# gooofy/zerovox

Hardware: AMD Instinct MI355X
Metric: audio samples/sec + RTF, 128-phoneme zero-shot synth @22.05kHz, 1/2/4/8 GPU (higher is better)
Workload: dtype f16+bf16

## Files before the change

### zerovox_amd/csrc/attention.hip

```cpp
#include "mfma_util.h"
#include "zvx_kernels.h"

#include <type_traits>

namespace zvx {

#ifndef FA_EXP
#define FA_EXP 0
#endif
#ifdef FA_PROFILE
#define FA_STAMP(k) do { const unsigned long long t_ = __builtin_readcyclecounter(); tacc[k] += t_ - tlast; tlast = t_; } while (0)
#else
#define FA_STAMP(k) do {} while (0)
#endif
#define FA_BQ 128
#define FA_BK 64
#define FA_NKB (FA_BK / 32)
#define FA_TAU 8.0f

typedef __attribute__((ext_vector_type(8))) _Float16 fa_f16x8;
template <bool F16>
__device__ __forceinline__ unsigned fa_pack2(float lo, float hi) {
    if (F16) {
        typedef _Float16 h2 __attribute__((ext_vector_type(2)));
// ... 278 lines not shown
        constexpr int C4N = NCOLS / 4, N = NROWS * C4N, IT = (N + 255) / 256;
        AfTile<IT> t;
#pragma unroll
        for (int it = 0; it < IT; it++) {
            const int i = tid + it * 256, r = i / C4N, c4 = i - r * C4N, row = row0 + r;
            t.v[it] = make_float4(0.f, 0.f, 0.f, 0.f);
            if (i < N && row < len) t.v[it] = *(const float4*)(src + (long)row * a.ld + c4 * 4);
        }
        return t;
    };
    auto tile_commit = [&](const auto& t, auto nrows_c, auto ncols_c, float* dst, int pitch) {
        constexpr int NROWS = decltype(nrows_c)::value, NCOLS = decltype(ncols_c)::value;
        constexpr int C4N = NCOLS / 4, N = NROWS * C4N, IT = (N + 255) / 256;
#pragma unroll
        for (int it = 0; it < IT; it++) {
            const int i = tid + it * 256, r = i / C4N, c4 = i - r * C4N;
            if (i < N) *(float4*)(dst + r * pitch + c4 * 4) = t.v[it];
        }
    };
    auto load_tile = [&](const float* src, int row0, auto nrows_c, auto ncols_c, float* dst, int pitch) {
        tile_commit(tile_fetch(src, row0, nrows_c, ncols_c), nrows_c, ncols_c, dst, pitch);
    };
    constexpr std::integral_constant<int, AF_BQ> c_bq{};
    constexpr std::integral_constant<int, AF_BK> c_bk{};
    constexpr std::integral_constant<int, D> c_d{};
    constexpr std::integral_constant<int, C0> c_c0{};
    constexpr std::integral_constant<int, C1> c_c1{};
    load_tile(base + a.q_off, q0, c_bq, c_d, Qs, QP);

    f32x16 o0, o1, o2;
#pragma unroll
    for (int e = 0; e < 16; e++) { o0[e] = 0.f; o1[e] = 0.f; o2[e] = 0.f; }
    float m_run = -INFINITY, l_run = 0.f;
    const int srow = tid >> 3, ssub = tid & 7;
    const float* const qrow = Qs + l32 * QP + 4 * kh;
    const float* const krow = Ks + (wave * 32 + l32) * KP + 4 * kh;
    const float* const prow = Ps + l32 * PP + 4 * kh;

    const int ntiles = (len + AF_BK - 1) / AF_BK;
    for (int kt = 0; kt < ntiles; kt++) {
        const int k0 = kt * AF_BK;
        const bool my_keys = k0 + wave * 32 < len;
        f32x16 s, s2;
#pragma unroll
        for (int e = 0; e < 16; e++) { s[e] = 0.f; s2[e] = 0.f; }
        __syncthreads();
        load_tile(base + a.k_off, k0, c_bk, c_c0, Ks, KP);
        __syncthreads();
        const auto k1 = tile_fetch(base + a.k_off + C0, k0, c_bk, c_c1);
        if (my_keys) {
#pragma unroll
            for (int j = 0; j < C0 / 8; j++) {
                const float4 qa = *(const float4*)(qrow + 8 * j), kb = *(const float4*)(krow + 8 * j);
                s = __builtin_amdgcn_mfma_f32_32x32x2f32(qa.x, kb.x, s, 0, 0, 0);
                s2 = __builtin_amdgcn_mfma_f32_32x32x2f32(qa.y, kb.y, s2, 0, 0, 0);
                s = __builtin_amdgcn_mfma_f32_32x32x2f32(qa.z, kb.z, s, 0, 0, 0);
                s2 = __builtin_amdgcn_mfma_f32_32x32x2f32(qa.w, kb.w, s2, 0, 0, 0);
            }
        }
        __syncthreads();
        tile_commit(k1, c_bk, c_c1, Ks, KP);
        const auto v0 = tile_fetch(base + a.v_off, k0, c_bk, c_c0);
        __syncthreads();
        if (my_keys) {
#pragma unroll
            for (int j = 0; j < C1 / 8; j++) {
                const float4 qa = *(const float4*)(qrow + C0 + 8 * j), kb = *(const float4*)(krow + 8 * j);
                s = __builtin_amdgcn_mfma_f32_32x32x2f32(qa.x, kb.x, s, 0, 0, 0);
                s2 = __builtin_amdgcn_mfma_f32_32x32x2f32(qa.y, kb.y, s2, 0, 0, 0);
                s = __builtin_amdgcn_mfma_f32_32x32x2f32(qa.z, kb.z, s, 0, 0, 0);
                s2 = __builtin_amdgcn_mfma_f32_32x32x2f32(qa.w, kb.w, s2, 0, 0, 0);
            }
            s += s2;
        }
#pragma unroll
        for (int e = 0; e < 16; e++) Ps[(8 * (e >> 2) + 4 * kh + (e & 3)) * PP + wave * 32 + l32] = s[e] * a.scale;
        __syncthreads();
        tile_commit(v0, c_bk, c_c0, Ks, KP);
        const auto v1 = tile_fetch(base + a.v_off + C0, k0, c_bk, c_c1);
        {
            float* const pr = Ps + srow * PP + ssub * 16;
            float v[16];
#pragma unroll
            for (int i = 0; i < 4; i++) { const float4 t = *(const float4*)(pr + 4 * i); v[4 * i] = t.x; v[4 * i + 1] = t.y; v[4 * i + 2] = t.z; v[4 * i + 3] = t.w; }
            const int kbase = k0 + ssub * 16;
            float m = -INFINITY;
#pragma unroll
            for (int i = 0; i < 16; i++) if (kbase + i < len) m = fmaxf(m, v[i]);
            m = fmaxf(m, __shfl_xor(m, 1, 64)); m = fmaxf(m, __shfl_xor(m, 2, 64)); m = fmaxf(m, __shfl_xor(m, 4, 64));
            const float m_new = fmaxf(m_run, m);
            const float alpha = m_run == -INFINITY ? 0.f : expf(m_run - m_new);
            float sum = 0.f;
#pragma unroll
            for (int i = 0; i < 16; i++) { v[i] = kbase + i < len ? expf(v[i] - m_new) : 0.f; sum += v[i]; }
            sum += __shfl_xor(sum, 1, 64); sum += __shfl_xor(sum, 2, 64); sum += __shfl_xor(sum, 4, 64);
            l_run = alpha * l_run + sum; m_run = m_new;
#pragma unroll
            for (int i = 0; i < 4; i++) *(float4*)(pr + 4 * i) = make_float4(v[4 * i], v[4 * i + 1], v[4 * i + 2], v[4 * i + 3]);
            if (ssub == 0) As[srow] = alpha;
        }
        __syncthreads();
        {
            float al[16];
#pragma unroll
            for (int g = 0; g < 4; g++) { const float4 t = *(const float4*)(As + 8 * g + 4 * kh); al[4 * g] = t.x; al[4 * g + 1] = t.y; al[4 * g + 2] = t.z; al[4 * g + 3] = t.w; }
#pragma unroll
            for (int e = 0; e < 16; e++) { o0[e] *= al[e]; o1[e] *= al[e]; o2[e] *= al[e]; }
        }
        auto pv_tile = [&](f32x16 acc, int col) {
            const float* const vc = Ks + col + 4 * kh * KP;
            f32x16 acc2;
#pragma unroll
            for (int e = 0; e < 16; e++) acc2[e] = 0.f;
#pragma unroll
            for (int j = 0; j < AF_BK / 8; j++) {
                const float4 pa = *(const float4*)(prow + 8 * j);
                const float* const vj = vc + 8 * j * KP;
                acc = __builtin_amdgcn_mfma_f32_32x32x2f32(pa.x, vj[0], acc, 0, 0, 0);
                acc2 = __builtin_amdgcn_mfma_f32_32x32x2f32(pa.y, vj[KP], acc2, 0, 0, 0);
                acc = __builtin_amdgcn_mfma_f32_32x32x2f32(pa.z, vj[2 * KP], acc, 0, 0, 0);
                acc2 = __builtin_amdgcn_mfma_f32_32x32x2f32(pa.w, vj[3 * KP], acc2, 0, 0, 0);
            }
            return acc + acc2;
        };
        o0 = pv_tile(o0, wave * 32 + l32);
        __syncthreads();
        tile_commit(v1, c_bk, c_c1, Ks, KP);
        __syncthreads();
        o1 = pv_tile(o1, min(wave * 32 + l32, C1 - 1));
        if (NT1 > 4 && wave == 3) o2 = pv_tile(o2, min(128 + l32, C1 - 1));
    }
    __syncthreads();
    if (ssub == 0) As[srow] = 1.0f / l_run;
    __syncthreads();
    float* const op = a.out + (long)b * a.o_bs + (long)h * D;
    auto store_tile = [&](const f32x16& acc, int col) {
        if (col >= D) return;
#pragma unroll
        for (int e = 0; e < 16; e++) {
            const int r = 8 * (e >> 2) + 4 * kh + (e & 3), q = q0 + r;
            if (q < a.L) {
                const float val = q < len ? acc[e] * As[r] : 0.f;
                op[(long)q * a.ldo + col] = val;
                if (a.planes) {
                    unsigned short hi, lo;
                    if (a.planes_f16) {
                        const _Float16 hh = (_Float16)__builtin_amdgcn_fmed3f(val, -65504.f, 65504.f);
                        hi = __builtin_bit_cast(unsigned short, hh);
                        lo = __builtin_bit_cast(unsigned short, (_Float16)__builtin_amdgcn_fmed3f((val - (float)hh) * 2048.f, -65504.f, 65504.f));
                    } else {
                        hi = __builtin_bit_cast(unsigned short, (__bf16)val);
                        lo = __builtin_bit_cast(unsigned short, (__bf16)(val - __uint_as_float((unsigned)hi << 16)));
                    }
                    unsigned short* const pp = a.planes + ((long)b * a.L + q) * 3 * a.planes_C + h * D + col;
                    pp[0] = hi; pp[a.planes_C] = hi; pp[2 * a.planes_C] = lo;
                }
            }
        }
    };
    store_tile(o0, wave * 32 + l32);
    store_tile(o1, C0 + wave * 32 + l32);
    if (NT1 > 4 && wave == 3) store_tile(o2, C0 + 128 + l32);
}

bool launch_attention_f32(const AttnF32Args& a, hipStream_t stream, bool dry_run) {
    if (a.D != 264 || a.L <= 0 || a.ld % 4 || a.q_off % 4 || a.k_off % 4 || a.v_off % 4) return false;
    if (dry_run) return true;
    if ((size_t)a.qkv & 15) return false;
    constexpr int D = 264, KP = (D - 128) + 4;
    const size_t lds = sizeof(float) * ((size_t)AF_BQ * (D + 4) + (size_t)AF_BK * KP + (size_t)AF_BQ * (AF_BK + 4) + 32);
    auto kfn = attn_f32_kernel<264>;
    if (!lds_opt_in((const void*)kfn)) return false;
    const dim3 grid((a.L + AF_BQ - 1) / AF_BQ, a.nbatch * a.nheads), block(256);
    hipLaunchKernelGGL(kfn, grid, block, lds, stream, a);
    return true;
}

}
```

### zerovox_amd/csrc/gemm.hip

```cpp
#include "mfma_util.h"
#include "zvx_kernels.h"

#include <cstring>
#include <type_traits>

#ifndef ZVX_GEMM_PART
#define ZVX_GEMM_PART 0
#endif
#define ZVX_PART_MAIN (ZVX_GEMM_PART != 2)
#define ZVX_PART_RESFUSE (ZVX_GEMM_PART != 1)
#if ZVX_GEMM_PART == 2
extern thread_local bool zvx_gemm_dry_run;
#else
thread_local hipEvent_t zvx_gemm_ev_start = nullptr, zvx_gemm_ev_stop = nullptr;
thread_local bool zvx_gemm_dry_run = false;
#endif
#define g_dry_run zvx_gemm_dry_run

#define ZVX_LAUNCH(...) do { if (!g_dry_run) ZVX_DISPATCH(__VA_ARGS__); } while (0)

namespace zvx {


#define PITCH 80
// ... 594 lines not shown
    constexpr bool WREG = R == 0;
    constexpr int F = BN / 32, CNT = F >= 4 ? F / 4 : 1, WD = 4, D = WREG ? WD : R - 1, WAITN = WREG ? (WD - 1) * TN : (D - 2) * CNT;
    const int nt32_total = (a.N + 31) >> 5;
    const int nsteps = a.ntaps * 4, gtotal = nkc * nsteps + nkc2 * 4;
    const uint4* wsrc[CNT];
#pragma unroll
    for (int j = 0; j < CNT; j++) {
        const int f = wave * CNT + j, t32 = (n0 >> 5) + f;
        wsrc[j] = (const uint4*)a.Wp + (long)(t32 < nt32_total ? t32 : 0) * gtotal * 64 + lane;
    }
    const int xrow0 = HL + wr * (BM / WM) + (lane & 31);
    const int koff = (lane >> 5) * 16;
    unsigned char* ring = slab + ((SR * SLAB_PITCH + 1023) & ~1023);
    const unsigned lds_base = (unsigned)(size_t)(__attribute__((address_space(3))) unsigned char*)slab;
    const int dvreg = a.dv[lane & (ZVX_MAX_TAPS - 1)];
    const bool loader = wave * CNT < F;
    const unsigned char* wq[TN];
#pragma unroll
    for (int i = 0; i < TN; i++) {
        const int t32 = (n0 >> 5) + wc * TN + i;
        wq[i] = (const unsigned char*)a.Wp + (long)(t32 < nt32_total ? t32 : 0) * gtotal * 1024;
    }
    const bool wave_dead = __builtin_amdgcn_readfirstlane((int)(n0 + wc * TN * 32 >= a.N)) != 0;
    const unsigned lane16 = lane * 16;
    u32x4 wreg[WREG ? WD : 1][TN] = {};
    auto wload = [&](int gs, int slot) {
        const long off = (long)(gs < gtotal ? gs : gtotal - 1) * 1024;
#pragma unroll
        for (int i = 0; i < TN; i++)
            asm volatile("global_load_dwordx4 %0, %1, %2" : "+v"(wreg[WREG ? slot : 0][i]) : "v"(lane16), "s"(wq[i] + off) : "memory");
    };
    auto dma = [&](int gs) {
        if (WREG || !loader) return;
        const int slot = gs & (R - 1);
        const long off = (long)(gs < gtotal ? gs : gtotal - 1) * 64;
#pragma unroll
        for (int j = 0; j < CNT; j++)
            __builtin_amdgcn_global_load_lds((const __attribute__((address_space(1))) void*)(wsrc[j] + off),
                                             (__attribute__((address_space(3))) void*)(ring + (slot * F + wave * CNT + j) * 1024), 16, 0, 0);
    };
    if (WREG) { wload(0, 0); wload(1, 1); wload(2, 2); wload(3, 3); }
    else {
#pragma unroll
        for (int s0 = 0; s0 < D; s0++) dma(s0);
    }

    for (int kc = 0; kc < nkc + nkc2; kc++) {
        const bool src2 = !FULLK && kc >= nkc;
        const unsigned short* const Xs = src2 ? Xp2 : Xp;
        const int ldxs = src2 ? a.ldx2 : a.ldx, Ks = src2 ? a.K2 : a.K, kbase = (src2 ? kc - nkc : kc) * SLAB_KC;
        {
            constexpr int FCH = NIT > 10 ? (NIT + 1) / 2 : NIT;
#pragma unroll
            for (int h0 = 0; h0 < NIT; h0 += FCH) {
                uint4 sv[FCH];
#pragma unroll
                for (int i = 0; i < FCH; i++) {
                    const int it = h0 + i;
                    const int c = tid + it * 256;
                    const int row = c >> 3, q = c & 7;
                    const int g = m0 - HL + row, k = kbase + q * 8;
                    sv[i] = make_uint4(0, 0, 0, 0);
                    if (it < NIT && c < SR * 8 && g >= 0 && g < in_rows && k < Ks && ((rowmask >> it) & 1)) sv[i] = *(const uint4*)(Xs + (long)g * ldxs + k);
                }
                if (kc && h0 == 0) __syncthreads();
#pragma unroll
                for (int i = 0; i < FCH; i++) {
                    const int c = tid + (h0 + i) * 256;
                    if (h0 + i < NIT && c < SR * 8) *(uint4*)(slab + (c >> 3) * SLAB_PITCH + (c & 7) * 16) = sv[i];
                }
            }
        }
        __syncthreads();
        int nk16 = 4;
        if (!FULLK) { nk16 = src2 ? n16_2 - (kc - nkc) * 4 : n16 - kc * 4; if (nk16 > 4) nk16 = 4; if (wave_dead) nk16 = 0; }
        const int ntaps_kc = src2 ? 1 : ntaps;

        uint4 xA[TM], wA[TN], xB[TM], wB[TN];
        const unsigned ring_rd = lds_base + (unsigned)(size_t)(ring - slab) + lane * 16 + wc * TN * 1024;
        const int gs0 = src2 ? nkc * nsteps + (kc - nkc) * 4 : kc * nsteps;
        auto rd = [&](uint4 (&xf)[TM], uint4 (&wf)[TN], int gs, unsigned rowoff, int kk) {
            if (!WREG) {
                const unsigned wa = ring_rd + (gs & ((WREG ? 1 : R) - 1)) * (F * 1024);
#pragma unroll
                for (int i = 0; i < TN; i++)
                    asm volatile("ds_read_b128 %0, %1 offset:%2" : "=v"(wf[i]) : "v"(wa), "n"(i * 1024));
            }
#pragma unroll
            for (int j = 0; j < TM; j++)
                asm volatile("ds_read_b128 %0, %1" : "=v"(xf[j]) : "v"(lds_base + rowoff + j * 32 * SLAB_PITCH + kk * 32));
        };
        auto mma = [&](uint4 (&xf)[TM], uint4 (&wf)[TN]) {
#pragma unroll
            for (int i = 0; i < TN; i++)
#pragma unroll
                for (int j = 0; j < TM; j++)
                    acc[i][j] = F16 ? __builtin_amdgcn_mfma_f32_32x32x16_f16(__builtin_bit_cast(f16x8, wf[i]), __builtin_bit_cast(f16x8, xf[j]), acc[i][j], 0, 0, 0)
                                    : __builtin_amdgcn_mfma_f32_32x32x16_bf16(__builtin_bit_cast(bf16x8, wf[i]),
                                                                       __builtin_bit_cast(bf16x8, xf[j]), acc[i][j], 0, 0, 0);
        };
        auto mma_r = [&](uint4 (&xf)[TM], int slot) {
#pragma unroll
            for (int i = 0; i < TN; i++)
#pragma unroll
                for (int j = 0; j < TM; j++)
                    acc[i][j] = F16 ? __builtin_amdgcn_mfma_f32_32x32x16_f16(__builtin_bit_cast(f16x8, wreg[WREG ? slot : 0][i]), __builtin_bit_cast(f16x8, xf[j]), acc[i][j], 0, 0, 0)
                                    : __builtin_amdgcn_mfma_f32_32x32x16_bf16(__builtin_bit_cast(bf16x8, wreg[WREG ? slot : 0][i]),
                                                                       __builtin_bit_cast(bf16x8, xf[j]), acc[i][j], 0, 0, 0);
        };
        auto rowoff_of = [&](int tap) {
            const int d = src2 ? 0 : __builtin_amdgcn_readlane(dvreg, tap < ntaps ? tap : ntaps - 1);
            return (unsigned)((xrow0 + d) * SLAB_PITCH + koff);
        };
        unsigned rowoff = rowoff_of(0);
        rd(xA, wA, gs0, rowoff, 0);
        for (int tap = 0; tap < ntaps_kc; tap++) {
            const unsigned rowoff_next = rowoff_of(tap + 1);
#pragma unroll
            for (int kk = 0; kk < 4; kk++) {
                const int gs = gs0 + tap * 4 + kk;
                if (WREG) asm volatile("s_waitcnt vmcnt(%0)" :: "n"(WAITN) : "memory");
                else asm volatile("s_waitcnt vmcnt(%0)\n\ts_barrier" :: "n"(WAITN) : "memory");
                dma(gs + D);
                if (kk & 1) rd(xA, wA, gs + 1, kk == 3 ? rowoff_next : rowoff, (kk + 1) & 3);
                else        rd(xB, wB, gs + 1, rowoff, kk + 1);
                asm volatile("s_waitcnt lgkmcnt(%0)" :: "n"(WREG ? TM : TM + TN) : "memory");
                __builtin_amdgcn_sched_barrier(0);
                if (FULLK || kk < nk16) {
                    if (WREG) { if (kk & 1) mma_r(xB, kk); else mma_r(xA, kk); }
                    else { if (kk & 1) mma(xB, wB); else mma(xA, wA); }
                }
                __builtin_amdgcn_sched_barrier(0);
                if (WREG) wload(gs + WD, kk);
            }
            rowoff = rowoff_next;
        }
        asm volatile("s_waitcnt lgkmcnt(0)" ::: "memory");
    }
    if (WREG) {
#pragma unroll
        for (int sl = 0; sl < (WREG ? WD : 1); sl++)
#pragma unroll
            for (int i = 0; i < TN; i++) asm volatile("s_waitcnt vmcnt(0)" : "+v"(wreg[sl][i]) :: "memory");
    } else {
        asm volatile("s_waitcnt vmcnt(0)" ::: "memory");
    }
    __syncthreads();
    if (EPI == ZVX_EPI_FLIP)
        epilogue_direct<TM, TN, !F16>(a, acc, b, m0 + wr * (BM / WM), n0 + wc * (BN / WN), out_len, lane, slab + wave * (32 * (TN * 64 + 16)));
    else if (EPI == ZVX_EPI(0, 0, 1))
        epilogue_direct<TM, TN, F16>(a, acc, b, m0 + wr * (BM / WM), n0 + wc * (BN / WN), out_len, lane, slab + wave * (32 * (TN * 64 + 16)));
    else
        epilogue_rows<TM, TN, 0, EPI, (F16 && EPI >= 0)>(a, acc, b, m0 + wr * (BM / WM), n0 + wc * (BN / WN), out_len, lane, slab + wave * (32 * (TN * 32 * 4 + 16)));
}

template <int C, int NT, int BM, int WM, int WN, int MINW, int MAXH = 64, bool F16 = false>
__global__ __launch_bounds__(256, MINW) void convreg_kernel(const GemmArgs a) {
    constexpr int TM = BM / WM / 32;
    constexpr int KS = C / 16;
    constexpr int PITCH_ = C * 2 + 16;
    constexpr int CPR = C / 8;
    constexpr int NIT = ((BM + MAXH) * CPR + 255) / 256;
    constexpr int FCH = NIT > 12 ? 8 : NIT;
    static_assert(WM * WN == 4 && WN * 32 == C, "wave layout");
    extern __shared__ __attribute__((aligned(16))) unsigned char slab[];

    const int tid = threadIdx.x, lane = tid & 63, wave = tid >> 6;
    const int wr = wave % WM, wc = wave / WM;
    int wg;
    {
        const int nwg = gridDim.x, id = blockIdx.x, q = nwg >> 3, r = nwg & 7, xcd = id & 7;
        wg = (xcd < r ? xcd * (q + 1) : r * (q + 1) + (xcd - r) * q) + (id >> 3);
    }
    const int m0 = wg * BM, b = blockIdx.y;
    const int out_len = a.out_len ? a.out_len[b] : a.M;
    const int in_len = a.in_len ? a.in_len[b] : a.in_len_static;
    if (m0 >= out_len || m0 >= a.M) return;
    const int HL = a.halo_l, SR = BM + a.halo_l + a.halo_r;
    const unsigned short* Xp = (const unsigned short*)a.X + (long)b * a.x_bs;

    uint4 w[NT][KS];
    {
        const uint4* Wq = (const uint4*)a.Wp + ((long)wc * NT * 4) * 64 + lane;
#pragma unroll
        for (int t = 0; t < NT; t++)
#pragma unroll
            for (int kk = 0; kk < KS; kk++) w[t][kk] = Wq[(t * 4 + kk) * 64];
    }
    {
        const bool flat = MAXH > 64 && a.flat_win;
        const int in_rows = flat ? a.flat_rows : in_len;
#pragma unroll
        for (int h0 = 0; h0 < NIT; h0 += FCH) {
            uint4 sv[FCH];
#pragma unroll
            for (int i = 0; i < FCH; i++) {
                const int c = tid + (h0 + i) * 256;
                const int row = c / CPR, q = c % CPR;
                const int g = m0 - HL + row;
                sv[i] = make_uint4(0, 0, 0, 0);
                if (h0 + i < NIT && c < SR * CPR && g >= 0 && g < in_rows && (!flat || (g % a.flat_win) < in_len)) sv[i] = *(const uint4*)(Xp + (long)g * a.ldx + q * 8);
            }
#pragma unroll
            for (int i = 0; i < FCH; i++) {
                const int c = tid + (h0 + i) * 256;
                if (h0 + i < NIT && c < SR * CPR) *(uint4*)(slab + (c / CPR) * PITCH_ + (c % CPR) * 16) = sv[i];
            }
        }
    }
    __syncthreads();

    f32x16 acc[1][TM];
#pragma unroll
    for (int j = 0; j < TM; j++)
#pragma unroll
        for (int e = 0; e < 16; e++) acc[0][j][e] = 0.f;
    const int xrow0 = HL + wr * (BM / WM) + (lane & 31);
    const int koff = (lane >> 5) * 16;
#pragma unroll
    for (int t = 0; t < NT; t++) {
        const unsigned char* rowp = slab + (xrow0 + a.dv[t]) * PITCH_ + koff;
#pragma unroll
        for (int kk = 0; kk < KS; kk++)
#pragma unroll
            for (int j = 0; j < TM; j++) {
                const uint4 xf = *(const uint4*)(rowp + j * 32 * PITCH_ + kk * 32);
                acc[0][j] = mfma16<F16>(w[t][kk], xf, acc[0][j]);
            }
    }
    __syncthreads();
    epilogue_rows<TM, 1>(a, acc, b, m0 + wr * (BM / WM), wc * 32, out_len, lane, slab + wave * (32 * (32 * 4 + 16)));
}

typedef __attribute__((ext_vector_type(2))) unsigned u32x2_t;
__device__ __forceinline__ void store_block_mfma_layout(unsigned short* row_ptr , const uint2 (&pk)[4], int lane, bool ok) {
#pragma unroll
    for (int pr = 0; pr < 2; pr++) {
        const u32x2_t sx = __builtin_amdgcn_permlane32_swap(pk[2 * pr].x, pk[2 * pr + 1].x, false, false);
        const u32x2_t sy = __builtin_amdgcn_permlane32_swap(pk[2 * pr].y, pk[2 * pr + 1].y, false, false);
        if (ok) *(u32x4*)(row_ptr + 8 * (2 * pr + (lane >> 5))) = (u32x4){sx.x, sy.x, sx.y, sy.y};
    }
}

template <int C, int BM, int WM, int WN, int MAXH, int MODE, int WGPC, bool POOL = false>
__global__ __launch_bounds__(WM * WN * 64, WM * WN * WGPC / 4) void conv2d_persist_kernel(const GemmArgs a, const int ntm, const int ntiles) {
    constexpr int NTHR = WM * WN * 64;
    constexpr int NT = 9, TM = BM / WM / 32, KS = C / 16, PITCH_ = C * 2 + 16, CPR = C / 8, RSTEP = NTHR / CPR;
    constexpr int NIT = ((BM + MAXH) * CPR + NTHR - 1) / NTHR;
    constexpr bool EC_LDS = NTHR > 256;
    static_assert(WN * 32 == C && BM % (WM * 32) == 0, "wave layout");
    extern __shared__ __attribute__((aligned(16))) unsigned char slab[];

    const int tid = threadIdx.x, lane = tid & 63, wave = __builtin_amdgcn_readfirstlane(tid >> 6);
    const int wr = wave % WM, wc = wave / WM;
    const int G = gridDim.x, xcd = blockIdx.x & 7, slot = blockIdx.x >> 3;
    auto tile_of = [&](int r) {
        const int base = r * G, n = ntiles - base < G ? ntiles - base : G;
        if (n <= 0) return ntiles;
        const int per = (n + 7) >> 3, t = xcd * per + slot;
        return (slot < per && t < n) ? base + t : ntiles;
    };
    const int HL = a.halo_l, SR = BM + a.halo_l + a.halo_r, win = a.flat_win, in_rows = a.flat_rows;

    uint4 w[NT][KS];
    {
        const uint4* Wq = (const uint4*)a.Wp + ((long)wc * NT * 4) * 64 + lane;
#pragma unroll
        for (int t = 0; t < NT; t++)
#pragma unroll
            for (int kk = 0; kk < KS; kk++) w[t][kk] = Wq[(t * 4 + kk) * 64];
    }
    float* const ecl = (float*)(slab + ((SR * PITCH_ + 15) & ~15));
    float4 ec0[EC_LDS ? 1 : 4], ec1[(MODE == 1 && !EC_LDS) ? 4 : 1];
    if (EC_LDS) {
        if (tid < C) { ecl[tid] = MODE == 0 ? a.bias[tid] : a.post_scale[tid]; if (MODE == 1) ecl[C + tid] = a.post_shift[tid]; }
    } else {
#pragma unroll
        for (int g = 0; g < 4; g++) {
            const int ch = wc * 32 + 8 * g + 4 * (lane >> 5);
            if (MODE == 0) ec0[g] = *(const float4*)(a.bias + ch);
            else { ec0[g] = *(const float4*)(a.post_scale + ch); ec1[g] = *(const float4*)(a.post_shift + ch); }
        }
    }
    u32x4 sv[NIT];
    const int row_t = tid / CPR, q8 = (tid % CPR) * 8;
    auto request = [&](int t) __attribute__((always_inline)) {
        const int b = t / ntm, m0 = (t - b * ntm) * BM;
        const int in_len = a.in_len[b];
        const __amdgpu_buffer_rsrc_t rs = __builtin_amdgcn_make_buffer_rsrc((void*)((const unsigned short*)a.X + (long)b * a.x_bs), 0, in_rows * a.ldx * 2, 0x00020000);
        int g = m0 - HL + row_t;
        int col = (g + 2 * win) % win;
#pragma unroll
        for (int it = 0; it < NIT; it++) {
            const bool ok = tid + it * NTHR < SR * CPR && g >= 0 && g < in_rows && col < in_len;
            sv[it] = __builtin_amdgcn_raw_buffer_load_b128(rs, ok ? (g * a.ldx + q8) * 2 : (int)0x80000000, 0, 0);
            g += RSTEP; col += RSTEP; if (col >= win) col -= win;
        }
    };
    int r = 0, t = tile_of(0);
    if (t < ntiles) request(t);
    const int xrow0 = HL + wr * (BM / WM) + (lane & 31);
    const int koff = (lane >> 5) * 16;
    constexpr bool pool = MODE == 0 && POOL;
    while (t < ntiles) {
        const int b = t / ntm, mt = t - b * ntm, m0 = mt * BM;
        if (r) asm volatile("s_waitcnt lgkmcnt(0)\n\ts_barrier" ::: "memory");
// ... 872 lines not shown
    if (a.flat_win && !a.bflat) {
        if (a.N == a.K && (a.N == 32 || a.N == 64) && !(a.slab_small & 32) && a.dtype == DT_BF16 && a.ntaps == 9 && a.in_len && !a.out_len && hl == a.flat_win + 1 && hr == hl &&
            a.flat_win >= 64 && (long)a.flat_rows * a.ldx * 2 < 0x7fffffffL &&
            a.out && a.out_dtype == DT_BF16 && a.alpha == 1.f && a.out_scale == 1.f && !a.res_mode && !a.accum_mode && !a.out_split3 && a.ldo % 8 == 0 &&
            ((a.post_scale && a.post_shift && a.bias_mode == 0 && a.act == ACT_RELU) || (!a.post_scale && a.bias_mode == 1 && a.bias && a.act == ACT_NONE))) {
            if (a.N == 32 && hl + hr <= 544) { launch_conv2d_persist<32, 384, 4, 1, 544, 2>(a, stream); return 26; }
            if (a.N == 64 && hl + hr <= 288) { launch_conv2d_persist<64, 256, 4, 2, 288, 1>(a, stream); return 27; }
        }
        if (a.N == a.K && a.N == 32 && launch_convreg_c<32, 384, 4, 1, 2>(a, stream)) return 14;
        if (a.N == a.K && a.N == 64 && launch_convreg_c<64, 256, 2, 2, 2>(a, stream)) return 15;
        if (a.N % 128 || a.K % SLAB_KC || hl + hr > 160) return -4;
        const int pad256 = ((a.M + 255) / 256) * 256, pad128 = ((a.M + 127) / 128) * 128;
        if ((long)pad256 * 100 > (long)pad128 * 115) {
            dim3 g128((a.N / 128) * (pad128 / 128), a.nbatch);
            size_t lds128 = ((size_t)(128 + hl + hr) * SLAB_PITCH + 1023) & ~(size_t)1023;
            const size_t stage128 = (size_t)4 * 32 * (2 * 128 + 16);
            if (lds128 < stage128) lds128 = stage128;
            ZVX_LAUNCH((convslab_kernel<128, 128, 2, 2, true, 2, 0, -1, 160>), g128, dim3(256), lds128, stream, a);
            return 22;
        }
        dim3 grid((a.N / 128) * ((a.M + 255) / 256), a.nbatch);
        size_t lds = ((size_t)(256 + hl + hr) * SLAB_PITCH + 1023) & ~(size_t)1023;
        ZVX_LAUNCH((convslab_kernel<256, 128, 2, 2, true, 2, 0, -1, 160>), grid, dim3(256), lds, stream, a);
        return 7;
    }
    if (a.dtype != DT_F32 && a.N == a.K && !a.K2 && (a.ntaps == 3 || a.ntaps == 5 || a.ntaps == 7 || a.ntaps == 11)) {
        if (a.N == 32 && launch_convreg_c<32, 512, 4, 1, 2>(a, stream)) return 14;
        if (a.N == 64 && launch_convreg_c<64, 256, 2, 2, 2>(a, stream)) return 15;
    }
    if (hl + hr > 64) {
        if (hl + hr <= 160 && a.N % 128 == 0 && a.K % SLAB_KC == 0 && !a.K2 && !a.bflat && !a.flat_win && gemm_epi_mode_of(a) == ZVX_EPI(1, 1, 1)) {
            dim3 grid((a.N / 128) * ((a.M + 255) / 256), a.nbatch);
            const size_t lds = ((size_t)(256 + hl + hr) * SLAB_PITCH + 1023) & ~(size_t)1023;
            if (a.dtype == DT_F16) ZVX_LAUNCH((convslab_kernel<256, 128, 2, 2, true, 2, 0, ZVX_EPI(1, 1, 1), 160, true>), grid, dim3(256), lds, stream, a);
            else ZVX_LAUNCH((convslab_kernel<256, 128, 2, 2, true, 2, 0, ZVX_EPI(1, 1, 1), 160>), grid, dim3(256), lds, stream, a);
            return 7;
        }
        return -4;
    }
    static const int bns[4] = {256, 128, 64, 32};
    static const double eff[4] = {0.95, 1.0, 0.7, 0.4};
    int best = 0; double best_cost = -1;
    for (int i = 0; i < 4; i++) {
        const double cost = (double)((a.N + bns[i] - 1) / bns[i]) * bns[i] / eff[i];
        if (best_cost < 0 || cost < best_cost - 1e-9) { best_cost = cost; best = i; }
    }
    static const int bms[4] = {128, 256, 256, 256};
    const int ncu = num_cus();
    if (g_slab_small >= 2 && a.M <= 64 && a.nbatch * ((a.N + 127) / 128) * 4 <= ncu && a.N >= 64 && hl + hr <= 64) {
        a.bflat = 0;
        dim3 g32((a.N + 31) / 32, a.nbatch);
        const size_t lds32 = (((size_t)(256 + hl + hr) * SLAB_PITCH + 1023) & ~(size_t)1023) + (size_t)8 * 1024;
        launch_slab_variant<256, 32, 4, 1, 2, 8>(a, g32, lds32, stream);
        return 9;
    }
    if (g_slab_small && a.M > 128 && a.N >= 128 && hl + hr <= 64) {
        const long wg256 = (long)((a.N + 127) / 128) * ((a.M + 255) / 256) * a.nbatch;
        if (wg256 * 2 <= ncu) {
            a.bflat = 0;
            const bool r64 = wg256 * 4 <= ncu;
            const int bm = r64 ? 64 : 128;
            dim3 gs(((a.N + 127) / 128) * ((a.M + bm - 1) / bm), a.nbatch);
            size_t lds = ((size_t)(bm + hl + hr) * SLAB_PITCH + 1023) & ~(size_t)1023;
            const size_t stage = (size_t)4 * 32 * (2 * 128 + 16);
            if (lds < stage) lds = stage;
            if (r64) launch_slab_variant<64, 128, 2, 2, 2, 0>(a, gs, lds, stream);
            else launch_slab_variant<128, 128, 2, 2, 2, 0>(a, gs, lds, stream);
            return 22;
        }
    }
    if (a.M <= 128 && a.N >= 128) {
        a.bflat = 0;
        const int wide = ((a.N + 255) / 256) * a.nbatch;
        const bool narrow = wide < 2 * ncu;
        const int bn = narrow ? 128 : 256;
        dim3 grid((a.N + bn - 1) / bn, a.nbatch);
        size_t lds = ((size_t)(128 + hl + hr) * SLAB_PITCH + 1023) & ~(size_t)1023;
        const size_t stage = (size_t)4 * 32 * (2 * 128 + 16);
        if (lds < stage) lds = stage;
        if (narrow && a.M > (g_slab_small ? 32 : 64) && ((a.N + 127) / 128) * a.nbatch < 2 * ncu) {
            dim3 g64(((a.N + 127) / 128) * ((a.M + 63) / 64), a.nbatch);
            launch_slab_variant<64, 128, 2, 2, 2, 0>(a, g64, lds, stream);
            return 22;
        }
        if (narrow) { launch_slab_variant<128, 128, 2, 2, 2, 0>(a, grid, lds, stream); return 22; }
        launch_slab_variant<128, 256, 1, 4, 2, 0>(a, grid, lds, stream);
        return 6;
    }
    if (a.ntaps == 1 && a.N >= 512) {
        const long slots = 2L * ncu;
        auto rounds = [&](int bm_, int bn_) {
            const long ntn_ = (a.N + bn_ - 1) / bn_, utt = ntn_ * ((a.M + bm_ - 1) / bm_) * a.nbatch;
            const long flat = a.bflat ? ntn_ * (((long)a.nbatch * a.bflat + bm_ - 1) / bm_) : utt;
            return ((flat < utt ? flat : utt) + slots - 1) / slots;
        };
        best = rounds(256, 128) <= rounds(128, 256) ? 1 : 0;
    }
    const bool wreg = best <= 1;
    const int ring_slots = wreg ? 0 : (best == 0 ? 4 : 8);
    const int bn = bns[best], bm = bms[best];
    const int ntn = (a.N + bn - 1) / bn;
    if (a.bflat) {
        const long slots = 2L * ncu;
        const long wg_utt = (long)ntn * ((a.M + bm - 1) / bm) * a.nbatch, wg_flat = (long)ntn * (((long)a.nbatch * a.bflat + bm - 1) / bm);
        if ((wg_flat + slots - 1) / slots < (wg_utt + slots - 1) / slots) { a.flat_win = a.bflat; a.flat_rows = a.nbatch * a.bflat; a.M = a.flat_rows; a.nbatch = 1; }
        else a.bflat = 0;
    }
    if (best == 1 && bflat_hint && a.M > 256 && hl + hr <= 64) {
        const long slots = 2L * ncu;
        const long t256 = (long)ntn * ((a.M + 255) / 256) * a.nbatch, t128 = (long)ntn * ((a.M + 127) / 128) * a.nbatch;
        const long eff256 = 2 * ((t256 + slots - 1) / slots), eff128 = (t128 + slots - 1) / slots;
        if (eff128 < eff256) {
            dim3 g128(ntn * ((a.M + 127) / 128), a.nbatch);
            size_t lds128 = ((size_t)(128 + hl + hr) * SLAB_PITCH + 1023) & ~(size_t)1023;
            const size_t stage128 = (size_t)4 * 32 * (2 * 128 + 16);
            if (lds128 < stage128) lds128 = stage128;
            switch (gemm_epi_mode_of(a)) {
                case ZVX_EPI(0, 0, 1): launch_slab_variant<128, 128, 2, 2, 2, 0, ZVX_EPI(0, 0, 1)>(a, g128, lds128, stream); break;
                case ZVX_EPI_DEC(0): launch_slab_variant<128, 128, 2, 2, 2, 0, ZVX_EPI_DEC(0)>(a, g128, lds128, stream); break;
                case ZVX_EPI_DEC(1): launch_slab_variant<128, 128, 2, 2, 2, 0, ZVX_EPI_DEC(1)>(a, g128, lds128, stream); break;
                default: launch_slab_variant<128, 128, 2, 2, 2, 0>(a, g128, lds128, stream);
            }
            return 22;
        }
    }
    const int ntm = (a.M + bm - 1) / bm;
    dim3 grid(ntn * ntm, a.nbatch);
    const int tn = (bn >= 128) ? 2 : 1;
    if (a.accum_mode && a.accum && a.accum_dtype == DT_F16 && tn == 2 && !(best == 1 && gemm_epi_mode_of(a) >= 0)) return -6;
    size_t lds = (((size_t)(bm + hl + hr) * SLAB_PITCH + 1023) & ~(size_t)1023) + (size_t)ring_slots * (bn / 32) * 1024;
    const size_t stage = (size_t)4 * 32 * (tn * 128 + 16);
    if (lds < stage) lds = stage;
    switch (best) {
        case 0: launch_slab_variant<128, 256, 1, 4, 2, 0>(a, grid, lds, stream); break;
        case 1: switch (gemm_epi_mode_of(a)) {
                    case ZVX_EPI(0, 0, 1): launch_slab_variant<256, 128, 2, 2, 2, 0, ZVX_EPI(0, 0, 1)>(a, grid, lds, stream); break;
                    case ZVX_EPI_FLIP: launch_slab_variant<256, 128, 2, 2, 2, 0, ZVX_EPI_FLIP>(a, grid, lds, stream); break;
                    case ZVX_EPI(1, 0, 1): launch_slab_variant<256, 128, 2, 2, 2, 0, ZVX_EPI(1, 0, 1)>(a, grid, lds, stream); break;
                    case ZVX_EPI(1, 2, 0): launch_slab_variant<256, 128, 2, 2, 2, 0, ZVX_EPI(1, 2, 0)>(a, grid, lds, stream); break;
                    case ZVX_EPI(1, 3, 0): launch_slab_variant<256, 128, 2, 2, 2, 0, ZVX_EPI(1, 3, 0)>(a, grid, lds, stream); break;
                    case ZVX_EPI(1, 1, 1): launch_slab_variant<256, 128, 2, 2, 2, 0, ZVX_EPI(1, 1, 1)>(a, grid, lds, stream); break;
                    case ZVX_EPI_DEC(0): launch_slab_variant<256, 128, 2, 2, 2, 0, ZVX_EPI_DEC(0)>(a, grid, lds, stream); break;
                    case ZVX_EPI_DEC(1): launch_slab_variant<256, 128, 2, 2, 2, 0, ZVX_EPI_DEC(1)>(a, grid, lds, stream); break;
                    default: launch_slab_variant<256, 128, 2, 2, 2, 0>(a, grid, lds, stream);
                }
                break;
        case 2: launch_slab_variant<256, 64, 2, 2, 2, 8>(a, grid, lds, stream); break;
        case 3: launch_slab_variant<256, 32, 4, 1, 2, 8>(a, grid, lds, stream); break;
    }
    return 6 + best;
}


int launch_gemm(const GemmArgs& a, hipStream_t stream) {
    if (a.N <= 0 || a.M <= 0 || a.nbatch <= 0) return -1;
    if (a.ds_out) return launch_conv2d_s2(a, stream) ? 28 : -7;
    if (a.stride == 2 && a.wout > 0 && a.ntaps == 9 && a.K == 64 && a.Wp && launch_conv2d_s2(a, stream)) return 29;
    if (a.ntaps < 1 || a.ntaps > ZVX_MAX_TAPS) return -2;
    if (a.out_split3 && (a.out_dtype != DT_F32 || a.N % 8 || a.flat_win || a.wout > 0)) return -2;
    if (a.N % 4 && (a.bias_mode == 1 || a.res_mode || a.accum_mode || a.post_scale || a.ldo < ((a.N + 3) & ~3))) return -2;
    if (a.Wp && a.dtype == DT_BF16 && a.wout > 0 && a.stride == 1 && a.ntaps == 9 && a.wout == a.win && a.M == a.hin * a.win && a.nheads == 1 && a.w_bs == 0 &&
        !a.k_len && a.K % 16 == 0 && a.N % 32 == 0 && a.ldo % 8 == 0 && a.ldx == a.K && !a.res_mode && !a.accum_mode && a.bias_mode != 2 && a.win <= 271) {
        bool ok9 = true;
        for (int t = 0; t < 9; t++) ok9 = ok9 && a.du[t] == t / 3 - 1 && a.dv[t] == t % 3 - 1;
        if (ok9 && (a.N == a.K ? (a.N == 32 || a.N == 64 || (a.N % 128 == 0 && 2 * (a.win + 1) <= 160)) : false)) {
            GemmArgs f = a;
            f.flat_win = a.win; f.flat_rows = a.hin * a.win;
            for (int t = 0; t < 9; t++) { f.dv[t] = a.du[t] * a.win + a.dv[t]; f.du[t] = 0; }
            f.wout = 0; f.out_len = nullptr;
            const int id = launch_convslab(f, stream);
            if (id >= 0) return id;
        }
    }
    if (a.Wp && a.dtype != DT_F32 && a.wout <= 0 && a.nheads == 1 && a.w_bs == 0 && !a.k_len && a.K % 16 == 0 && a.N % 8 == 0 && a.ldo % 8 == 0) {
        int lo = 0, hi = 0;
        for (int i = 0; i < a.ntaps; i++) { if (a.dv[i] < lo) lo = a.dv[i]; if (a.dv[i] > hi) hi = a.dv[i]; }
        if (hi - lo <= 64 && hi >= 0 && lo <= 0) return launch_convslab(a, stream);
        if (hi - lo <= 96 && hi >= 0 && lo <= 0 && a.ntaps == 7 && a.N == a.K && (a.N == 32 || a.N == 64 || a.N == 128) && !a.K2 && !a.out_split3 && !a.bflat) {
            const int id = launch_convslab(a, stream);
            if (id >= 0) return id;
        }
    }
    if (a.out_split3 || a.K2) return -2;
    static const int bns[3] = {128, 64, 32};
    static const double eff[3] = {1.0, 0.75, 0.45};
    int best = 0; double best_cost = -1;
    for (int i = 0; i < 3; i++) {
        const double cost = (double)((a.N + bns[i] - 1) / bns[i]) * bns[i] / eff[i];
        if (best_cost < 0 || cost < best_cost - 1e-9) { best_cost = cost; best = i; }
    }
    int bn = bns[best], bm = (bn == 128) ? 128 : 256;
    int ntn = (a.N + bn - 1) / bn, ntm = (a.M + bm - 1) / bm;
    if ((long)ntn * ntm * a.nbatch * a.nheads < 512 && a.N >= 64) {
        bm = bn = 64; ntn = (a.N + 63) / 64; ntm = (a.M + 63) / 64;
        dim3 grid(ntn * ntm, a.nbatch * a.nheads), block(256);
        if (a.dtype == DT_BF16) { ZVX_LAUNCH((gemm_kernel<DT_BF16, 64, 64, 2, 2>), grid, block, 0, stream, a); return 18; }
        if (a.dtype == DT_F16) { ZVX_LAUNCH((gemm_kernel<DT_F16, 64, 64, 2, 2>), grid, block, 0, stream, a); return 18; }
        ZVX_LAUNCH((gemm_kernel<DT_F32, 64, 64, 2, 2>), grid, block, 0, stream, a);
        return 19;
    }
    dim3 grid(ntn * ntm, a.nbatch * a.nheads), block(256);
    const int base = (a.dtype != DT_F32) ? 0 : 3;
    const int id = base + best;
    if (a.dtype == DT_F16) {
        switch (id) {
            case 0: ZVX_LAUNCH((gemm_kernel<DT_F16, 128, 128, 2, 2>), grid, block, 0, stream, a); break;
            case 1: ZVX_LAUNCH((gemm_kernel<DT_F16, 256, 64, 4, 1>), grid, block, 0, stream, a); break;
            case 2: ZVX_LAUNCH((gemm_kernel<DT_F16, 256, 32, 4, 1>), grid, block, 0, stream, a); break;
        }
        return id;
    }
    switch (id) {
        case 0: ZVX_LAUNCH((gemm_kernel<DT_BF16, 128, 128, 2, 2>), grid, block, 0, stream, a); break;
        case 1: ZVX_LAUNCH((gemm_kernel<DT_BF16, 256, 64, 4, 1>), grid, block, 0, stream, a); break;
        case 2: ZVX_LAUNCH((gemm_kernel<DT_BF16, 256, 32, 4, 1>), grid, block, 0, stream, a); break;
        case 3: ZVX_LAUNCH((gemm_kernel<DT_F32, 128, 128, 2, 2>), grid, block, 0, stream, a); break;
        case 4: ZVX_LAUNCH((gemm_kernel<DT_F32, 256, 64, 4, 1>), grid, block, 0, stream, a); break;
        case 5: ZVX_LAUNCH((gemm_kernel<DT_F32, 256, 32, 4, 1>), grid, block, 0, stream, a); break;
    }
    return id;
}

int gemm_variant_of(const GemmArgs& a) {
    g_dry_run = true;
    const int id = a.fused == 2 ? launch_rb2fuse(a, nullptr) : (a.fused ? launch_resfuse(a, nullptr) : launch_gemm(a, nullptr));
    g_dry_run = false;
    return id;
}

#endif
}
```

### zerovox_amd/csrc/ops.hip

```cpp
#include "zvx_kernels.h"

#include <algorithm>

namespace zvx {

__device__ __forceinline__ float ld(const void* p, int dt, long i) {
    if (dt == DT_F16) return (float)((const _Float16*)p)[i];
    return dt == DT_F32 ? ((const float*)p)[i] : __uint_as_float(((unsigned)((const unsigned short*)p)[i]) << 16);
}
__device__ __forceinline__ unsigned short tobf(float f) {
    unsigned u = __float_as_uint(f);
    u += 0x7fffu + ((u >> 16) & 1u);
    return (unsigned short)(u >> 16);
}
__device__ __forceinline__ void unpack8(const uint4 t, int dt, float v[8]) {
    if (dt == DT_F16) {
        typedef _Float16 h2 __attribute__((ext_vector_type(2)));
        const h2 a = __builtin_bit_cast(h2, t.x), b = __builtin_bit_cast(h2, t.y), c = __builtin_bit_cast(h2, t.z), d = __builtin_bit_cast(h2, t.w);
        v[0] = (float)a.x; v[1] = (float)a.y; v[2] = (float)b.x; v[3] = (float)b.y; v[4] = (float)c.x; v[5] = (float)c.y; v[6] = (float)d.x; v[7] = (float)d.y;
    } else {
        v[0] = __uint_as_float(t.x << 16); v[1] = __uint_as_float(t.x & 0xffff0000u);
        v[2] = __uint_as_float(t.y << 16); v[3] = __uint_as_float(t.y & 0xffff0000u);
        v[4] = __uint_as_float(t.z << 16); v[5] = __uint_as_float(t.z & 0xffff0000u);
        v[6] = __uint_as_float(t.w << 16); v[7] = __uint_as_float(t.w & 0xffff0000u);
    }
}
__device__ __forceinline__ float clamp_h(float v) { return __builtin_amdgcn_fmed3f(v, -65504.f, 65504.f); }
__device__ __forceinline__ uint4 pack8(const float v[8], int dt) {
    uint4 o;
    if (dt == DT_F16) {
        typedef _Float16 h2 __attribute__((ext_vector_type(2)));
        o.x = __builtin_bit_cast(unsigned, (h2){(_Float16)clamp_h(v[0]), (_Float16)clamp_h(v[1])}); o.y = __builtin_bit_cast(unsigned, (h2){(_Float16)clamp_h(v[2]), (_Float16)clamp_h(v[3])});
        o.z = __builtin_bit_cast(unsigned, (h2){(_Float16)clamp_h(v[4]), (_Float16)clamp_h(v[5])}); o.w = __builtin_bit_cast(unsigned, (h2){(_Float16)clamp_h(v[6]), (_Float16)clamp_h(v[7])});
    } else {
        o.x = (unsigned)tobf(v[0]) | ((unsigned)tobf(v[1]) << 16); o.y = (unsigned)tobf(v[2]) | ((unsigned)tobf(v[3]) << 16);
        o.z = (unsigned)tobf(v[4]) | ((unsigned)tobf(v[5]) << 16); o.w = (unsigned)tobf(v[6]) | ((unsigned)tobf(v[7]) << 16);
    }
    return o;
}
__device__ __forceinline__ void st(void* p, int dt, long i, float v) {
    if (dt == DT_F16) { ((_Float16*)p)[i] = (_Float16)clamp_h(v); return; }
    if (dt == DT_F32) ((float*)p)[i] = v; else ((unsigned short*)p)[i] = tobf(v);
}
__device__ __forceinline__ float wave_sum(float v) {
#pragma unroll
    for (int o = 32; o > 0; o >>= 1) v += __shfl_xor(v, o, 64);
    return v;
}
__device__ __forceinline__ float wave_max(float v) {
#pragma unroll
    for (int o = 32; o > 0; o >>= 1) v = fmaxf(v, __shfl_xor(v, o, 64));
    return v;
}
__device__ __forceinline__ float act_apply(float v, int act, float slope) {
    if (act == ACT_RELU) return fmaxf(v, 0.f);
    if (act == ACT_LRELU) return v >= 0.f ? v : v * slope;
    if (act == ACT_TANH) return tanhf(v);
    return v;
}

__global__ void k_cast(const void* in, int idt, void* out, int odt, size_t n) {
    size_t i = (size_t)blockIdx.x * blockDim.x + threadIdx.x;
    const size_t stride = (size_t)gridDim.x * blockDim.x;
    for (; i < n; i += stride) st(out, odt, i, ld(in, idt, i));
}
void launch_cast(const void* in, int in_dt, void* out, int out_dt, size_t n, hipStream_t s) {
    if (!n) return;
    int blocks = (int)((n + 255) / 256); if (blocks > 4096) blocks = 4096;
    hipLaunchKernelGGL(k_cast, dim3(blocks), dim3(256), 0, s, in, in_dt, out, out_dt, n);
}
__global__ __launch_bounds__(256) void k_transpose16(const unsigned short* in, int ld_in, unsigned short* out, int ld_out, int rows_max, int C, const int* len) {
    __shared__ unsigned short tile[64][66];
    const int b = blockIdx.z, r0 = blockIdx.y * 64, c0 = blockIdx.x * 64;
    const int rows = len ? min(len[b], rows_max) : rows_max;
    const unsigned short* ip = in + (long)b * rows_max * ld_in;
    unsigned short* op = out + (long)b * C * ld_out;
    for (int i = threadIdx.x; i < 64 * 64; i += 256) {
        const int r = i >> 6, c = i & 63;
        tile[r][c] = (r0 + r < rows && c0 + c < C) ? ip[(long)(r0 + r) * ld_in + c0 + c] : (unsigned short)0;
    }
    __syncthreads();
    for (int i = threadIdx.x; i < 64 * 64; i += 256) {
        const int c = i >> 6, r = i & 63;
        if (c0 + c < C && r0 + r < ld_out) op[(long)(c0 + c) * ld_out + r0 + r] = (r0 + r < rows) ? tile[r][c] : (unsigned short)0;
    }
}
void launch_transpose16(const void* in, int ld_in, void* out, int ld_out, int B, int rows, int C, hipStream_t s, const int* len) {
    if (rows <= 0) return;
    hipLaunchKernelGGL(k_transpose16, dim3((C + 63) / 64, (ld_out + 63) / 64, B), dim3(256), 0, s, (const unsigned short*)in, ld_in, (unsigned short*)out, ld_out, rows, C, len);
}

void launch_f32_to_bf16(const float* in, bf16_t* out, size_t n, hipStream_t s) { launch_cast(in, DT_F32, out, DT_BF16, n, s); }

__device__ __forceinline__ void split2(float v, unsigned short& hi, unsigned short& lo) {
    hi = tobf(v);
    lo = tobf(v - __uint_as_float(((unsigned)hi) << 16));
}
__device__ __forceinline__ void split2h(float v, unsigned short& hi, unsigned short& lo) {
    const _Float16 h = (_Float16)clamp_h(v);
    hi = __builtin_bit_cast(unsigned short, h);
    lo = __builtin_bit_cast(unsigned short, (_Float16)clamp_h((v - (float)h) * 2048.f));
}
__device__ __forceinline__ void split2x(float v, int f16, unsigned short& hi, unsigned short& lo) { if (f16) split2h(v, hi, lo); else split2(v, hi, lo); }
__global__ __launch_bounds__(256) void k_split3(const float* x, int ldx, unsigned short* out, int rows_max, const int* rows, int C, int f16) {
    const int b = blockIdx.y, r = blockIdx.x;
    const bool live = r < (rows ? rows[b] : rows_max);
    const float* xr = x + ((long)b * rows_max + r) * ldx;
    unsigned short* o = out + ((long)b * rows_max + r) * 3 * C;
    for (int c = threadIdx.x * 4; c < C; c += blockDim.x * 4) {
        unsigned short h[4], l[4];
        if (live) { const float4 v = *(const float4*)(xr + c); split2x(v.x, f16, h[0], l[0]); split2x(v.y, f16, h[1], l[1]); split2x(v.z, f16, h[2], l[2]); split2x(v.w, f16, h[3], l[3]); }
        else { for (int e = 0; e < 4; e++) h[e] = l[e] = 0; }
        const uint2 hv = make_uint2(h[0] | ((unsigned)h[1] << 16), h[2] | ((unsigned)h[3] << 16));
        const uint2 lv = make_uint2(l[0] | ((unsigned)l[1] << 16), l[2] | ((unsigned)l[3] << 16));
        *(uint2*)(o + c) = hv; *(uint2*)(o + C + c) = hv; *(uint2*)(o + 2 * C + c) = lv;
    }
}
void launch_split3(const float* x, int ldx, void* out, int B, int rows_max, const int* rows, int C, hipStream_t s, int f16) {
    if (rows_max <= 0) return;
    hipLaunchKernelGGL(k_split3, dim3(rows_max, B), dim3(C >= 1024 ? 256 : 128), 0, s, x, ldx, (unsigned short*)out, rows_max, rows, C, f16);
}
__global__ void k_split3_w(const float* w, unsigned short* out, long nrows, int K, int f16, float scale) {
    const long r = blockIdx.x;
    if (r >= nrows) return;
    for (int k = threadIdx.x; k < K; k += blockDim.x) {
        unsigned short h, l, h3;
        if (f16) {
            const float v = w[r * K + k] * scale;
            const _Float16 wh = (_Float16)clamp_h(v);
            h = __builtin_bit_cast(unsigned short, wh);
            l = __builtin_bit_cast(unsigned short, (_Float16)(v - (float)wh));
            h3 = __builtin_bit_cast(unsigned short, (_Float16)clamp_h(v * (1.0f / 2048.f)));
        } else { split2(w[r * K + k], h, l); h3 = h; }
        out[r * 3 * K + k] = h; out[r * 3 * K + K + k] = l; out[r * 3 * K + 2 * K + k] = h3;
    }
}
void launch_split3_weights(const float* w, void* out, long nrows, int K, hipStream_t s, int f16, float scale) {
    hipLaunchKernelGGL(k_split3_w, dim3((unsigned)nrows), dim3(256), 0, s, w, (unsigned short*)out, nrows, K, f16, scale);
}
__global__ void k_absmax(const float* x, size_t n, unsigned* out) {
    float m = 0.f;
    for (size_t i = (size_t)blockIdx.x * blockDim.x + threadIdx.x; i < n; i += (size_t)gridDim.x * blockDim.x) m = fmaxf(m, fabsf(x[i]));
    m = wave_max(m);
    if ((threadIdx.x & 63) == 0) atomicMax(out, __float_as_uint(m));
}
void launch_absmax(const float* x, size_t n, float* out, hipStream_t s) {
    (void)hipMemsetAsync(out, 0, 4, s);
    if (!n) return;
    int blocks = (int)((n + 255) / 256); if (blocks > 1024) blocks = 1024;
    hipLaunchKernelGGL(k_absmax, dim3(blocks), dim3(256), 0, s, x, n, (unsigned*)out);
}

__global__ void k_embed(const int* ph, const int* pu, const float* emb, int ed, const float* pemb, int pd,
                        const float* pe, float* out, int Tmax, const int* T) {
    const int b = blockIdx.y, t = blockIdx.x;
    if (t >= T[b]) return;
    const int H = ed + pd;
    const int p = ph[b * Tmax + t], q = pu[b * Tmax + t];
    float* o = out + ((long)b * Tmax + t) * H;
    for (int c = threadIdx.x; c < H; c += blockDim.x) {
        float v = c < ed ? emb[(long)p * ed + c] : pemb[(long)q * pd + (c - ed)];
        o[c] = v + pe[(long)t * H + c];
    }
}
void launch_embed(const int* phoneme, const int* puncts, const float* emb, int emb_dim, const float* pemb,
                  int pemb_dim, const float* pe, float* out, int B, int Tmax, const int* T, hipStream_t s) {
    hipLaunchKernelGGL(k_embed, dim3(Tmax, B), dim3(128), 0, s, phoneme, puncts, emb, emb_dim, pemb, pemb_dim, pe, out, Tmax, T);
}

__global__ void k_layernorm(const void* x, int xdt, int ldx, void* y, int ydt, int ldy, int rows_max, const int* rows,
                            int C, int mode, float eps, const float* gamma, const float* beta, const float* bg,
                            long bg_bs, const float* post_add, unsigned short* planes, int planes_f16) {
    const int b = blockIdx.y;
    const int r = blockIdx.x * 4 + (threadIdx.x >> 6);
    const int lane = threadIdx.x & 63;
    const int nr = rows ? rows[b] : rows_max;
    if (r >= nr) {
        if (planes && r < rows_max) { unsigned short* o = planes + ((long)b * rows_max + r) * 3 * C; for (int c = lane; c < 3 * C; c += 64) o[c] = 0; }
        return;
    }
    const long xo = ((long)b * rows_max + r) * ldx, yo = ((long)b * rows_max + r) * ldy;
    if ((C & 7) == 0 && C <= 1024 && (ldx & 7) == 0 && (ldy & 7) == 0) {
        float v[2][8];
        bool has[2];
        float s = 0.f;
#pragma unroll
        for (int i = 0; i < 2; i++) {
            const int c = (lane + 64 * i) * 8;
            has[i] = c < C;
            if (has[i] && xdt == DT_F32) {
                const float4 t0 = *(const float4*)((const float*)x + xo + c), t1 = *(const float4*)((const float*)x + xo + c + 4);
                v[i][0] = t0.x; v[i][1] = t0.y; v[i][2] = t0.z; v[i][3] = t0.w; v[i][4] = t1.x; v[i][5] = t1.y; v[i][6] = t1.z; v[i][7] = t1.w;
            } else if (has[i]) unpack8(*(const uint4*)((const unsigned short*)x + xo + c), xdt, v[i]);
            else { for (int e = 0; e < 8; e++) v[i][e] = 0.f; }
#pragma unroll
            for (int e = 0; e < 8; e++) s += v[i][e];
        }
        const float mu = wave_sum(s) / C;
        float q = 0.f;
#pragma unroll
        for (int i = 0; i < 2; i++)
#pragma unroll
            for (int e = 0; e < 8; e++) { const float d = has[i] ? v[i][e] - mu : 0.f; q += d * d; }
        q = wave_sum(q);
        const float inv = mode == 0 ? 1.0f / sqrtf(q / C + eps) : 1.0f / (sqrtf(q / (C - 1)) + eps);
#pragma unroll
        for (int i = 0; i < 2; i++) {
            if (!has[i]) continue;
            const int c = (lane + 64 * i) * 8;
            const float* gp = mode == 0 ? gamma + c : bg + (long)b * bg_bs + C + c;
            const float* bp = mode == 0 ? beta + c : bg + (long)b * bg_bs + c;
            const float4 g0 = *(const float4*)gp, g1 = *(const float4*)(gp + 4), b0 = *(const float4*)bp, b1 = *(const float4*)(bp + 4);
            const float g[8] = {g0.x, g0.y, g0.z, g0.w, g1.x, g1.y, g1.z, g1.w}, be[8] = {b0.x, b0.y, b0.z, b0.w, b1.x, b1.y, b1.z, b1.w};
            float o[8];
#pragma unroll
            for (int e = 0; e < 8; e++) o[e] = (v[i][e] - mu) * inv * g[e] + be[e];
            if (post_add) {
                const float4 p0 = *(const float4*)(post_add + (long)b * C + c), p1 = *(const float4*)(post_add + (long)b * C + c + 4);
                o[0] += p0.x; o[1] += p0.y; o[2] += p0.z; o[3] += p0.w; o[4] += p1.x; o[5] += p1.y; o[6] += p1.z; o[7] += p1.w;
            }
            if (ydt != DT_F32) *(uint4*)((unsigned short*)y + yo + c) = pack8(o, ydt);
            else {
                *(float4*)((float*)y + yo + c) = make_float4(o[0], o[1], o[2], o[3]);
                *(float4*)((float*)y + yo + c + 4) = make_float4(o[4], o[5], o[6], o[7]);
            }
            if (planes) {
                unsigned short hh[8], ll[8];
#pragma unroll
                for (int e = 0; e < 8; e++) split2x(o[e], planes_f16, hh[e], ll[e]);
                const uint4 hv = make_uint4(hh[0] | ((unsigned)hh[1] << 16), hh[2] | ((unsigned)hh[3] << 16), hh[4] | ((unsigned)hh[5] << 16), hh[6] | ((unsigned)hh[7] << 16));
                const uint4 lv = make_uint4(ll[0] | ((unsigned)ll[1] << 16), ll[2] | ((unsigned)ll[3] << 16), ll[4] | ((unsigned)ll[5] << 16), ll[6] | ((unsigned)ll[7] << 16));
                unsigned short* po = planes + ((long)b * rows_max + r) * 3 * C + c;
                *(uint4*)po = hv; *(uint4*)(po + C) = hv; *(uint4*)(po + 2 * C) = lv;
            }
        }
        return;
    }
    float s = 0.f;
    for (int c = lane; c < C; c += 64) s += ld(x, xdt, xo + c);
    const float mu = wave_sum(s) / C;
    float q = 0.f;
    for (int c = lane; c < C; c += 64) { float d = ld(x, xdt, xo + c) - mu; q += d * d; }
    q = wave_sum(q);
    float inv;
    if (mode == 0) inv = 1.0f / sqrtf(q / C + eps);
    else inv = 1.0f / (sqrtf(q / (C - 1)) + eps);
    for (int c = lane; c < C; c += 64) {
        float g, be;
        if (mode == 0) { g = gamma[c]; be = beta[c]; }
        else { be = bg[(long)b * bg_bs + c]; g = bg[(long)b * bg_bs + C + c]; }
        float v = (ld(x, xdt, xo + c) - mu) * inv * g + be;
        if (post_add) v += post_add[(long)b * C + c];
        st(y, ydt, yo + c, v);
        if (planes) {
            unsigned short hi, lo;
            split2x(v, planes_f16, hi, lo);
            unsigned short* o = planes + ((long)b * rows_max + r) * 3 * C;
            o[c] = hi; o[C + c] = hi; o[2 * C + c] = lo;
        }
    }
}
void launch_layernorm(const void* x, int x_dt, int ldx, void* y, int y_dt, int ldy, int B, int rows_max,
                      const int* rows, int C, int mode, float eps, const float* gamma, const float* beta,
                      const float* bg, long bg_bs, const float* post_add, hipStream_t s, void* split_planes, int planes_f16) {
    hipLaunchKernelGGL(k_layernorm, dim3((rows_max + 3) / 4, B), dim3(256), 0, s, x, x_dt, ldx, y, y_dt, ldy, rows_max,
                       rows, C, mode, eps, gamma, beta, bg, bg_bs, post_add, (unsigned short*)split_planes, planes_f16);
}

__global__ void k_softmax_rows(const float* sc, int lds, void* P, int pdt, int ldp, int nheads, int Lmax, const int* len) {
    const int z = blockIdx.y, b = z / nheads;
    const int r = blockIdx.x * 4 + (threadIdx.x >> 6), lane = threadIdx.x & 63;
    const int L = len[b];
    if (r >= L) return;
    const float* row = sc + ((long)z * Lmax + r) * lds;
    const long po = ((long)z * Lmax + r) * ldp;
    float m = -INFINITY;
    for (int c = lane; c < L; c += 64) m = fmaxf(m, row[c]);
    m = wave_max(m);
    float s = 0.f;
    for (int c = lane; c < L; c += 64) s += expf(row[c] - m);
    s = wave_sum(s);
    const float inv = 1.0f / s;
    const int Lp = (L + 7) & ~7;
    for (int c = lane; c < Lp; c += 64) st(P, pdt, po + c, c < L ? expf(row[c] - m) * inv : 0.f);
}
void launch_softmax_rows(const float* scores, int lds, void* P, int p_dt, int ldp, int nbatch, int nheads,
                         int Lmax, const int* len, hipStream_t s) {
    hipLaunchKernelGGL(k_softmax_rows, dim3((Lmax + 3) / 4, nbatch * nheads), dim3(256), 0, s, scores, lds, P, p_dt, ldp, nheads, Lmax, len);
}

__global__ void k_rowdot(const float* x, int ldx, const float* w, float bias, float* out, int Tmax, const int* T, int C) {
    const int b = blockIdx.y, t = blockIdx.x * 4 + (threadIdx.x >> 6), lane = threadIdx.x & 63;
    if (t >= T[b]) return;
    const float* row = x + ((long)b * Tmax + t) * ldx;
    float s = 0.f;
    for (int c = lane; c < C; c += 64) s += row[c] * w[c];
    s = wave_sum(s);
    if (lane == 0) out[b * Tmax + t] = s + bias;
}
void launch_rowdot(const float* x, int ldx, const float* w, float bias, float* out, int B, int Tmax,
                   const int* T, int C, hipStream_t s) {
    hipLaunchKernelGGL(k_rowdot, dim3((Tmax + 3) / 4, B), dim3(256), 0, s, x, ldx, w, bias, out, Tmax, T, C);
}

__global__ void k_bucket_embed_add(const float* pred, const float* table, int nb, float* x, int ldx, int C, int* idx_out,
                                   int Tmax, const int* T) {
    const int b = blockIdx.y, t = blockIdx.x * 4 + (threadIdx.x >> 6), lane = threadIdx.x & 63;
    if (t >= T[b]) return;
    float p = rintf(pred[b * Tmax + t] * (float)(nb - 1));
    p = fminf(fmaxf(p, 0.f), (float)(nb - 1));
    const int idx = (int)p;
    if (lane == 0 && idx_out) idx_out[b * Tmax + t] = idx;
    float* row = x + ((long)b * Tmax + t) * ldx;
    for (int c = lane; c < C; c += 64) row[c] += table[(long)idx * C + c];
}
void launch_bucket_embed_add(const float* pred, const float* table, int nbins, float* x, int ldx, int C,
                             int* idx_out, int B, int Tmax, const int* T, hipStream_t s) {
    hipLaunchKernelGGL(k_bucket_embed_add, dim3((Tmax + 3) / 4, B), dim3(256), 0, s, pred, table, nbins, x, ldx, C, idx_out, Tmax, T);
}

__global__ void k_bucket_embed_add_ctl(const float* pred, const float* shift, const float* range, const float* target,
                                       const float* table, int nb, float* x, int ldx, int C, int* idx_out, int Tmax, const int* T) {
#pragma clang fp contract(off)
    const int b = blockIdx.y, t = blockIdx.x * 4 + (threadIdx.x >> 6), lane = threadIdx.x & 63;
    const int n = T[b];
    const float* pb = pred + (long)b * Tmax;
    if (blockIdx.x * 4 >= n) return;
    __shared__ float mean_s;
    if (range) {
        if (threadIdx.x < 64) {
            double s = 0.0;
            for (int u = lane; u < n; u += 64) s += (double)pb[u];
#pragma unroll
            for (int o = 32; o > 0; o >>= 1) s += __shfl_xor(s, o, 64);
            if (lane == 0) mean_s = (float)(s / (double)n);
        }
        __syncthreads();
    }
    if (t >= n) return;
    const float r1 = range ? range[b] - 1.0f : 0.f, sh = shift ? shift[b] : 0.f;
    float v = pb[t];
    if (range) v = v + r1 * (v - mean_s);
    if (shift) v = v + sh;
    if (target) { const float g = target[(long)b * Tmax + t]; if (g == g) v = g; }
    float p = rintf(v * (float)(nb - 1));
    p = fminf(fmaxf(p, 0.f), (float)(nb - 1));
    const int idx = (int)p;
    if (lane == 0 && idx_out) idx_out[b * Tmax + t] = idx;
    float* row = x + ((long)b * Tmax + t) * ldx;
    for (int c = lane; c < C; c += 64) row[c] += table[(long)idx * C + c];
}
void launch_bucket_embed_add_ctl(const float* pred, const float* shift, const float* range, const float* target, const float* table,
                                 int nbins, float* x, int ldx, int C, int* idx_out, int B, int Tmax, const int* T, hipStream_t s) {
    hipLaunchKernelGGL(k_bucket_embed_add_ctl, dim3((Tmax + 3) / 4, B), dim3(256), 0, s, pred, shift, range, target, table, nbins, x, ldx, C, idx_out, Tmax, T);
}

__global__ void k_durations(const int* forced, const float* logd, int* dur, int* cum, int* mel_len, int Tmax, const int* T) {
    const int b = blockIdx.x, lane = threadIdx.x;
    const int n = T[b];
    long long carry = 0;
    for (int t0 = 0; t0 < n; t0 += 64) {
        const int t = t0 + lane;
        int d = 0;
        if (t < n) {
            if (forced) d = min(max(forced[b * Tmax + t], 0), 65536);
            else d = (int)fminf(fmaxf(rintf(expf(logd[b * Tmax + t]) - 1.0f), 0.f), 65536.f);
            dur[b * Tmax + t] = d;
        }
        int v = d;
#pragma unroll
        for (int o = 1; o < 64; o <<= 1) { int u = __shfl_up(v, o, 64); if (lane >= o) v += u; }
        if (t < n) cum[b * Tmax + t] = (int)min(carry + v, 0x7fffffffLL);
        carry += __shfl(v, 63, 64);
    }
    if (lane == 0) mel_len[b] = (int)min(carry, 0x7fffffffLL);
}
void launch_durations(const int* forced, const float* logd, int* dur, int* cum, int* mel_len, int B, int Tmax,
                      const int* T, hipStream_t s) {
    hipLaunchKernelGGL(k_durations, dim3(B), dim3(64), 0, s, forced, logd, dur, cum, mel_len, Tmax, T);
}

__global__ void k_durations_q16(const int* forced, const float* logd, const int* q, int* dur, int* cum, int* mel_len, int Tmax, const int* T) {
    const int b = blockIdx.x, lane = threadIdx.x;
    const int n = T[b];
    long long carry = 0;
    for (int t0 = 0; t0 < n; t0 += 64) {
        const int t = t0 + lane;
        long long wgt = 0;
        if (t < n) {
            int d;
            if (forced) d = min(max(forced[b * Tmax + t], 0), 65536);
            else d = (int)fminf(fmaxf(rintf(expf(logd[b * Tmax + t]) - 1.0f), 0.f), 65536.f);
            wgt = (long long)d * q[b * Tmax + t];
        }
        long long v = wgt;
#pragma unroll
        for (int o = 1; o < 64; o <<= 1) { long long u = __shfl_up(v, o, 64); if (lane >= o) v += u; }
        if (t < n) {
            const long long P = carry + v;
            const long long Cn = (P + 32768) >> 16, Cp = (P - wgt + 32768) >> 16;
            dur[b * Tmax + t] = (int)(Cn - Cp);
            cum[b * Tmax + t] = (int)min(Cn, 0x7fffffffLL);
        }
        carry += __shfl(v, 63, 64);
    }
    if (lane == 0) mel_len[b] = (int)min((carry + 32768) >> 16, 0x7fffffffLL);
}
void launch_durations_q16(const int* forced, const float* logd, const int* q, int* dur, int* cum, int* mel_len, int B, int Tmax,
                          const int* T, hipStream_t s) {
    hipLaunchKernelGGL(k_durations_q16, dim3(B), dim3(64), 0, s, forced, logd, q, dur, cum, mel_len, Tmax, T);
}
// ... 1260 lines not shown
```

### zerovox_amd/csrc/zvx.hip

```cpp
#include "../../include/zvx.h"
#include "zvx_kernels.h"

#include <dlfcn.h>
#include <math.h>
#include <cmath>
#include <rccl/rccl.h>
#include <stdarg.h>
#include <stdio.h>
#include <string.h>

#include <algorithm>
#include <map>
#include <sstream>
#include <stdexcept>
#include <string>
#include <vector>

using namespace zvx;

namespace {

struct ZvxError : std::runtime_error {
    int code;
    ZvxError(int c, const std::string& m) : std::runtime_error(m), code(c) {}
// ... 89 lines not shown
    int slab_small = 2, slab_flat = 1;
    int poison_pads = 0;
    int sat_check = 0;
    unsigned long long* sat_count_dev() { return (unsigned long long*)buf("sat.count", 64); }
    void sat_scan(const void* x, int dt, long bs, int ld, int B, int rows_max, const int* rows, int C) {
        if (sat_check && x && dt == DT_F16) launch_count_sat16(x, bs, ld, B, rows_max, rows, C, sat_count_dev(), stream);
    }
    int use_rb2fuse = 1;
    int use_stagefuse = 1;
    struct NsWeights { void* W = nullptr; float* bias = nullptr; int woff[18] = {0}; };
    std::map<std::string, NsWeights> ns_weights;
    int use_pairstream = 1;
    int shape_log = 0;
    int max_frames = 1 << 18;
    int out_rate = 0;
    struct RsBank { int L = 0, M = 0, half = 0, T = 0, pitch = 0; const float* dev = nullptr; };
    std::map<std::pair<int, int>, RsBank> rs_banks;
    std::map<int, LoudCoef> loud_coefs;
    void* join_host = nullptr;
    size_t join_host_cap = 0;
    void* join_pinned(size_t bytes) {
        if (bytes > join_host_cap) {
            if (join_host) { HIPCHK(hipStreamSynchronize(stream)); HIPCHK(hipHostFree(join_host)); join_host = nullptr; join_host_cap = 0; }
            const size_t cap = bytes + bytes / 8 + 256;
            HIPCHK(hipHostMalloc(&join_host, cap, hipHostMallocDefault));
            join_host_cap = cap;
        }
        return join_host;
    }
    hipEvent_t stage_ev[ZVX_T_COUNT][2];
    bool stage_used[ZVX_T_COUNT];
    float stage_ms[ZVX_T_COUNT];
    std::vector<GemmEvent> pending;
    std::vector<zvx_kernel_stat> stats;
    std::string tag = "other";
    std::map<std::string, zvx_kernel_stat> tagstats;
    std::map<std::string, zvx_kernel_stat> namedstats;
    std::vector<hipEvent_t> event_pool;

    int cfg_int(const char* k) const {
        auto it = cfg.find(k);
        if (it == cfg.end()) fail(ZVX_E_MANIFEST, "manifest: missing cfg '%s'", k);
        return atoi(it->second.c_str());
    }
    std::vector<int> cfg_list(const char* k) const {
        auto it = cfg.find(k);
        if (it == cfg.end()) fail(ZVX_E_MANIFEST, "manifest: missing cfg '%s'", k);
        std::vector<int> v; std::stringstream ss(it->second); std::string tok;
        while (std::getline(ss, tok, ',')) if (!tok.empty()) v.push_back(atoi(tok.c_str()));
        return v;
    }
    const Tensor& t(const std::string& name) const {
        auto it = tensors.find(name);
        if (it == tensors.end()) fail(ZVX_E_MANIFEST, "weights: tensor '%s' missing", name.c_str());
        return it->second;
    }
    bool has(const std::string& name) const { return tensors.count(name) != 0; }
    const float* pf(const std::string& name) const { return (const float*)t(name).dev; }

    void drain_for_free() {
        HIPCHK(hipStreamSynchronize(stream));
        for (hipStream_t s2 : {main0, front_stream, aux_stream, voc_aux[0], voc_aux[1], comm_stream, copy_stream})
            if (s2 && s2 != stream) HIPCHK(hipStreamSynchronize(s2));
    }
    void* buf(const std::string& name, size_t bytes) {
        DevBuf& d = bufs[name];
        if (bytes > d.cap) {
            if (d.base) { drain_for_free(); HIPCHK(hipFree(d.base)); d.base = nullptr; d.p = nullptr; }
            size_t cap = bytes + bytes / 8 + 256;
            HIPCHK(hipMalloc(&d.base, cap));
            HIPCHK(hipMemsetAsync(d.base, 0, cap, stream));
            d.p = d.base;
            d.cap = cap;
        }
        return d.p;
    }
    char* carve(const std::string& pool, const std::vector<std::string>& names, size_t bytes_each, size_t* stride_out) {
        const size_t stride = (bytes_each + 255) & ~(size_t)255;
        char* base = (char*)buf(pool, stride * names.size());
        for (size_t i = 0; i < names.size(); i++) {
            DevBuf& d = bufs[names[i]];
            if (d.base) { drain_for_free(); HIPCHK(hipFree(d.base)); d.base = nullptr; }
            d.p = base + i * stride; d.cap = stride;
        }
        *stride_out = stride;
        return base;
    }
    int* ibuf(const std::string& name, size_t n) { return (int*)buf(name, n * sizeof(int)); }
    float* fbuf(const std::string& name, size_t n) { return (float*)buf(name, n * sizeof(float)); }
    struct Arena { char* p = nullptr; size_t cap = 0, cur = 0; hipEvent_t ev = nullptr; bool pending = false; };
    Arena arena[2];
    int arena_i = 0;
    int api_depth = 0;
    static constexpr size_t ARENA_BYTES = 2u << 20;
    void arena_begin() {
        Arena& a = arena[arena_i];
        if (a.pending) { HIPCHK(hipEventSynchronize(a.ev)); a.pending = false; }
        a.cur = 0;
    }
    void arena_end() {
        Arena& a = arena[arena_i];
        if (!a.cur || !stream) return;
        if (!a.ev) HIPCHK(hipEventCreateWithFlags(&a.ev, hipEventDisableTiming));
        HIPCHK(hipEventRecord(a.ev, stream));
        a.pending = true;
        arena_i ^= 1;
    }
    void upload(void* dst, const void* src, size_t bytes) {
        Arena& a = arena[arena_i];
        const size_t need = (bytes + 63) & ~(size_t)63;
        if (!a.p) { HIPCHK(hipHostMalloc((void**)&a.p, ARENA_BYTES, hipHostMallocDefault)); a.cap = ARENA_BYTES; }
        if (a.cur + need > a.cap) {
            HIPCHK(hipMemcpyAsync(dst, src, bytes, hipMemcpyHostToDevice, stream));
            HIPCHK(hipStreamSynchronize(stream));
            return;
        }
        memcpy(a.p + a.cur, src, bytes);
        HIPCHK(hipMemcpyAsync(dst, a.p + a.cur, bytes, hipMemcpyHostToDevice, stream));
        a.cur += need;
    }
    int* upload_ints(const std::string& name, const int* v, size_t n) {
        int* d = ibuf(name, n);
        upload(d, v, n * sizeof(int));
        return d;
    }
    size_t es() const { return dtype_size(dt); }

    hipEvent_t new_event() {
        hipEvent_t e;
        if (!event_pool.empty()) { e = event_pool.back(); event_pool.pop_back(); return e; }
        HIPCHK(hipEventCreate(&e));
        return e;
    }
    void stage_begin(int s) { if (profile) { HIPCHK(hipEventRecord(stage_ev[s][0], stream)); } }
    void stage_end(int s) { if (profile) { HIPCHK(hipEventRecord(stage_ev[s][1], stream)); stage_used[s] = true; } }

    template <typename V, typename L, typename D>
    void profiled(V&& vid, L&& launch, D&& describe) {
        const bool prof = profile >= 2 && (profile_only < 0 || vid() == profile_only);
        if (!prof) { launch(); return; }
        GemmEvent ev{};
        ev.a = new_event(); ev.b = new_event();
        struct Armed { Armed(hipEvent_t a, hipEvent_t b) { profile_events(a, b); } ~Armed() { profile_events(nullptr, nullptr); } };
        ev.variant = [&] { Armed armed(ev.a, ev.b); return launch(); }();
        describe(ev);
        ev.tag = tag;
        pending.push_back(ev);
    }
    void gemm(GemmArgs& a) {
        if (a.flops <= 0) a.flops = 2.0 * (double)a.M * a.nbatch * a.nheads * (double)a.N * ((double)a.K * a.ntaps + (double)a.K2);
        if (!a.Wp && a.dtype != DT_F32) { auto it = packed.find(a.W); if (it != packed.end()) a.Wp = it->second; }
        a.slab_small = slab_small | (spk_s2_fuse ? 0 : 32); a.xcd_flat = slab_flat;
        profiled([&] { return gemm_variant_of(a); }, [&] {
            const int id = a.fused == 2 ? launch_rb2fuse(a, stream) : (a.fused ? launch_resfuse(a, stream) : launch_gemm(a, stream));
            if (id < 0) fail(ZVX_E_INVALID, "launch_gemm rejected shape M=%d N=%d K=%d taps=%d", a.M, a.N, a.K, a.ntaps);
            return id;
        }, [&](GemmEvent& ev) {
            ev.flops = a.flops; ev.rows = (long)a.M * a.nbatch * a.nheads; ev.N = a.N; ev.K = a.K; ev.taps = a.ntaps; ev.res = a.res_mode; ev.fused = a.fused;
            const double esz = dtype_size(a.dtype);
            const double cells = (double)a.M * a.nbatch * a.nheads * a.N;
            ev.bytes = ((double)a.M * a.nbatch * a.nheads) * (double)(a.K + a.K2) * esz + (double)a.N * ((double)a.K * a.ntaps + a.K2) * esz * (a.fused ? 2 : 1) +
                       (a.out ? cells * dtype_size(a.out_dtype) : 0.0) + ((a.res_mode && !a.fused) ? cells * dtype_size(a.res_dtype) : 0.0) +
                       ((a.accum && (a.accum_mode & 1)) ? cells * dtype_size(a.accum_dtype) : 0.0) + ((a.accum && (a.accum_mode & 2)) ? cells * dtype_size(a.accum_dtype) : 0.0);
        });
        if (sat_check && a.nheads == 1) {
            sat_scan(a.out, a.out_dtype, a.o_bs, a.ldo, a.nbatch, a.M, a.out_len, a.N);
            if (a.accum && (a.accum_mode & 2)) sat_scan(a.accum, a.accum_dtype, a.a_bs, a.lda, a.nbatch, a.M, a.out_len, a.N);
        }
    }
    bool run_stream(StreamArgs& a) {
        const int id = launch_resstream(a, this->stream, true);
        if (id < 0) return false;
        profiled([&] { return id; }, [&] {
            const int id2 = launch_resstream(a, this->stream, false);
            if (id2 < 0) fail(ZVX_E_INVALID, "launch_resstream rejected a shape its dry run accepted (C=%d k=%d pairs=%d)", a.C, a.ntaps, a.npair);
            return id2;
        }, [&](GemmEvent& ev) {
            const double rows = (double)a.M * a.nbatch;
            ev.flops = 2.0 * 2.0 * a.npair * rows * a.C * a.C * a.ntaps; ev.rows = (long)rows; ev.N = a.C; ev.K = a.C; ev.taps = a.ntaps;
            ev.res = a.accum_mode; ev.fused = 10 + a.npair;
            ev.bytes = rows * a.C * 2.0 * (1 + (a.out ? 1 : 0) + ((a.accum && (a.accum_mode & 1)) ? 1 : 0) + ((a.accum && (a.accum_mode & 2)) ? 1 : 0));
        });
        return true;
    }
    template <typename F>
    void timed(double flops, double bytes, F&& f, const char* kname = nullptr) {
        const bool prof = profile >= 2 && profile_only < 0;
        GemmEvent ev{};
        if (prof) { ev.a = new_event(); ev.b = new_event(); HIPCHK(hipEventRecord(ev.a, stream)); }
        f();
        if (prof) { HIPCHK(hipEventRecord(ev.b, stream)); ev.variant = -1; ev.flops = flops; ev.bytes = bytes; ev.tag = tag; if (kname) ev.kname = kname; pending.push_back(ev); }
    }
    void resolve_events() {
        if (stats.empty()) {
            stats.resize(gemm_num_variants());
            for (int i = 0; i < gemm_num_variants(); i++) { memset(&stats[i], 0, sizeof stats[i]); snprintf(stats[i].name, 64, "%s", gemm_variant_name(i)); }
        }
        for (auto& e : pending) {
            float ms = 0.f;
            HIPCHK(hipEventElapsedTime(&ms, e.a, e.b));
            if (shape_log && e.variant >= 0) fprintf(stderr, "launch %-24s rows=%-8ld N=%-4d K=%-4d taps=%-2d res=%d fused=%d  %8.3f ms %8.1f TF/s %8.1f GB/s(alg)\n",
                                   gemm_variant_name(e.variant), e.rows, e.N, e.K, e.taps, e.res, e.fused, ms, e.flops / ms / 1e9, e.bytes / ms / 1e6);
            else if (shape_log) fprintf(stderr, "launch %-24s [%s]  %8.3f ms %8.1f GB/s(alg)\n", "(helper)", e.tag.c_str(), ms, e.bytes / ms / 1e6);
            if (e.variant >= 0) { auto& s = stats[e.variant]; s.launches++; s.ms += ms; s.flops += e.flops; s.bytes += e.bytes; }
            auto& ts = tagstats[e.tag];
            if (!ts.name[0]) snprintf(ts.name, 64, "%s", e.tag.c_str());
            ts.launches++; ts.ms += ms; ts.flops += e.flops; ts.bytes += e.bytes;
            if (!e.kname.empty()) {
                auto& ks = namedstats[e.kname];
                if (!ks.name[0]) snprintf(ks.name, 64, "%s", e.kname.c_str());
                ks.launches++; ks.ms += ms; ks.flops += e.flops; ks.bytes += e.bytes;
            }
            event_pool.push_back(e.a); event_pool.push_back(e.b);
        }
        pending.clear();
        for (int s = 0; s < ZVX_T_COUNT; s++)
            if (stage_used[s]) { float ms = 0.f; HIPCHK(hipEventElapsedTime(&ms, stage_ev[s][0], stage_ev[s][1])); stage_ms[s] = ms; stage_used[s] = false; }
    }
    void sync() {
        if (front_stream) HIPCHK(hipStreamSynchronize(front_stream));
        HIPCHK(hipStreamSynchronize(stream));
        if (comm_stream) HIPCHK(hipStreamSynchronize(comm_stream));
        if (copy_stream && !copy_is_comm) HIPCHK(hipStreamSynchronize(copy_stream));
        if (profile) resolve_events();
    }
    void quiesce_side_streams() noexcept {
        if (front_stream) (void)hipStreamSynchronize(front_stream);
        if (aux_stream) (void)hipStreamSynchronize(aux_stream);
        for (int i = 0; i < 2; i++) if (voc_aux[i]) (void)hipStreamSynchronize(voc_aux[i]);
        front_dirty_main = true; mel_free_pending = false;
    }
    void front_setup() {
        if (front_stream) return;
        int least = 0, greatest = 0;
        HIPCHK(hipDeviceGetStreamPriorityRange(&least, &greatest));
        HIPCHK(hipStreamCreateWithPriority(&front_stream, hipStreamNonBlocking, greatest));
        HIPCHK(hipEventCreateWithFlags(&ev_front_done, hipEventDisableTiming));
        HIPCHK(hipEventCreateWithFlags(&ev_mel_free, hipEventDisableTiming));
        HIPCHK(hipEventCreateWithFlags(&ev_main_join, hipEventDisableTiming));
    }
};

namespace {

GemmArgs gemm_base(int dtype) {
    GemmArgs a;
    memset(&a, 0, sizeof a);
    a.dtype = dtype; a.nbatch = 1; a.nheads = 1; a.ntaps = 1; a.stride = 1; a.wout = 0; a.hin = 1; a.win = 0;
    a.alpha = 1.f; a.out_scale = 1.f; a.out_dtype = dtype; a.res_dtype = dtype;
    return a;
}
void set_taps_1d(GemmArgs& a, int k, int dilation) {
    a.ntaps = k;
    for (int i = 0; i < k; i++) { a.du[i] = 0; a.dv[i] = (int)((i - (k - 1) / 2) * dilation); }
}

void parse_manifest(zvx_ctx* c, const char* manifest, const void* weights, size_t nbytes) {
    if (!manifest || !weights) fail(ZVX_E_MANIFEST, "manifest/weights pointer is NULL");
    const size_t nfloats = nbytes / 4;
    c->host_blob.assign((const float*)weights, (const float*)weights + nfloats);
    std::stringstream ss(manifest);
    std::string line;
    bool first = true;
    while (std::getline(ss, line)) {
        if (line.empty()) continue;
        std::stringstream ls(line);
        std::string kw; ls >> kw;
        if (first) { if (kw != "zvx_manifest") fail(ZVX_E_MANIFEST, "manifest: bad magic '%s'", kw.c_str()); first = false; continue; }
        if (kw == "cfg") {
            std::string k, v; ls >> k; std::getline(ls, v);
            size_t p = v.find_first_not_of(' ');
            c->cfg[k] = p == std::string::npos ? "" : v.substr(p);
        } else if (kw == "tensor") {
            std::string name, kind; int nd = 0; ls >> name >> kind >> nd;
            Tensor t; t.kind = kind.empty() ? 'p' : kind[0]; t.numel = 1;
            for (int i = 0; i < nd; i++) { int d; ls >> d; t.dims.push_back(d); t.numel *= (size_t)d; }
            ls >> t.off;
            if (ls.fail() || t.off + t.numel > nfloats) fail(ZVX_E_MANIFEST, "manifest: tensor '%s' out of blob bounds", name.c_str());
            c->tensors[name] = t;
        } else {
            fail(ZVX_E_MANIFEST, "manifest: unknown line '%s'", line.c_str());
        }
    }
    if (first) fail(ZVX_E_MANIFEST, "manifest: empty");
}

void build_split_weights(zvx_ctx* c, bool f16) {
    const char* sfx = f16 ? ".s3h" : ".s3";
    if (c->has(std::string("enc.0.wqk") + sfx)) return;
    std::vector<std::pair<std::string, Tensor>> add;
    size_t stotal = 0;
    for (auto& kv : c->tensors) {
        const Tensor& t = kv.second;
        const bool mine = kv.first.rfind("enc.", 0) == 0;
        if (!mine || t.kind != 'f' || t.dtype != DT_F32 || t.dims.size() != 3 || (3 * t.dim(2)) % 16 || t.dim(1) % 8) continue;
        Tensor s3 = t;
        s3.kind = 's'; s3.dtype = f16 ? DT_F16 : DT_BF16; s3.dims = {t.dim(0), t.dim(1), 3 * t.dim(2)}; s3.numel = t.numel * 3; s3.host = nullptr;
        stotal += ((s3.numel * 2 + 255) & ~(size_t)255) + ((packed_weight_elems(s3.dim(0), s3.dim(1), s3.dim(2)) * 2 + 255) & ~(size_t)255);
        add.emplace_back(kv.first + sfx, s3);
    }
    char* sarena = stotal ? (char*)c->buf(f16 ? "weights_split_h" : "weights_split", stotal) : nullptr;
    float* mx_d = f16 ? c->fbuf("weights_split_absmax", 64) : nullptr;
    size_t soff = 0;
    for (auto& kv : add) {
        Tensor& s3 = kv.second;
        const Tensor& src = c->tensors[kv.first.substr(0, kv.first.size() - strlen(sfx))];
        float scale = 1.f;
        if (f16) {
            float mx = 0.f;
            launch_absmax((const float*)src.dev, src.numel, mx_d, c->stream);
            HIPCHK(hipMemcpyAsync(&mx, mx_d, 4, hipMemcpyDeviceToHost, c->stream));
            HIPCHK(hipStreamSynchronize(c->stream));
            if (!(mx > 0.f) || !std::isfinite(mx)) mx = 1.f;
            int e = 0; (void)frexpf(mx, &e);
            int sh = 15 - e; sh = std::max(-24, std::min(sh, 40));
            scale = ldexpf(1.f, sh);
            s3.alpha = ldexpf(1.f, -sh);
        }
        s3.dev = sarena + soff; soff += (s3.numel * 2 + 255) & ~(size_t)255;
        launch_split3_weights((const float*)src.dev, s3.dev, (long)src.dim(0) * src.dim(1), src.dim(2), c->stream, f16 ? 1 : 0, scale);
        void* pk = sarena + soff; soff += (packed_weight_elems(s3.dim(0), s3.dim(1), s3.dim(2)) * 2 + 255) & ~(size_t)255;
        launch_pack_weights(s3.dev, s3.dim(0), s3.dim(1), s3.dim(2), pk, c->stream);
        c->packed[s3.dev] = pk;
        c->tensors[kv.first] = s3;
    }
    HIPCHK(hipStreamSynchronize(c->stream));
}

void upload_weights(zvx_ctx* c) {
    size_t total = 0;
    for (auto& kv : c->tensors) {
        Tensor& t = kv.second;
        t.dtype = (t.kind == 'w') ? c->dt : DT_F32;
        total += (t.numel * dtype_size(t.dtype) + 255) & ~(size_t)255;
    }
    char* arena = (char*)c->buf("weights", total);
    float* staging = c->fbuf("weights_staging", c->host_blob.size());
    HIPCHK(hipMemcpyAsync(staging, c->host_blob.data(), c->host_blob.size() * 4, hipMemcpyHostToDevice, c->stream));
    size_t off = 0;
    for (auto& kv : c->tensors) {
        Tensor& t = kv.second;
        t.dev = arena + off;
        t.host = c->host_blob.data() + t.off;
        launch_cast(staging + t.off, DT_F32, t.dev, t.dtype, t.numel, c->stream);
        off += (t.numel * dtype_size(t.dtype) + 255) & ~(size_t)255;
    }
    size_t ptotal = 0;
    for (auto& kv : c->tensors) {
        Tensor& t = kv.second;
        if (t.kind == 'w' && t.dtype == DT_BF16 && t.dims.size() == 3 && t.dim(2) % 8 == 0)
            ptotal += (packed_weight_elems(t.dim(0), t.dim(1), t.dim(2)) * 2 + 255) & ~(size_t)255;
    }
    if (ptotal) {
        char* parena = (char*)c->buf("weights_packed", ptotal);
        size_t poff = 0;
        for (auto& kv : c->tensors) {
            Tensor& t = kv.second;
            if (t.kind == 'w' && t.dtype == DT_BF16 && t.dims.size() == 3 && t.dim(2) % 8 == 0) {
                launch_pack_weights(t.dev, t.dim(0), t.dim(1), t.dim(2), parena + poff, c->stream);
                c->packed[t.dev] = parena + poff;
                poff += (packed_weight_elems(t.dim(0), t.dim(1), t.dim(2)) * 2 + 255) & ~(size_t)255;
            }
        }
    }
    if (c->dt == DT_BF16) {
        std::vector<std::pair<std::string, Tensor>> add16;
        size_t htotal = 0;
        for (auto& kv : c->tensors) {
            const Tensor& t = kv.second;
            if ((kv.first.rfind("sty.", 0) != 0 && kv.first.rfind("dec.", 0) != 0 && kv.first.rfind("voc.", 0) != 0) || t.kind != 'w' || t.dtype != DT_BF16 || t.dims.size() != 3 || t.dim(2) % 8) continue;
            Tensor hcopy = t; hcopy.dtype = DT_F16; hcopy.kind = 'h';
            htotal += ((t.numel * 2 + 255) & ~(size_t)255) + ((packed_weight_elems(t.dim(0), t.dim(1), t.dim(2)) * 2 + 255) & ~(size_t)255);
            add16.emplace_back(kv.first + ".h16", hcopy);
        }
        char* harena = htotal ? (char*)c->buf("weights_f16", htotal) : nullptr;
        size_t hoff = 0;
        for (auto& kv : add16) {
            Tensor& t = kv.second;
            t.dev = harena + hoff; hoff += (t.numel * 2 + 255) & ~(size_t)255;
            launch_cast(staging + t.off, DT_F32, t.dev, DT_F16, t.numel, c->stream);
            void* pk = harena + hoff; hoff += (packed_weight_elems(t.dim(0), t.dim(1), t.dim(2)) * 2 + 255) & ~(size_t)255;
            launch_pack_weights(t.dev, t.dim(0), t.dim(1), t.dim(2), pk, c->stream);
            c->packed[t.dev] = pk;
            c->tensors[kv.first] = t;
        }
    }
    for (const char* blk : {"sty.enc0", "sty.dec0", "sty.dec1", "sty.dec2"})
        for (const char* sfx : {"", ".h16"}) {
            const std::string n2 = std::string(blk) + ".c2" + sfx, ns = std::string(blk) + ".sc" + sfx;
            if (!c->has(n2) || !c->has(ns) || c->has(std::string(blk) + ".sc_b")) continue;
            const Tensor& t2 = c->t(n2); const Tensor& ts = c->t(ns);
            if (t2.dims.size() != 3 || ts.dims.size() != 3 || ts.dim(0) != 1 || ts.dim(1) != t2.dim(1) || !c->packed.count(t2.dev) || !c->packed.count(ts.dev)) continue;
            const size_t bytes = (packed_weight_elems(t2.dim(0), t2.dim(1), t2.dim(2)) + packed_weight_elems(1, ts.dim(1), ts.dim(2))) * 2;
            void* comb = c->buf("weights_pair." + n2, bytes);
            launch_pack_pair(c->packed[t2.dev], t2.dim(0), t2.dim(2), c->packed[ts.dev], 1, ts.dim(2), t2.dim(1), comb, c->stream);
            c->pair_packed[t2.dev] = comb;
        }
    {
        std::vector<std::pair<std::string, Tensor>> add;
        for (auto& kv : c->tensors) {
            const std::string& nm = kv.first;
            if (nm.size() < 5 || nm.compare(nm.size() - 4, 4, ".wqk") != 0) continue;
            const std::string pre = nm.substr(0, nm.size() - 4);
            const Tensor& wqk = kv.second;
            if (!c->has(pre + ".wv") || !c->has(pre + ".bqk") || !c->has(pre + ".bv") || wqk.dtype != DT_F32 || wqk.dims.size() != 3) continue;
            const Tensor& wv = c->t(pre + ".wv");
            if (wv.dtype != DT_F32 || wv.dims.size() != 3 || wv.dim(2) != wqk.dim(2)) continue;
            Tensor w = wqk; w.dims = {1, wqk.dim(1) + wv.dim(1), wqk.dim(2)}; w.numel = wqk.numel + wv.numel; w.host = nullptr;
            w.dev = c->buf(pre + ".wqkv", w.numel * 4);
            HIPCHK(hipMemcpyAsync(w.dev, wqk.dev, wqk.numel * 4, hipMemcpyDeviceToDevice, c->stream));
            HIPCHK(hipMemcpyAsync((float*)w.dev + wqk.numel, wv.dev, wv.numel * 4, hipMemcpyDeviceToDevice, c->stream));
            const Tensor& bqk = c->t(pre + ".bqk"); const Tensor& bv = c->t(pre + ".bv");
            Tensor bb = bqk; bb.dims = {(int)(bqk.numel + bv.numel)}; bb.numel = bqk.numel + bv.numel; bb.host = nullptr;
            bb.dev = c->buf(pre + ".bqkv", bb.numel * 4);
            HIPCHK(hipMemcpyAsync(bb.dev, bqk.dev, bqk.numel * 4, hipMemcpyDeviceToDevice, c->stream));
            HIPCHK(hipMemcpyAsync((float*)bb.dev + bqk.numel, bv.dev, bv.numel * 4, hipMemcpyDeviceToDevice, c->stream));
            add.emplace_back(pre + ".wqkv", w); add.emplace_back(pre + ".bqkv", bb);
        }
        for (auto& kv : add) c->tensors[kv.first] = kv.second;
    }
    {
        std::vector<std::pair<std::string, Tensor>> add;
        for (auto& kv : c->tensors) {
            const std::string& nm = kv.first;
            const std::string sfx = ".wqk.h16";
            if (nm.size() <= sfx.size() || nm.compare(nm.size() - sfx.size(), sfx.size(), sfx) != 0) continue;
            const std::string pre = nm.substr(0, nm.size() - sfx.size());
            if (!c->has(pre + ".wv.h16") || !c->has(pre + ".bqk") || !c->has(pre + ".bv")) continue;
            const Tensor& wqk = kv.second; const Tensor& wv = c->t(pre + ".wv.h16");
            if (wqk.dims.size() != 3 || wv.dims.size() != 3 || wqk.dim(0) != 1 || wv.dim(0) != 1 || wv.dim(2) != wqk.dim(2) || wqk.dim(2) % 8) continue;
            Tensor w = wqk; w.dims = {1, wqk.dim(1) + wv.dim(1), wqk.dim(2)}; w.numel = wqk.numel + wv.numel; w.host = nullptr;
            w.dev = c->buf(pre + ".wqkv.h16", w.numel * 2);
            HIPCHK(hipMemcpyAsync(w.dev, wqk.dev, wqk.numel * 2, hipMemcpyDeviceToDevice, c->stream));
            HIPCHK(hipMemcpyAsync((char*)w.dev + wqk.numel * 2, wv.dev, wv.numel * 2, hipMemcpyDeviceToDevice, c->stream));
            void* pk = c->buf(pre + ".wqkv.h16.packed", packed_weight_elems(1, w.dim(1), w.dim(2)) * 2);
            launch_pack_weights(w.dev, 1, w.dim(1), w.dim(2), pk, c->stream);
            c->packed[w.dev] = pk;
            add.emplace_back(pre + ".wqkv.h16", w);
            if (!c->has(pre + ".bqkv")) {
                const Tensor& bqk = c->t(pre + ".bqk"); const Tensor& bv = c->t(pre + ".bv");
                Tensor bb = bqk; bb.dims = {(int)(bqk.numel + bv.numel)}; bb.numel = bqk.numel + bv.numel; bb.host = nullptr;
                bb.dev = c->buf(pre + ".bqkv", bb.numel * 4);
                HIPCHK(hipMemcpyAsync(bb.dev, bqk.dev, bqk.numel * 4, hipMemcpyDeviceToDevice, c->stream));
                HIPCHK(hipMemcpyAsync((float*)bb.dev + bqk.numel, bv.dev, bv.numel * 4, hipMemcpyDeviceToDevice, c->stream));
                add.emplace_back(pre + ".bqkv", bb);
            }
        }
        for (auto& kv : add) c->tensors[kv.first] = kv.second;
    }
    if (c->enc_split) build_split_weights(c, c->enc_split == 2);
    HIPCHK(hipStreamSynchronize(c->stream));
    DevBuf& st = c->bufs["weights_staging"];
    HIPCHK(hipFree(st.base)); st.base = nullptr; st.p = nullptr; st.cap = 0;
}

void read_config(zvx_ctx* c) {
    auto it = c->cfg.find("precision");
    if (it == c->cfg.end()) fail(ZVX_E_MANIFEST, "manifest: missing cfg 'precision'");
    if (it->second == "bf16") c->dt = DT_BF16; else if (it->second == "f32") c->dt = DT_F32;
    else fail(ZVX_E_MANIFEST, "manifest: unknown precision '%s'", it->second.c_str());
    c->enc_split = c->dt == DT_BF16 ? (c->cfg.count("enc_split") ? std::max(0, std::min(2, c->cfg_int("enc_split"))) : 2) : 0;
    c->H = c->cfg_int("hidden"); c->emb_dim = c->cfg_int("emb_dim"); c->punct_dim = c->cfg_int("punct_dim");
    c->n_phone_rows = c->cfg_int("n_phone_rows"); c->n_punct_rows = c->cfg_int("n_punct_rows");
    c->max_txt_len = c->cfg_int("max_txt_len"); c->max_mel_len = c->cfg_int("max_mel_len");
    c->enc_layers = c->cfg_int("enc_layers"); c->enc_heads = c->cfg_int("enc_heads"); c->ffn_dim = c->cfg_int("ffn_dim");
    auto fk = c->cfg_list("ffn_k"); if (fk.size() != 2) fail(ZVX_E_MANIFEST, "manifest: ffn_k needs 2 entries");
    c->ffn_k0 = fk[0]; c->ffn_k1 = fk[1];
    c->vp_dim = c->cfg_int("vp_dim"); c->vp_k = c->cfg_int("vp_k"); c->n_bins = c->cfg_int("n_bins");
    c->dec_layers = c->cfg_int("dec_layers"); c->dec_heads = c->cfg_int("dec_heads"); c->dec_scln = c->cfg_int("dec_scln");
    c->n_mels = c->cfg_int("n_mels"); c->hop = c->cfg_int("hop"); c->res_dim = c->cfg_int("res_dim");
    c->rn_layers = c->cfg_list("rn_layers"); c->rn_filters = c->cfg_list("rn_filters"); c->rn_asp = c->cfg_int("rn_asp");
    const std::string dk = c->cfg["dec_kind"];
    if (dk == "fastspeech2") c->dec_kind = 0; else if (dk == "styletts") c->dec_kind = 1;
    else fail(ZVX_E_MANIFEST, "unknown decoder kind: '%s'", dk.c_str());
    c->voc_resblock = c->cfg_int("voc_resblock"); c->voc_c0 = c->cfg_int("voc_c0");
    c->voc_rates = c->cfg_list("voc_rates"); c->voc_ksizes = c->cfg_list("voc_ksizes"); c->voc_rb_k = c->cfg_list("voc_rb_k");
    {
        std::stringstream ss(c->cfg["voc_rb_d"]); std::string grp;
        while (std::getline(ss, grp, ';')) {
            std::vector<int> v; std::stringstream gs(grp); std::string tok;
            while (std::getline(gs, tok, ',')) if (!tok.empty()) v.push_back(atoi(tok.c_str()));
            c->voc_rb_d.push_back(v);
        }
    }
    int prod = 1; for (int r : c->voc_rates) prod *= r;
    if (prod != c->hop) fail(ZVX_E_MANIFEST, "prod(voc_rates)=%d != hop=%d", prod, c->hop);
    if (c->voc_rb_d.size() != c->voc_rb_k.size()) fail(ZVX_E_MANIFEST, "voc_rb_d / voc_rb_k size mismatch");
    if (c->H % 8 || (c->H / c->enc_heads) % 8 || (c->H / c->dec_heads) % 8) fail(ZVX_E_UNSUPPORTED, "hidden/head dims must be multiples of 8");
}

struct FftWeights { std::string p; bool scln; const float* bg; long bg_bs; const float* post_add; };

void fft_block(zvx_ctx* c, void* x, int dt, int B, int Lmax, const int* len_dev, int nheads, const FftWeights& w, int Ls = 0, bool flat = false) {
    if (Ls <= 0) Ls = Lmax;
    const int H = c->H, d = H / nheads, Lp = (Lmax + 7) & ~7, F = c->ffn_dim;
    const size_t es = dtype_size(dt);
    const bool h16 = dt == DT_F16;
    auto wdev = [&](const char* n) { return c->t(w.p + n + (h16 ? ".h16" : "")).dev; };
    void* qk = c->buf("fft.qk", (size_t)B * Ls * 2 * H * es);
    void* vt = c->buf("fft.vt", (size_t)B * H * Lp * es);
    float* sc = c->fbuf("fft.scores", (size_t)B * nheads * Lmax * Lp);
    void* P = c->buf("fft.P", (size_t)B * nheads * Lmax * Lp * es);
    void* o = c->buf("fft.o", (size_t)B * Ls * H * es);
    float* y = c->fbuf("fft.y", (size_t)B * Ls * H);
    void* const yv = h16 ? c->buf("fft.y16", (size_t)B * Ls * H * 2) : (void*)y;
    const int ydt = h16 ? (int)DT_F16 : (int)DT_F32;
    void* hbuf = c->buf("fft.h", (size_t)B * Ls * F * es);

    const bool sp16 = c->enc_split == 2;
    const char* const s3 = sp16 ? ".s3h" : ".s3";
    const bool split = dt == DT_F32 && c->enc_split && c->has(w.p + ".wqk" + s3);
    void* xs = split ? c->buf("fft.xs", (size_t)B * Ls * 3 * H * 2) : nullptr;
    auto split_of = [&](const float* src, int C, void* dst) { launch_split3(src, C, dst, B, Ls, len_dev, C, c->stream, sp16); };
    auto as_split = [&](GemmArgs& a, const void* planes, int C, const std::string& wname) {
        const Tensor& ws = c->t(wname + s3);
        a.dtype = sp16 ? DT_F16 : DT_BF16; a.X = planes; a.x_bs = (long)Ls * 3 * C; a.ldx = 3 * C; a.K = 3 * C;
        a.alpha = ws.alpha;
        a.W = ws.dev; a.ldw = 3 * C; a.w_ts = (long)ws.dim(1) * 3 * C;
        a.flops = 2.0 * (double)a.M * a.nbatch * a.N * C * a.ntaps;
    };
    AttnF32Args af;
    memset(&af, 0, sizeof af);
    af.ld = 3 * H; af.bs = (long)Ls * 3 * H; af.q_off = 0; af.k_off = H; af.v_off = 2 * H;
    af.out = (float*)o; af.o_bs = (long)Ls * H; af.ldo = H; af.len = len_dev; af.L = Lmax; af.D = d; af.nheads = nheads; af.nbatch = B;
    af.scale = (float)(1.0 / pow((double)d, 0.5));
    const bool fused_f32 = dt == DT_F32 && c->use_attn_f32 && c->has(w.p + ".wqkv") && launch_attention_f32(af, c->stream, true);
    const bool xs_from_producer = split && c->fft_xs_ready == x;
    if (split && !xs_from_producer) split_of((const float*)x, H, xs);
    c->fft_xs_ready = nullptr;
    if (fused_f32) {
        float* qkv = c->fbuf("fft.qkv", (size_t)B * Ls * 3 * H);
        GemmArgs a = gemm_base(dt);
        a.X = x; a.x_bs = (long)Ls * H; a.ldx = H; a.W = c->t(w.p + ".wqkv").dev; a.ldw = H;
        a.M = Lmax; a.N = 3 * H; a.K = H; a.nbatch = B; a.in_len = len_dev; a.out_len = len_dev; if (flat) a.bflat = Ls;
        if (split) { as_split(a, xs, H, w.p + ".wqkv"); a.out_dtype = DT_F32; }
        a.bias = c->pf(w.p + ".bqkv"); a.bias_mode = 1;
        a.out = qkv; a.o_bs = (long)Ls * 3 * H; a.ldo = 3 * H;
        c->gemm(a);
        af.qkv = qkv;
        if (split) { af.planes = (unsigned short*)xs; af.planes_C = H; af.planes_f16 = sp16; }
        c->timed(4.0 * B * nheads * (double)Lmax * Lmax * d, (double)B * Lmax * 4.0 * H * 4, [&] { launch_attention_f32(af, c->stream, false); });
    } else {
    if (split) split_of((const float*)x, H, xs);
    void* qkvbuf = h16 ? c->buf("fft.qkv16", (size_t)B * Ls * 3 * H * es) : nullptr;
    if (h16) {
        GemmArgs a = gemm_base(dt);
        a.X = x; a.x_bs = (long)Ls * H; a.ldx = H; a.W = c->t(w.p + ".wqkv.h16").dev; a.ldw = H;
        a.M = Lmax; a.N = 3 * H; a.K = H; a.nbatch = B; a.in_len = len_dev; a.out_len = len_dev; if (flat) a.bflat = Ls;
        a.bias = c->pf(w.p + ".bqkv"); a.bias_mode = 1;
        a.out = qkvbuf; a.o_bs = (long)Ls * 3 * H; a.ldo = 3 * H;
        c->gemm(a);
        c->timed(0, (double)B * Lmax * H * 4.0, [&] { launch_transpose16((const char*)qkvbuf + (size_t)2 * H * es, 3 * H, vt, Lp, B, Ls, H, c->stream, len_dev); });
    } else {
    {
        GemmArgs a = gemm_base(dt);
        a.X = x; a.x_bs = (long)Ls * H; a.ldx = H; a.W = wdev(".wqk"); a.ldw = H;
        a.M = Lmax; a.N = 2 * H; a.K = H; a.nbatch = B; a.in_len = len_dev; a.out_len = len_dev; if (flat) a.bflat = Ls;
        if (split) { as_split(a, xs, H, w.p + ".wqk"); a.out_dtype = DT_F32; }
        a.bias = c->pf(w.p + ".bqk"); a.bias_mode = 1;
        a.out = qk; a.o_bs = (long)Ls * 2 * H; a.ldo = 2 * H;
        c->gemm(a);
    }
    {
        GemmArgs a = gemm_base(dt);
        a.X = c->t(w.p + ".wv").dev; a.x_bs = 0; a.ldx = H; a.W = x; a.w_bs = (long)Ls * H; a.ldw = H;
        a.M = H; a.N = Lmax; a.K = H; a.nbatch = B; a.in_len_static = H;
        a.bias = c->pf(w.p + ".bv"); a.bias_mode = 2;
        a.out = vt; a.o_bs = (long)H * Lp; a.ldo = Lp;
        if (Lp > Lmax) HIPCHK(hipMemset2DAsync((char*)vt + (size_t)Lmax * es, (size_t)Lp * es, 0, (size_t)(Lp - Lmax) * es, (size_t)B * H, c->stream));
        c->gemm(a);
        launch_zero_tail_cols(vt, (int)es, Lp, (long)H * Lp, B, H, Lmax, len_dev, c->stream);
    }
    }
    FlashArgs fa;
    memset(&fa, 0, sizeof fa);
    fa.qk = qk; fa.qk_bs = (long)Ls * 2 * H; fa.ldq = 2 * H; fa.k_off = H; fa.vt = vt;
    if (h16) { fa.qk = qkvbuf; fa.qk_bs = (long)Ls * 3 * H; fa.ldq = 3 * H; } fa.vt_bs = (long)H * Lp; fa.ldv = Lp;
    fa.out = o; fa.o_bs = (long)Ls * H; fa.ldo = H; fa.len = len_dev; fa.L = Lmax; fa.D = d; fa.nheads = nheads; fa.nbatch = B;
    fa.scale = (float)(1.0 / pow((double)d, 0.5));
    fa.f16 = h16;
    const bool flash = (dt == DT_BF16 || h16) && c->use_flash && launch_flash_attention(fa, c->stream, true);
    if (h16 && !flash) fail(ZVX_E_UNSUPPORTED, "half-precision FFT block without the fused attention (head depth %d)", d);
    if (flash) {
        c->timed(4.0 * B * nheads * (double)Lmax * Lmax * d, (double)B * Lmax * (3.0 * H + H) * es, [&] { launch_flash_attention(fa, c->stream, false); });
        c->sat_scan(o, dt, (long)Ls * H, H, B, Lmax, len_dev, H);
    } else {
    {
        GemmArgs a = gemm_base(dt);
        a.X = qk; a.x_bs = (long)Ls * 2 * H; a.x_hs = d; a.ldx = 2 * H;
        a.W = (const char*)qk + (size_t)H * es; a.w_bs = (long)Ls * 2 * H; a.w_hs = d; a.ldw = 2 * H;
        a.M = Lmax; a.N = Lmax; a.K = d; a.nbatch = B; a.nheads = nheads; a.in_len = len_dev; a.out_len = len_dev;
        a.alpha = (float)(1.0 / pow((double)d, 0.5));
        a.out = sc; a.out_dtype = DT_F32; a.o_bs = (long)nheads * Lmax * Lp; a.o_hs = (long)Lmax * Lp; a.ldo = Lp;
        a.flops = 2.0 * B * nheads * (double)Lmax * Lmax * d;
        c->gemm(a);
    }
    c->timed(0, (double)B * nheads * Lmax * Lp * (4.0 + es), [&] { launch_softmax_rows(sc, Lp, P, dt, Lp, B, nheads, Lmax, len_dev, c->stream); });
    {
        GemmArgs a = gemm_base(dt);
        a.X = P; a.x_bs = (long)nheads * Lmax * Lp; a.x_hs = (long)Lmax * Lp; a.ldx = Lp;
        a.W = vt; a.w_bs = (long)H * Lp; a.w_hs = (long)d * Lp; a.ldw = Lp;
        a.M = Lmax; a.N = d; a.K = Lp; a.k_len = len_dev; a.nbatch = B; a.nheads = nheads; a.in_len = len_dev; a.out_len = len_dev;
        a.out = o; a.o_bs = (long)Ls * H; a.o_hs = d; a.ldo = H;
        a.flops = 2.0 * B * nheads * (double)Lmax * Lmax * d;
        c->gemm(a);
    }
    }
    }
    {
        GemmArgs a = gemm_base(dt);
        a.X = o; a.x_bs = (long)Ls * H; a.ldx = H; a.W = wdev(".wo"); a.ldw = H;
        a.M = Lmax; a.N = H; a.K = H; a.nbatch = B; a.in_len = len_dev; a.out_len = len_dev; if (flat) a.bflat = Ls;
        a.bias = c->pf(w.p + ".bo"); a.bias_mode = 1;
        a.res = x; a.r_bs = (long)Ls * H; a.ldr = H; a.res_mode = 1; a.res_dtype = dt;
        a.out = yv; a.out_dtype = ydt; a.o_bs = (long)Ls * H; a.ldo = H;
        if (split) { if (!fused_f32) split_of((const float*)o, H, xs); as_split(a, xs, H, w.p + ".wo"); }
        c->gemm(a);
    }
    const double ln_bytes = (double)B * Lmax * H * ((h16 ? 2.0 : 4.0) + es);
    c->timed(0, ln_bytes, [&] {
        if (w.scln) launch_layernorm(yv, ydt, H, x, dt, H, B, Ls, len_dev, H, 1, 1e-8f, nullptr, nullptr, w.bg, w.bg_bs, nullptr, c->stream);
        else launch_layernorm(yv, ydt, H, x, dt, H, B, Ls, len_dev, H, 0, 1e-5f, c->pf(w.p + ".ln1_g"), c->pf(w.p + ".ln1_b"), nullptr, 0, nullptr, c->stream, split ? xs : nullptr, sp16);
    });
    c->sat_scan(x, dt, (long)Ls * H, H, B, Lmax, len_dev, H);
    {
        GemmArgs a = gemm_base(dt);
        a.X = x; a.x_bs = (long)Ls * H; a.ldx = H; a.W = wdev(".w1"); a.ldw = H; a.w_ts = (long)F * H;
        a.M = Lmax; a.N = F; a.K = H; a.nbatch = B; a.in_len = len_dev; a.out_len = len_dev; if (flat) a.bflat = Ls;
        set_taps_1d(a, c->ffn_k0, 1);
        a.bias = c->pf(w.p + ".b1"); a.bias_mode = 1; a.act = ACT_RELU;
        a.out = hbuf; a.o_bs = (long)Ls * F; a.ldo = F;
        void* hs = split ? c->buf("fft.hs", (size_t)B * Ls * 3 * F * 2) : nullptr;
        if (split) {
            if (w.scln) split_of((const float*)x, H, xs);
            as_split(a, xs, H, w.p + ".w1");
            a.out_dtype = DT_F32; a.out_split3 = sp16 ? 2 : 1; a.out = hs; a.o_bs = (long)Ls * 3 * F; a.ldo = 3 * F;
        }
        c->gemm(a);
    }
    {
        GemmArgs a = gemm_base(dt);
        a.X = hbuf; a.x_bs = (long)Ls * F; a.ldx = F; a.W = wdev(".w2"); a.ldw = F; a.w_ts = (long)H * F;
        a.M = Lmax; a.N = H; a.K = F; a.nbatch = B; a.in_len = len_dev; a.out_len = len_dev; if (flat) a.bflat = Ls;
        set_taps_1d(a, c->ffn_k1, 1);
        a.bias = c->pf(w.p + ".b2"); a.bias_mode = 1;
        a.res = x; a.r_bs = (long)Ls * H; a.ldr = H; a.res_mode = 1; a.res_dtype = dt;
        a.out = yv; a.out_dtype = ydt; a.o_bs = (long)Ls * H; a.ldo = H;
        if (split) as_split(a, c->buf("fft.hs", (size_t)B * Ls * 3 * F * 2), F, w.p + ".w2");
        c->gemm(a);
    }
    c->timed(0, ln_bytes, [&] {
        if (w.scln) launch_layernorm(yv, ydt, H, x, dt, H, B, Ls, len_dev, H, 1, 1e-8f, nullptr, nullptr, w.bg + 2 * H, w.bg_bs, w.post_add, c->stream);
        else launch_layernorm(yv, ydt, H, x, dt, H, B, Ls, len_dev, H, 0, 1e-5f, c->pf(w.p + ".ln2_g"), c->pf(w.p + ".ln2_b"), nullptr, 0, w.post_add, c->stream, split ? xs : nullptr, sp16);
    });
    c->sat_scan(x, dt, (long)Ls * H, H, B, Lmax, len_dev, H);
    if (split && !w.scln) c->fft_xs_ready = x;
}

void variance_predictor(zvx_ctx* c, const char* nm, const float* x, int B, int Tmax, const int* T_dev, float* pred, const char* bufsfx = "") {
    const int H = c->H, Fv = c->vp_dim;
    const std::string p = std::string("va.") + nm;
    float* h1 = c->fbuf(std::string("va.h1") + bufsfx, (size_t)B * Tmax * Fv);
    float* h2 = c->fbuf(std::string("va.h2") + bufsfx, (size_t)B * Tmax * Fv);
    {
        GemmArgs a = gemm_base(DT_F32);
        a.X = x; a.x_bs = (long)Tmax * H; a.ldx = H; a.W = c->t(p + ".c1").dev; a.ldw = H; a.w_ts = (long)Fv * H;
        a.M = Tmax; a.N = Fv; a.K = H; a.nbatch = B; a.in_len = T_dev; a.out_len = T_dev;
        set_taps_1d(a, c->vp_k, 1);
        a.bias = c->pf(p + ".b1"); a.bias_mode = 1; a.act = ACT_RELU;
        a.out = h1; a.o_bs = (long)Tmax * Fv; a.ldo = Fv;
        c->gemm(a);
    }
    launch_layernorm(h1, DT_F32, Fv, h1, DT_F32, Fv, B, Tmax, T_dev, Fv, 0, 1e-5f, c->pf(p + ".ln1_g"), c->pf(p + ".ln1_b"), nullptr, 0, nullptr, c->stream);
    {
        GemmArgs a = gemm_base(DT_F32);
        a.X = h1; a.x_bs = (long)Tmax * Fv; a.ldx = Fv; a.W = c->t(p + ".c2").dev; a.ldw = Fv; a.w_ts = (long)Fv * Fv;
        a.M = Tmax; a.N = Fv; a.K = Fv; a.nbatch = B; a.in_len = T_dev; a.out_len = T_dev;
        a.ntaps = c->vp_k;
        for (int k = 0; k < c->vp_k; k++) { a.du[k] = 0; a.dv[k] = (int)(k - 1); }
        a.bias = c->pf(p + ".b2"); a.bias_mode = 1; a.act = ACT_RELU;
        a.out = h2; a.o_bs = (long)Tmax * Fv; a.ldo = Fv;
        c->gemm(a);
    }
    launch_layernorm(h2, DT_F32, Fv, h2, DT_F32, Fv, B, Tmax, T_dev, Fv, 0, 1e-5f, c->pf(p + ".ln2_g"), c->pf(p + ".ln2_b"), nullptr, 0, nullptr, c->stream);
    launch_rowdot(h2, Fv, c->pf(p + ".lw"), c->t(p + ".lb").host[0], pred, B, Tmax, T_dev, Fv, c->stream);
}

void check_prosody(const zvx_prosody* p, const int32_t* T, int B, int Tmax) {
    const float* per_utt[4] = {p->pitch_shift, p->pitch_range, p->energy_shift, p->energy_range};
    const char* nm[4] = {"pitch_shift", "pitch_range", "energy_shift", "energy_range"};
    for (int i = 0; i < 4; i++)
        if (per_utt[i])
            for (int b = 0; b < B; b++) {
                const float v = per_utt[i][b];
                if (!std::isfinite(v)) fail(ZVX_E_INVALID, "prosody %s[%d] is not finite", nm[i], b);
                if ((i & 1) && (v < 0.f || v > 4.f)) fail(ZVX_E_INVALID, "prosody %s[%d]=%g outside [0, 4]", nm[i], b, v);
            }
    const float* tg[2] = {p->pitch_target, p->energy_target};
    for (int i = 0; i < 2; i++)
        if (tg[i])
            for (int b = 0; b < B; b++)
                for (int t = 0; t < T[b]; t++) {
                    const float v = tg[i][(size_t)b * Tmax + t];
                    if (v == v && !(v >= 0.f && v <= 1.f)) fail(ZVX_E_INVALID, "prosody %s_target[%d][%d]=%g is neither NaN nor in [0, 1]", i ? "energy" : "pitch", b, t, v);
                }
    if (p->dur_scale_q16)
        for (int b = 0; b < B; b++)
            for (int t = 0; t < T[b]; t++) {
                const int q = p->dur_scale_q16[(size_t)b * Tmax + t];
                if (q < 4096 || q > 1048576) fail(ZVX_E_INVALID, "prosody dur_scale_q16[%d][%d]=%d outside [4096, 1048576]", b, t, q);
            }
}

void run_encode(zvx_ctx* c, const int32_t* phoneme, const int32_t* puncts, const int32_t* duration, const int32_t* T,
                int B, int Tmax, const float* spk, int32_t* mel_len_out, int Lmax_cap, const zvx_prosody* pros = nullptr) {
    const int H = c->H;
    c->have_features = false; c->have_mel = false;
    if (c->stream != c->front_stream) c->front_dirty_main = true;
    if (B <= 0 || Tmax <= 0) fail(ZVX_E_INVALID, "B and Tmax must be positive");
    if (c->vp_k != 3) fail(ZVX_E_UNSUPPORTED, "vp_kernel_size != 3 changes the sequence length (fs2.py:543 padding=1)");
    c->T_host.assign(T, T + B);
    for (int b = 0; b < B; b++) {
        if (T[b] <= 0 || T[b] > Tmax) fail(ZVX_E_INVALID, "T[%d]=%d out of range (1..%d)", b, T[b], Tmax);
        for (int t = 0; t < T[b]; t++) {
            const int ph = phoneme[b * Tmax + t], pu = puncts[b * Tmax + t];
            if (ph < 0 || ph >= c->n_phone_rows) fail(ZVX_E_INVALID, "phoneme id %d out of range at [%d][%d]", ph, b, t);
            if (pu < 0 || pu >= c->n_punct_rows) fail(ZVX_E_INVALID, "punct id %d out of range at [%d][%d]", pu, b, t);
        }
    }
    if (pros) check_prosody(pros, T, B, Tmax);
    c->B = B; c->Tmax = Tmax; c->have_features = false; c->have_mel = false;
    const size_t nid = (size_t)B * Tmax;
    std::vector<std::string> planes = {"in.phoneme", "in.puncts", "in.duration", "in.T", "in.spk"};
    const void* pros_src[3] = {pros ? pros->pitch_target : nullptr, pros ? pros->energy_target : nullptr, pros ? pros->dur_scale_q16 : nullptr};
    int pros_plane[3] = {-1, -1, -1};
    if (pros) {
        planes.push_back("in.pros_utt");
        const char* nm[3] = {"in.pitch_target", "in.energy_target", "in.dur_scale"};
        for (int i = 0; i < 3; i++) if (pros_src[i]) { pros_plane[i] = (int)planes.size(); planes.push_back(nm[i]); }
    }
    const size_t np = planes.size();
    size_t in_stride = 0;
    char* in_base = c->carve("in.all", planes, std::max(std::max(nid, (size_t)B * 4), (size_t)B * H) * 4, &in_stride);
    c->in_stage.resize(in_stride * np / sizeof(int));
    {
        int* hs = c->in_stage.data();
        const size_t st = in_stride / sizeof(int);
        memcpy(hs, phoneme, nid * 4); memcpy(hs + st, puncts, nid * 4);
        if (duration) memcpy(hs + 2 * st, duration, nid * 4);
        memcpy(hs + 3 * st, T, (size_t)B * 4);
        memcpy(hs + 4 * st, spk, (size_t)B * H * 4);
        if (pros) {
            const float* per_utt[4] = {pros->pitch_shift, pros->pitch_range, pros->energy_shift, pros->energy_range};
            for (int i = 0; i < 4; i++) if (per_utt[i]) memcpy(hs + 5 * st + (size_t)i * B, per_utt[i], (size_t)B * 4);
            for (int i = 0; i < 3; i++) if (pros_src[i]) memcpy(hs + pros_plane[i] * st, pros_src[i], nid * 4);
        }
        c->upload(in_base, hs, in_stride * np);
    }
    int* ph_d = (int*)in_base; int* pu_d = (int*)(in_base + in_stride);
    int* dur_in = duration ? (int*)(in_base + 2 * in_stride) : nullptr;
    int* T_d = (int*)(in_base + 3 * in_stride);
    float* spk_d = (float*)(in_base + 4 * in_stride);
    const float* pros_utt = pros ? (const float*)(in_base + 5 * in_stride) : nullptr;
    const float* p_shift = (pros && pros->pitch_shift) ? pros_utt : nullptr;
    const float* p_range = (pros && pros->pitch_range) ? pros_utt + B : nullptr;
    const float* e_shift = (pros && pros->energy_shift) ? pros_utt + 2 * B : nullptr;
    const float* e_range = (pros && pros->energy_range) ? pros_utt + 3 * B : nullptr;
    const float* p_tgt = pros_src[0] ? (const float*)(in_base + pros_plane[0] * in_stride) : nullptr;
    const float* e_tgt = pros_src[1] ? (const float*)(in_base + pros_plane[1] * in_stride) : nullptr;
    const int* dq = pros_src[2] ? (const int*)(in_base + pros_plane[2] * in_stride) : nullptr;
    const bool pitch_ctl = p_shift || p_range || p_tgt, energy_ctl = e_shift || e_range || e_tgt;

    c->stage_begin(ZVX_T_ENCODER);
    c->tag = "encoder";
    const float* pe = c->pf("enc.pe");
    if (Tmax > c->t("enc.pe").dim(0)) {
        std::vector<float> tab((size_t)Tmax * H);
        for (int pos = 0; pos < Tmax; pos++)
            for (int j = 0; j < H; j++) {
                const double ang = pos / pow(10000.0, 2.0 * (j / 2) / H);
                tab[(size_t)pos * H + j] = (float)((j & 1) ? cos(ang) : sin(ang));
            }
        float* d = c->fbuf("enc.pe_ext", tab.size());
        HIPCHK(hipMemcpyAsync(d, tab.data(), tab.size() * 4, hipMemcpyHostToDevice, c->stream));
        HIPCHK(hipStreamSynchronize(c->stream));
        pe = d;
    }
    float* x = c->fbuf("enc.x", nid * H);
    launch_embed(ph_d, pu_d, c->pf("enc.emb"), c->emb_dim, c->pf("enc.pemb"), c->punct_dim, pe, x, B, Tmax, T_d, c->stream);
    c->fft_xs_ready = nullptr;
    for (int i = 0; i < c->enc_layers; i++) {
        FftWeights w{"enc." + std::to_string(i), false, nullptr, 0, (i == c->enc_layers - 1) ? spk_d : nullptr};
        fft_block(c, x, DT_F32, B, Tmax, T_d, c->enc_heads, w);
    }
    c->fft_xs_ready = nullptr;
    c->stage_end(ZVX_T_ENCODER);

    c->stage_begin(ZVX_T_VARIANCE);
    c->tag = "variance";
    HIPCHK(hipMemcpyAsync(c->fbuf("enc.out", nid * H), x, nid * H * 4, hipMemcpyDeviceToDevice, c->stream));
    size_t va_stride = 0;
// ... 1165 lines not shown
    need = rs ? (int)rs_out_len(need_native, rs_L, rs_M) : need_native;
    const bool host_async = flags & ZVX_HOST_ASYNC;
    if (!host_async && wav_stride < need) fail(ZVX_E_BUFFER, "wav_stride %lld < %d samples", (long long)wav_stride, need);
    const zvx_ctx::RsBank* bank = rs ? &rs_bank(c, rs_L, rs_M) : nullptr;
    c->stage_begin(ZVX_T_VOCODER);
    void* wdev; long wstride;
    const bool dev_out = (flags & ZVX_DEVICE_OUT) && !host_async;
    const int pcm16 = (flags & ZVX_PCM16) ? 1 : 0;
    const size_t ss = pcm16 ? 2 : 4;
    zvx_ctx::HostSlot* hs = nullptr;
    if (host_async) {
        const int slot = c->host_next; c->host_next ^= 1; c->host_last = slot;
        hs = &c->host_slot[slot];
        if (!c->copy_stream) { if (c->comm_stream) { c->copy_stream = c->comm_stream; c->copy_is_comm = true; } else HIPCHK(hipStreamCreateWithFlags(&c->copy_stream, hipStreamNonBlocking)); }
        if (!hs->ready) { HIPCHK(hipEventCreateWithFlags(&hs->ready, hipEventDisableTiming)); HIPCHK(hipEventCreateWithFlags(&hs->done, hipEventDisableTiming)); }
        if (hs->pending) { HIPCHK(hipEventSynchronize(hs->done)); hs->pending = false; }
        wstride = (std::max(need, 1) + 7) & ~7;
        const size_t bytes = (size_t)B * wstride * ss;
        if (bytes > hs->cap) {
            if (hs->p) { HIPCHK(hipHostFree(hs->p)); hs->p = nullptr; hs->cap = 0; }
            const size_t cap = bytes + bytes / 8 + 256;
            HIPCHK(hipHostMalloc(&hs->p, cap, hipHostMallocDefault));
            hs->cap = cap;
        }
        wdev = c->buf(slot ? "wav.async1" : "wav.async0", bytes);
        hs->B = B; hs->pcm16 = pcm16; hs->stride = wstride; hs->need = need;
    } else if (dev_out) {
        wdev = wav; wstride = wav_stride;
        auto f = c->gather_fence.find(wav);
        if (f != c->gather_fence.end()) HIPCHK(hipStreamWaitEvent(c->stream, f->second, 0));
    }
    else { wstride = (std::max(need, 1) + 7) & ~7; wdev = c->buf("wav", (size_t)B * wstride * ss); }
    if (rs) {
        const long nstride = (std::max(need_native, 1) + 7) & ~7;
        float* native = c->fbuf("wav.native", (size_t)B * nstride);
        run_vocoder(c, c->fbuf("mel", 0), c->n_mels, c->Lmax, c->mel_len_host.data(), P.data(), B, native, nstride, 0);
        c->stage_end(ZVX_T_VOCODER);
        double nin = 0, nout = 0;
        for (int b = 0; b < B; b++) { nin += (double)c->mel_len_host[b] * c->hop; nout += (double)rs_out_len((long)c->mel_len_host[b] * c->hop, rs_L, rs_M); }
        if (need > 0) run_resample(c, *bank, native, nstride, c->ibuf("voc.lens", 0), c->hop, B, wdev, wstride, pcm16, 0, 0, -1, need, nin, nout);
    } else {
        run_vocoder(c, c->fbuf("mel", 0), c->n_mels, c->Lmax, c->mel_len_host.data(), P.data(), B, wdev, wstride, pcm16);
        c->stage_end(ZVX_T_VOCODER);
    }
    if (host_async) {
        HIPCHK(hipEventRecord(hs->ready, c->stream));
        HIPCHK(hipStreamWaitEvent(c->copy_stream, hs->ready, 0));
        if (need > 0) HIPCHK(hipMemcpyAsync(hs->p, wdev, (size_t)B * wstride * ss, hipMemcpyDeviceToHost, c->copy_stream));
        HIPCHK(hipEventRecord(hs->done, c->copy_stream));
        hs->pending = true;
        return;
    }
    if (!dev_out && need > 0)
        HIPCHK(hipMemcpy2DAsync(wav, (size_t)wav_stride * ss, wdev, (size_t)wstride * ss, (size_t)need * ss, B, hipMemcpyDeviceToHost, c->stream));
    if (!(dev_out && (flags & ZVX_NO_SYNC))) c->sync();
}

template <typename F>
zvx_status guarded(zvx_ctx* ctx, F&& f) {
    if (!ctx) return ZVX_E_INVALID;
    try {
        HIPCHK(hipSetDevice(ctx->device));
        const bool outer = ctx->api_depth++ == 0;
        struct End { zvx_ctx* c; ~End() { try { if (--c->api_depth == 0) c->arena_end(); } catch (...) {} } } end{ctx};
        if (outer) ctx->arena_begin();
        f();
        return ZVX_OK;
    } catch (const ZvxError& e) {
        ctx->err = e.what();
        ctx->quiesce_side_streams();
        return e.code;
    } catch (const std::exception& e) {
        ctx->err = e.what();
        ctx->quiesce_side_streams();
        return ZVX_E_INVALID;
    }
}

}

extern "C" {

zvx_status zvx_create(const char* manifest, const void* weights, size_t nbytes, int device, zvx_ctx** out) {
    if (!out) return ZVX_E_INVALID;
    *out = nullptr;
    zvx_ctx* c = new zvx_ctx();
    try {
        int ndev = 0;
        hipError_t e = hipGetDeviceCount(&ndev);
        if (e != hipSuccess || ndev <= 0) fail(ZVX_E_HIP, "no HIP device available (%s)", hipGetErrorString(e));
        if (device < 0 || device >= ndev) fail(ZVX_E_INVALID, "device %d out of range (%d visible)", device, ndev);
        c->device = device;
        HIPCHK(hipSetDevice(device));
        HIPCHK(hipStreamCreate(&c->stream));
        c->main0 = c->stream;
        for (int s = 0; s < ZVX_T_COUNT; s++) { HIPCHK(hipEventCreate(&c->stage_ev[s][0])); HIPCHK(hipEventCreate(&c->stage_ev[s][1])); c->stage_used[s] = false; c->stage_ms[s] = 0.f; }
        parse_manifest(c, manifest, weights, nbytes);
        read_config(c);
        upload_weights(c);
        *out = c;
        return ZVX_OK;
    } catch (const ZvxError& e) {
        g_create_error = e.what();
        delete c;
        return e.code;
    } catch (const std::exception& e) {
        g_create_error = e.what();
        delete c;
        return ZVX_E_INVALID;
    }
}

void zvx_destroy(zvx_ctx* c) {
    if (!c) return;
    (void)hipSetDevice(c->device);
    if (c->front_stream) (void)hipStreamSynchronize(c->front_stream);
    if (c->stream) (void)hipStreamSynchronize(c->stream);
    zvx_comm_destroy(c);
    for (int i = 0; i < 2; i++) { if (c->arena[i].p) (void)hipHostFree(c->arena[i].p); if (c->arena[i].ev) (void)hipEventDestroy(c->arena[i].ev); }
    if (c->copy_stream && !c->copy_is_comm) { (void)hipStreamSynchronize(c->copy_stream); (void)hipStreamDestroy(c->copy_stream); }
    for (auto& hs : c->host_slot) { if (hs.p) (void)hipHostFree(hs.p); if (hs.ready) (void)hipEventDestroy(hs.ready); if (hs.done) (void)hipEventDestroy(hs.done); }
    if (c->join_host) (void)hipHostFree(c->join_host);
    for (int i = 0; i < 2; i++) if (c->voc_aux[i]) { (void)hipStreamSynchronize(c->voc_aux[i]); (void)hipStreamDestroy(c->voc_aux[i]); }
    for (int i = 0; i < 3; i++) if (c->voc_ev[i]) (void)hipEventDestroy(c->voc_ev[i]);
    if (c->aux_stream) { (void)hipStreamSynchronize(c->aux_stream); (void)hipStreamDestroy(c->aux_stream); (void)hipEventDestroy(c->ev_aux[0]); (void)hipEventDestroy(c->ev_aux[1]); }
    if (c->front_stream) {
        (void)hipStreamSynchronize(c->front_stream); (void)hipStreamDestroy(c->front_stream);
        (void)hipEventDestroy(c->ev_front_done); (void)hipEventDestroy(c->ev_mel_free); (void)hipEventDestroy(c->ev_main_join);
    }
    for (auto& kv : c->bufs) if (kv.second.base) (void)hipFree(kv.second.base);
    for (auto e : c->event_pool) (void)hipEventDestroy(e);
    if (c->stream) {
        for (int s = 0; s < ZVX_T_COUNT; s++) { (void)hipEventDestroy(c->stage_ev[s][0]); (void)hipEventDestroy(c->stage_ev[s][1]); }
        (void)hipStreamDestroy(c->stream);
    }
    delete c;
}

const char* zvx_last_error(const zvx_ctx* c) { return c ? c->err.c_str() : g_create_error.c_str(); }

namespace {

struct Switch { const char* key; int zvx_ctx::*v; bool (*ok)(int64_t); };
bool flag(int64_t v) { return v == 0 || v == 1; }
bool count(int64_t v) { return v >= 0 && v <= INT32_MAX; }
const Switch kSwitches[] = {
    {"profile", &zvx_ctx::profile, [](int64_t v) { return v >= 0 && v <= 2; }},
    {"profile_only", &zvx_ctx::profile_only, [](int64_t v) { return v >= -1 && v < gemm_num_variants(); }},
    {"shape_log", &zvx_ctx::shape_log, flag},
    {"rs_prof", &zvx_ctx::rs_prof, flag},
    {"f16_sat_check", &zvx_ctx::sat_check, flag},
    {"poison_pads", &zvx_ctx::poison_pads, flag},
    {"max_frames", &zvx_ctx::max_frames, [](int64_t v) { return v >= 1 && v <= (1 << 24); }},
    {"enc_split", &zvx_ctx::enc_split, [](int64_t v) { return v >= 0 && v <= 2; }},
    {"attn_f32", &zvx_ctx::use_attn_f32, flag},
    {"flash", &zvx_ctx::use_flash, flag},
    {"front_overlap", &zvx_ctx::front_overlap, [](int64_t v) { return v >= 0 && v <= 2; }},
    {"va_overlap_maxb", &zvx_ctx::va_overlap_maxb, count},
    {"dec_f16", &zvx_ctx::dec_f16, flag},
    {"dec_flat", &zvx_ctx::dec_flat, flag},
    {"dec_sc_fuse", &zvx_ctx::dec_sc_fuse, flag},
    {"norm_fuse_maxb", &zvx_ctx::norm_fuse_maxb, count},
    {"voc_f16", &zvx_ctx::voc_f16, flag},
    {"voc_f16_stages", &zvx_ctx::voc_f16_stages, [](int64_t v) { return v >= -1 && v <= INT32_MAX; }},
    {"voc_overlap_maxb", &zvx_ctx::voc_overlap_maxb, count},
    {"voc_overlap_frames", &zvx_ctx::voc_overlap_frames, count},
    {"stagefuse", &zvx_ctx::use_stagefuse, flag},
    {"rb2fuse", &zvx_ctx::use_rb2fuse, flag},
    {"resstream", &zvx_ctx::use_resstream, flag},
    {"rs_seg_min", &zvx_ctx::rs_seg_min, [](int64_t v) { return v >= -1 && v <= INT32_MAX; }},
    {"pairstream", &zvx_ctx::use_pairstream, [](int64_t v) { return v == -1 || v == 0 || v == 1 || v == 3; }},
    {"slab_small", &zvx_ctx::slab_small, [](int64_t v) { return (v & ~32) >= 0 && (v & ~32) <= 2; }},
    {"slab_flat", &zvx_ctx::slab_flat, flag},
    {"spk_pool_fuse", &zvx_ctx::spk_pool_fuse, flag},
    {"spk_s2_fuse", &zvx_ctx::spk_s2_fuse, flag},
    {"out_rate", &zvx_ctx::out_rate, count},
};
const Switch* find_switch(const char* key) {
    for (const Switch& s : kSwitches) if (!strcmp(s.key, key)) return &s;
    return nullptr;
}

}

int64_t zvx_get_int(const zvx_ctx* c, const char* key) {
    if (!c || !key) return -1;
    if (const Switch* s = find_switch(key)) return c->*s->v;
    const std::string k(key);
    if (k == "precision") return c->dt == DT_F32 ? 1 : 0;
    if (k == "hidden") return c->H;
    if (k == "n_mels") return c->n_mels;
    if (k == "hop") return c->hop;
    if (k == "device") return c->device;
    if (k == "dec_kind") return c->dec_kind;
    if (k == "Lmax") return c->Lmax;
    if (k == "f16_sat_events") {
        zvx_ctx* m = const_cast<zvx_ctx*>(c);
        unsigned long long n = 0;
        if (hipSetDevice(m->device) != hipSuccess) return -1;
        try { unsigned long long* d = m->sat_count_dev(); m->sync(); if (hipMemcpy(&n, d, sizeof n, hipMemcpyDeviceToHost) != hipSuccess) return -1; } catch (...) { return -1; }
        return (int64_t)n;
    }
    if (k == "host_slot") return c->host_last;
    if (k.rfind("variant_id:", 0) == 0) { for (int i = 0; i < gemm_num_variants(); i++) if (k.substr(11) == gemm_variant_name(i)) return i; return -1; }
    auto it = c->cfg.find(k);
    if (it != c->cfg.end()) return atoll(it->second.c_str());
    return -1;
}

zvx_status zvx_set_int(zvx_ctx* c, const char* key, int64_t value) {
    return guarded(c, [&] {
        if (!key) fail(ZVX_E_INVALID, "key is NULL");
        const Switch* s = find_switch(key);
        if (!s) fail(ZVX_E_INVALID, "unknown option '%s'", key);
        if (!s->ok(value)) fail(ZVX_E_INVALID, "option '%s' does not take the value %lld", key, (long long)value);
        const std::string k(key);
        if (k == "out_rate" && value) {
            int L = 1, M = 1;
            rs_pair(model_rate(c), (int)value, &L, &M);
            if ((int)value != model_rate(c)) rs_bank(c, L, M);
        }
        if (k == "profile" || k == "profile_only" || k == "f16_sat_check" || k == "front_overlap") c->sync();
        c->*s->v = (int)value;
        if (k == "f16_sat_check") HIPCHK(hipMemsetAsync(c->sat_count_dev(), 0, 64, c->stream));
        if (k == "front_overlap") c->front_dirty_main = true;
        if (k == "enc_split") {
            if (c->dt != DT_BF16) c->enc_split = 0;
            if (c->enc_split) { c->sync(); build_split_weights(c, c->enc_split == 2); }
        }
    });
}

zvx_status zvx_spkemb(zvx_ctx* c, const float* ref_mels, const int32_t* lens, int B, int Tmax, float* out) {
    return guarded(c, [&] {
        if (!ref_mels || !lens || !out || B <= 0 || Tmax <= 0) fail(ZVX_E_INVALID, "zvx_spkemb: bad arguments");
        run_spkemb(c, ref_mels, lens, B, Tmax, out, 0);
    });
}

zvx_status zvx_spkemb_ex(zvx_ctx* c, const float* ref_mels, const int32_t* lens, int B, int Tmax, float* out, int flags) {
    return guarded(c, [&] {
        if (!ref_mels || !lens || !out || B <= 0 || Tmax <= 0) fail(ZVX_E_INVALID, "zvx_spkemb_ex: bad arguments");
        run_spkemb(c, ref_mels, lens, B, Tmax, out, flags);
    });
}

zvx_status zvx_melspec(zvx_ctx* c, const float* wav, const int32_t* nsamples, int B, int Nmax, float* mel, int Tmax, int32_t* frames) {
    return guarded(c, [&] {
        if (!wav || !nsamples || B <= 0 || Nmax <= 0 || Tmax <= 0) fail(ZVX_E_INVALID, "zvx_melspec: bad arguments");
        run_melspec(c, wav, nsamples, B, Nmax, mel, Tmax, frames);
    });
}

zvx_status zvx_encode(zvx_ctx* c, const int32_t* phoneme, const int32_t* puncts, const int32_t* duration, const int32_t* T,
                      int B, int Tmax, const float* spk, int32_t* mel_len, float* log_duration, float* pitch, float* energy) {
    return zvx_encode_ex(c, phoneme, puncts, duration, T, B, Tmax, spk, mel_len, log_duration, pitch, energy, nullptr);
}

zvx_status zvx_encode_ex(zvx_ctx* c, const int32_t* phoneme, const int32_t* puncts, const int32_t* duration, const int32_t* T,
                         int B, int Tmax, const float* spk, int32_t* mel_len, float* log_duration, float* pitch, float* energy,
                         const zvx_prosody* prosody) {
    return guarded(c, [&] {
        if (!phoneme || !puncts || !T || !spk) fail(ZVX_E_INVALID, "zvx_encode: NULL input");
        run_encode(c, phoneme, puncts, duration, T, B, Tmax, spk, mel_len, 0, prosody);
        const size_t nid = (size_t)B * Tmax;
        if (log_duration) HIPCHK(hipMemcpyAsync(log_duration, c->fbuf("va.logd", nid), nid * 4, hipMemcpyDeviceToHost, c->stream));
        if (pitch) HIPCHK(hipMemcpyAsync(pitch, c->fbuf("va.pitch", nid), nid * 4, hipMemcpyDeviceToHost, c->stream));
        if (energy) HIPCHK(hipMemcpyAsync(energy, c->fbuf("va.energy", nid), nid * 4, hipMemcpyDeviceToHost, c->stream));
        c->sync();
    });
}

zvx_status zvx_decode(zvx_ctx* c, float* mel_out, int Lstride, int flags) {
    return guarded(c, [&] {
        if (!c->have_features) fail(ZVX_E_STATE, "zvx_decode: no features in the context (call zvx_encode first)");
        const int B = c->B;
        int* L_d = c->upload_ints("dec.L", c->mel_len_host.data(), B);
        run_decode(c, c->fbuf("features", 0), c->fbuf("in.spk", 0), L_d, B, c->Lmax);
        if (mel_out && c->Lmax > 0) copy_out_rows(c, c->fbuf("mel", 0), c->Lmax, c->n_mels, mel_out, Lstride, B, flags & ZVX_DEVICE_OUT);
        c->sync();
    });
}

zvx_status zvx_decode_features(zvx_ctx* c, const float* features, const int32_t* L, int B, int Lmax, const float* spk,
                               float* mel_out, int Lstride) {
    return guarded(c, [&] {
        if (!features || !L || !spk || B <= 0 || Lmax <= 0) fail(ZVX_E_INVALID, "zvx_decode_features: bad arguments");
        for (int b = 0; b < B; b++) if (L[b] < 2 || L[b] > Lmax) fail(ZVX_E_INVALID, "L[%d]=%d out of range (2..%d)", b, L[b], Lmax);
        c->B = B; c->Lmax = Lmax; c->mel_len_host.assign(L, L + B); c->Tmax = 0;
        c->have_features = false; c->have_mel = false;
        float* f = c->fbuf("features", (size_t)B * Lmax * c->H);
        HIPCHK(hipMemcpyAsync(f, features, (size_t)B * Lmax * c->H * 4, hipMemcpyHostToDevice, c->stream));
        float* spk_d = c->fbuf("in.spk", (size_t)B * c->H);
        HIPCHK(hipMemcpyAsync(spk_d, spk, (size_t)B * c->H * 4, hipMemcpyHostToDevice, c->stream));
        int* L_d = c->upload_ints("dec.L", L, B);
        c->have_features = true;
        run_decode(c, f, spk_d, L_d, B, Lmax);
        if (mel_out) copy_out_rows(c, c->fbuf("mel", 0), Lmax, c->n_mels, mel_out, Lstride, B, false);
        c->sync();
    });
}

zvx_status zvx_vocode(zvx_ctx* c, const int32_t* pad_to, void* wav, int64_t wav_stride, int flags) {
    return guarded(c, [&] {
        if (!wav && !(flags & ZVX_HOST_ASYNC)) fail(ZVX_E_INVALID, "zvx_vocode: wav is NULL");
        do_vocode(c, pad_to, wav, wav_stride, flags);
    });
}

zvx_status zvx_vocode_mel(zvx_ctx* c, const float* mel, const int32_t* P, int B, int Pmax, void* wav, int64_t wav_stride, int flags) {
    return guarded(c, [&] {
        if (!mel || !P || (!wav && !(flags & ZVX_HOST_ASYNC)) || B <= 0 || Pmax <= 0) fail(ZVX_E_INVALID, "zvx_vocode_mel: bad arguments");
        for (int b = 0; b < B; b++) if (P[b] < 1 || P[b] > Pmax) fail(ZVX_E_INVALID, "P[%d]=%d out of range (1..%d)", b, P[b], Pmax);
        c->B = B; c->Lmax = Pmax; c->Tmax = 0; c->mel_len_host.assign(P, P + B);
        c->have_features = false; c->have_mel = false;
        float* m = c->fbuf("mel", (size_t)B * Pmax * c->n_mels);
        HIPCHK(hipMemcpyAsync(m, mel, (size_t)B * Pmax * c->n_mels * 4, (flags & ZVX_DEVICE_IN) ? hipMemcpyDeviceToDevice : hipMemcpyHostToDevice, c->stream));
        c->have_mel = true;
        do_vocode(c, nullptr, wav, wav_stride, flags);
    });
}

zvx_status zvx_resample(zvx_ctx* c, const float* in, const int32_t* nsamples, int B, int Nmax, int rate_in, int rate_out, void* out,
                        int64_t out_stride, int32_t* out_len, int flags) {
    return guarded(c, [&] { do_resample(c, in, nsamples, B, Nmax, rate_in, rate_out, out, out_stride, out_len, flags, 0, 0, -1); });
}

zvx_status zvx_resample_ex(zvx_ctx* c, const float* in, const int32_t* nsamples, int B, int Nmax, int rate_in, int rate_out, void* out,
                           int64_t out_stride, int32_t* out_len, int flags, int64_t in_origin, int64_t out_begin, int64_t out_count) {
    return guarded(c, [&] { do_resample(c, in, nsamples, B, Nmax, rate_in, rate_out, out, out_stride, out_len, flags, in_origin, out_begin, out_count); });
}

zvx_status zvx_trim_bounds(zvx_ctx* c, const float* in, const int32_t* nsamples, int B, int Nmax, const zvx_join_params* params, int32_t* begin,
                           int32_t* end, int flags) {
    return guarded(c, [&] { do_trim_bounds(c, in, nsamples, B, Nmax, params, begin, end, flags); });
}

zvx_status zvx_join(zvx_ctx* c, const float* in, const int32_t* nsamples, int B, int Nmax, const int32_t* gap, const zvx_join_params* params,
                    void* out, int64_t out_capacity, int64_t* out_len, int64_t* seg_pos, int32_t* seg_begin, int32_t* seg_len, int flags) {
    return guarded(c, [&] { do_join(c, in, nsamples, B, Nmax, gap, params, out, out_capacity, out_len, seg_pos, seg_begin, seg_len, flags); });
}

zvx_status zvx_loudness(zvx_ctx* c, const float* in, const int32_t* nsamples, int B, int Nmax, int rate, double* lufs, float* peak, int flags) {
    return guarded(c, [&] { do_loudness(c, "zvx_loudness", in, nsamples, B, Nmax, rate, nullptr, nullptr, 0, lufs, peak, nullptr, flags); });
}

zvx_status zvx_normalize(zvx_ctx* c, const float* in, const int32_t* nsamples, int B, int Nmax, int rate, const zvx_loudness_params* params,
                         void* out, int64_t out_stride, double* lufs, float* peak, float* gain, int flags) {
    return guarded(c, [&] {
        if (!params) fail(ZVX_E_INVALID, "zvx_normalize: params is NULL");
        do_loudness(c, "zvx_normalize", in, nsamples, B, Nmax, rate, params, out, out_stride, lufs, peak, gain, flags);
    });
}

zvx_status zvx_synthesize(zvx_ctx* c, const int32_t* phoneme, const int32_t* puncts, const int32_t* duration, const int32_t* T,
                          int B, int Tmax, const float* spk, const int32_t* pad_to, int Lmax_cap, void* wav, int64_t wav_stride,
                          int32_t* mel_len, float* mel_out, int Lstride, float* log_duration, int flags) {
    return zvx_synthesize_ex(c, phoneme, puncts, duration, T, B, Tmax, spk, pad_to, Lmax_cap, wav, wav_stride, mel_len, mel_out, Lstride,
                             log_duration, flags, nullptr);
}

zvx_status zvx_synthesize_ex(zvx_ctx* c, const int32_t* phoneme, const int32_t* puncts, const int32_t* duration, const int32_t* T,
                             int B, int Tmax, const float* spk, const int32_t* pad_to, int Lmax_cap, void* wav, int64_t wav_stride,
                             int32_t* mel_len, float* mel_out, int Lstride, float* log_duration, int flags, const zvx_prosody* prosody) {
    return guarded(c, [&] {
        const bool host_async = flags & ZVX_HOST_ASYNC;
        if (!phoneme || !puncts || !T || !spk || (!wav && !host_async)) fail(ZVX_E_INVALID, "zvx_synthesize: NULL input");
        if (host_async && ((mel_out && !(flags & ZVX_DEVICE_OUT)) || log_duration)) fail(ZVX_E_INVALID, "zvx_synthesize: ZVX_HOST_ASYNC takes no host mel / log_duration output (they would make the call wait)");
        auto front_end = [&] {
            run_encode(c, phoneme, puncts, duration, T, B, Tmax, spk, mel_len, Lmax_cap, prosody);
            if (log_duration) HIPCHK(hipMemcpyAsync(log_duration, c->fbuf("va.logd", 0), (size_t)B * Tmax * 4, hipMemcpyDeviceToHost, c->stream));
            int* L_d = c->upload_ints("dec.L", c->mel_len_host.data(), B);
            run_decode(c, c->fbuf("features", 0), c->fbuf("in.spk", 0), L_d, B, c->Lmax);
            if (mel_out && c->Lmax > 0) copy_out_rows(c, c->fbuf("mel", 0), c->Lmax, c->n_mels, mel_out, Lstride, B, flags & ZVX_DEVICE_OUT);
        };
        if (c->front_overlap == 2 || (c->front_overlap == 1 && (host_async || ((flags & ZVX_NO_SYNC) && (flags & ZVX_DEVICE_OUT))))) {
            c->front_setup();
            hipStream_t const main_stream = c->stream;
            if (c->front_dirty_main) {
                HIPCHK(hipEventRecord(c->ev_main_join, main_stream));
                HIPCHK(hipStreamWaitEvent(c->front_stream, c->ev_main_join, 0));
// ... 291 lines not shown
```

### zerovox_amd/csrc/zvx_kernels.h

```cpp
#pragma once
#include <hip/hip_runtime.h>
#include <hip/hip_ext.h>
#include <stdint.h>
#include <atomic>
#include <mutex>
#include <set>
#include <utility>

extern thread_local hipEvent_t zvx_gemm_ev_start, zvx_gemm_ev_stop;
#define ZVX_DISPATCH(kernel, grid, block, lds, stream, ...) \
    do { if (zvx_gemm_ev_start) hipExtLaunchKernelGGL(kernel, grid, block, lds, stream, zvx_gemm_ev_start, zvx_gemm_ev_stop, 0, __VA_ARGS__); \
         else hipLaunchKernelGGL(kernel, grid, block, lds, stream, __VA_ARGS__); } while (0)

namespace zvx {

inline void profile_events(hipEvent_t start, hipEvent_t stop) { zvx_gemm_ev_start = start; zvx_gemm_ev_stop = stop; }

typedef unsigned short bf16_t;

enum DType { DT_F32 = 0, DT_BF16 = 1, DT_F16 = 2 };
static inline size_t dtype_size(int dt) { return dt == DT_F32 ? 4 : 2; }
inline int num_cus() {
    static const int n = [] { int dev = 0, v = 0; if (hipGetDevice(&dev) != hipSuccess || hipDeviceGetAttribute(&v, hipDeviceAttributeMultiprocessorCount, dev) != hipSuccess || v <= 0) v = 256; return v; }();
    return n;
}
inline int persistent_cus() { return num_cus(); }

inline bool lds_opt_in(const void* kfn) {
    static std::mutex mu;
    static std::set<std::pair<const void*, int>> done;
    int dev = 0;
    if (hipGetDevice(&dev) != hipSuccess) return false;
    std::lock_guard<std::mutex> lk(mu);
    if (done.count({kfn, dev})) return true;
    if (hipFuncSetAttribute(kfn, hipFuncAttributeMaxDynamicSharedMemorySize, 160 * 1024) != hipSuccess) return false;
    done.insert({kfn, dev});
    return true;
}

enum Act { ACT_NONE = 0, ACT_RELU = 1, ACT_LRELU = 2, ACT_TANH = 3 };

#define ZVX_MAX_TAPS 16

struct GemmArgs {
    const void* X; long x_bs, x_hs; int ldx;
    const void* W; long w_bs, w_hs, w_ts; int ldw;
    const void* Wp;
    int halo_l, halo_r;
    const void* Wp2; const float* bias1; int dv1[ZVX_MAX_TAPS]; int fused; float slope1;
    int no_pairstream;
    int dtype;
    int M, N, K;
    int nbatch, nheads;
    const int* in_len;
    const int* out_len;
    const int* k_len;
    int in_len_static;
    int ntaps; int du[ZVX_MAX_TAPS], dv[ZVX_MAX_TAPS];
    int stride, wout, hin, win;
    int flat_win, flat_rows;
    int bflat;
    const void* X2; long x2_bs; int ldx2, K2;
    int xcd_flat;
    int slab_small;
    int out_split3;
    float alpha;
    const float* bias; int bias_mode;
    const void* res; long r_bs, r_hs; int ldr; int res_dtype; int res_mode;
    float res_inv_slope;
    void* accum; long a_bs; int lda; int accum_mode;
    int accum_dtype;
    float out_scale;
    int act; float slope;
    const float* post_scale; const float* post_shift;
    void* out; long o_bs, o_hs; int ldo; int out_dtype;
    float* se_part; int* se_part_S;
    void* ds_out; const void* ds_Wp; const float* ds_bias;
    double flops;
};

int launch_gemm(const GemmArgs& a, hipStream_t stream);
int gemm_variant_of(const GemmArgs& a);
int gemm_epi_mode_of(const GemmArgs& a);
int launch_resfuse(GemmArgs a, hipStream_t stream);
int launch_rb2fuse(GemmArgs a, hipStream_t stream);
size_t packed_weight_elems(int ntaps, int N, int K);
void launch_pack_pair(const void* packedA, int ntapsA, int KA, const void* packedB, int ntapsB, int KB, int N, void* out, hipStream_t s);
void launch_pack_weights(const void* w_bf16, int ntaps, int N, int K, void* out, hipStream_t s);
const char* gemm_variant_name(int id);
int gemm_num_variants();

struct StreamArgs {
    const void* X; long x_bs; int ldx;
    const void* W1[3]; const void* W2[3];
    const float* b1[3]; const float* b2[3];
    int dil[3];
    int C, ntaps, npair;
    void* out; long o_bs; int ldo;
    void* accum; long a_bs; int lda; int accum_mode;
    float slope1, res_inv_slope, out_scale, slope;
    const int* len; int M, nbatch;
    int S, nseg;
    int dX0, dT, dX[3];
    double flops;
    long long* prof;
    int seg_min;
    int f16;
};
int launch_resstream(StreamArgs a, hipStream_t stream, bool dry_run);

struct PairArgs {
    const void* X; long x_bs; int ldx;
    const void* W1; const void* W2;
    const float* b1; const float* b2;
    int C, ntaps, dil;
    void* out; long o_bs; int ldo;
    void* accum; long a_bs; int lda; int accum_mode;
    float slope1, res_inv_slope, out_scale, slope;
    const int* len; int M, nbatch;
    int force;
    int f16;
    int S, nseg, DX, DT, G0;
    long long* prof;
};
bool launch_pairstream(PairArgs a, hipStream_t stream, bool dry_run);

struct StageArgs {
    const void* X; long x_bs; int ldx;
    const void* W;
    int woff[18];
    const float* bias;
    int C, nk, ks[3], dil[3][3];
    void* out; long o_bs; int ldo;
    float slope1, res_inv_slope, slope;
    const int* len; int M, nbatch;
    int f16;
};
bool launch_narrowstage(const StageArgs& a, hipStream_t stream, bool dry_run);
int narrowstage_steps(int C, int k);
void launch_pack_narrow(const void* w16 , int k, int C, void* out, hipStream_t s);

struct FlashArgs {
    const void* qk; long qk_bs; int ldq; int k_off;
    const void* vt; long vt_bs; int ldv;
    void* out; long o_bs; int ldo;
    const int* len; int L, D, nheads, nbatch;
    float scale;
    int f16;
    long long* prof;
};
bool launch_flash_attention(const FlashArgs& a, hipStream_t stream, bool dry_run);
struct AttnF32Args {
    const float* qkv; long bs; int ld; int q_off, k_off, v_off;
    float* out; long o_bs; int ldo;
    unsigned short* planes; int planes_C;
    int planes_f16;
    const int* len; int L, D, nheads, nbatch;
    float scale;
};
bool launch_attention_f32(const AttnF32Args& a, hipStream_t stream, bool dry_run);

void launch_instnorm_fused(const void* x, int x_dt, int ldx, void* y, int y_dt, int ldy, int B, int Lmax, const int* L, int C, float eps,
                           float* mean, float* rstd, const float* gamma, const float* beta, long g_bs, int one_plus, int act, float slope, hipStream_t s);
void launch_transpose16(const void* in, int ld_in, void* out, int ld_out, int B, int rows, int C, hipStream_t s, const int* len = nullptr);
void launch_f32_to_bf16(const float* in, bf16_t* out, size_t n, hipStream_t s);
void launch_zero_tail_cols(void* x, int es, long ld, long bs, int B, int rows, int cols, const int* len, hipStream_t s);
void launch_cast(const void* in, int in_dt, void* out, int out_dt, size_t n, hipStream_t s);

void launch_split3(const float* x, int ldx, void* out, int B, int rows_max, const int* rows, int C, hipStream_t s, int f16 = 0);
void launch_split3_weights(const float* w, void* out, long nrows, int K, hipStream_t s, int f16 = 0, float scale = 1.f);
void launch_absmax(const float* x, size_t n, float* out , hipStream_t s);

void launch_embed(const int* phoneme, const int* puncts, const float* emb, int emb_dim, const float* pemb,
                  int pemb_dim, const float* pe, float* out, int B, int Tmax, const int* T, hipStream_t s);

void launch_layernorm(const void* x, int x_dt, int ldx, void* y, int y_dt, int ldy, int B, int rows_max,
                      const int* rows, int C, int mode, float eps, const float* gamma, const float* beta,
                      const float* bg, long bg_bs, const float* post_add, hipStream_t s, void* split_planes = nullptr, int planes_f16 = 0);

void launch_softmax_rows(const float* scores, int lds, void* P, int p_dt, int ldp, int nbatch, int nheads,
                         int Lmax, const int* len, hipStream_t s);

void launch_rowdot(const float* x, int ldx, const float* w, float bias, float* out, int B, int Tmax,
                   const int* T, int C, hipStream_t s);

void launch_bucket_embed_add(const float* pred, const float* table, int nbins, float* x, int ldx, int C,
                             int* idx_out, int B, int Tmax, const int* T, hipStream_t s);

void launch_durations(const int* forced, const float* logd, int* dur, int* cum, int* mel_len, int B, int Tmax,
                      const int* T, hipStream_t s);

void launch_bucket_embed_add_ctl(const float* pred, const float* shift, const float* range, const float* target, const float* table,
                                 int nbins, float* x, int ldx, int C, int* idx_out, int B, int Tmax, const int* T, hipStream_t s);
void launch_durations_q16(const int* forced, const float* logd, const int* q, int* dur, int* cum, int* mel_len, int B, int Tmax,
                          const int* T, hipStream_t s);

void launch_length_regulate(const float* x, int ldx, const int* cum, const int* T, const int* mel_len,
                            float* feats, int B, int Tmax, int Lmax, int C, hipStream_t s);
void launch_add_pe_cast(const float* x, const float* pe, void* y, int y_dt, int ldy, int B, int Lmax,
                        const int* L, int C, hipStream_t s, int out_rows_max = 0);

void launch_instnorm_stats(const void* x, int x_dt, int ldx, int B, int Lmax, const int* L, int C, float eps,
                           float* mean, float* rstd, hipStream_t s);
void launch_norm_affine_act(const void* x, int x_dt, int ldx, void* y, int y_dt, int ldy, int B, int Lmax,
                            const int* L, int C, const float* mean, const float* rstd, const float* gamma,
                            const float* beta, long g_bs, int one_plus, int act, float slope, hipStream_t s);

void launch_mel_pad(const void* mel, int m_dt, int ldm, int Lmax, const int* mel_len, void* v, int v_dt,
                    int ldv, int Pmax, const int* P, int B, int nm, hipStream_t s);
void launch_copy_rows_f32(const void* src, int s_dt, int lds, long s_bs, float* dst, long ldd, long d_bs,
                          int B, int rows_max, const int* rows, int C, hipStream_t s);

void launch_conv_post_tanh(const void* x, int x_dt, int ldx, long x_bs, const float* w , float bias,
                           int ktaps, int C, void* wav, long wav_bs, int pcm16, int B, int Nmax, const int* in_len,
                           int len_mul, const int* out_len, int out_mul, hipStream_t s);
struct ResampleArgs {
    const float* x; long x_bs; const int* in_len; int in_mul;
    void* out; long out_bs; int pcm16;
    int B, L, M, half, T, pitch;
    const float* bank;
    long in_origin, out_begin, out_count, out_max;
};
bool launch_resample_poly(const ResampleArgs& a, hipStream_t s);
struct JoinBoundsArgs {
    const float* x; long x_bs; const int* nsamples; int B;
    int frame, hop, tiled;
    double* unit; long upitch;
    double k, floor;
    int trim, keep;
    int* bounds;
};
void launch_join_powers(const JoinBoundsArgs& a, long units_max, hipStream_t s);
void launch_join_bounds(const JoinBoundsArgs& a, hipStream_t s);
void launch_join_layout(const int* bounds, const int* gap, int B, long* pos, int* seg_begin, int* seg_len, hipStream_t s);
struct JoinCopyArgs {
    const float* x; long x_bs; int B;
    const long* pos; const int* seg_begin; const int* seg_len;
    void* out; long cap; int pcm16, fade;
};
void launch_join_copy(const JoinCopyArgs& a, long upper, hipStream_t s);
struct LoudCoef { double b0, b1, b2, a1, a2, c1, c2; };
struct LoudArgs {
    const float* x; long x_bs; const int* nsamples; int B;
    int h;
    LoudCoef k;
    double* unit; long upitch;
    float* part_peak; int ppitch;
    double abs_gate;
    double* row_sum; long* row_cnt;
    double* lufs; float* peak; float* gain;
    double target; double max_gain_db; double ceiling;
    int want_gain;
};
void launch_loud_units(const LoudArgs& a, long units_max, hipStream_t s);
void launch_loud_gates(const LoudArgs& a, hipStream_t s);
void launch_loud_common(const LoudArgs& a, hipStream_t s);
struct LoudApplyArgs {
    const float* x; long x_bs; const int* nsamples; int B;
    const float* gain; void* out; long out_bs; int pcm16;
};
void launch_loud_apply(const LoudApplyArgs& a, long n_max, hipStream_t s);
void launch_count_sat16(const void* x, long bs, int ld, int B, int rows_max, const int* rows, int C, unsigned long long* count, hipStream_t s);
void launch_zero_tail_rows(float* x, int ldx, int B, int rows_max, const int* rows, int C, hipStream_t s);

void launch_spk_front(const float* mels, int Tmax, const int* lens, int F, const float* mean, const float* rstd,
                      const float* w , const float* bias, const float* bn_scale, const float* bn_shift,
                      int C0, void* out, int o_dt, int B, int Wout, hipStream_t s);
int se_pool_splits(int H, int Wmax);
void launch_se_pool(const void* x, int x_dt, int B, int H, int Wmax, const int* W, int C, float* partial, hipStream_t s);
void launch_se_fc(const float* partial, int S, int H, const int* W, const float* w1, const float* b1, const float* w2, const float* b2, int C,
                  int Cr, float* scale, int B, hipStream_t s, const float* pool_bias = nullptr);
void launch_se_apply(const void* x, const void* res, void* y, int dt, const float* scale, int B, int H, int Wmax,
                     const int* W, int C, hipStream_t s);
void launch_asp_pool(const void* x, int x_dt, const float* logits, int B, int F, int Wmax, const int* W, int C,
                     float* out, int with_std, hipStream_t s);
void launch_l2norm_rows(float* x, int B, int C, hipStream_t s);

void launch_reflect_pad(const float* wav, long w_bs, const int* n, float* out, long o_bs, int pad, int B, int out_cols, hipStream_t s);
void launch_stft_mag(const float* spec, int lds_, float* mag, int ldm, int nf, int B, int Tmax, const int* frames, hipStream_t s);
void launch_log_clip(float* x, int ldx, int C, float lo, int B, int Tmax, const int* frames, hipStream_t s);

void launch_fc_rows(const float* x, int ldx, const float* w, int ldw, const float* bias, float* out, int ldo, int B, int N, int K, hipStream_t s);

}
```

Measured before the change: 348.5 million.

## Add two-plane f16 split GEMM path for encoder convolutions

Adds a new default encoder split mode where activations are stored as two f16 planes (hi, scaled lo) instead of three, and weights are split into hi/lo planes. A dedicated conv-slab kernel computes the three cross products (wh*xh, wl*xh, scaled wh*xl) directly with MFMA, so the duplicated hi plane is no longer written or read. Attention output, split kernels and the FFN epilogue now emit the two-plane layout. This cuts activation bandwidth and the K dimension of the emulated-f32 GEMMs, but adds a new hand-scheduled kernel with its own accuracy and correctness risk.

```diff
diff --git a/zerovox_amd/csrc/attention.hip b/zerovox_amd/csrc/attention.hip
--- a/zerovox_amd/csrc/attention.hip
+++ b/zerovox_amd/csrc/attention.hip
@@ -454,8 +454,13 @@
                         hi = __builtin_bit_cast(unsigned short, (__bf16)val);
                         lo = __builtin_bit_cast(unsigned short, (__bf16)(val - __uint_as_float((unsigned)hi << 16)));
                     }
-                    unsigned short* const pp = a.planes + ((long)b * a.L + q) * 3 * a.planes_C + h * D + col;
-                    pp[0] = hi; pp[a.planes_C] = hi; pp[2 * a.planes_C] = lo;
+                    if (a.planes_f16 == 2) {
+                        unsigned short* const pp = a.planes + ((long)b * a.L + q) * 2 * a.planes_C + h * D + col;
+                        pp[0] = hi; pp[a.planes_C] = lo;
+                    } else {
+                        unsigned short* const pp = a.planes + ((long)b * a.L + q) * 3 * a.planes_C + h * D + col;
+                        pp[0] = hi; pp[a.planes_C] = hi; pp[2 * a.planes_C] = lo;
+                    }
                 }
             }
         }
diff --git a/zerovox_amd/csrc/gemm.hip b/zerovox_amd/csrc/gemm.hip
--- a/zerovox_amd/csrc/gemm.hip
+++ b/zerovox_amd/csrc/gemm.hip
@@ -770,6 +770,220 @@
         epilogue_direct<TM, TN, F16>(a, acc, b, m0 + wr * (BM / WM), n0 + wc * (BN / WN), out_len, lane, slab + wave * (32 * (TN * 64 + 16)));
     else
         epilogue_rows<TM, TN, 0, EPI, (F16 && EPI >= 0)>(a, acc, b, m0 + wr * (BM / WM), n0 + wc * (BN / WN), out_len, lane, slab + wave * (32 * (TN * 32 * 4 + 16)));
+}
+
+template <int TM, int TN, int EPI>
+__device__ __forceinline__ void epilogue_split2(const GemmArgs& a, f32x16 (&acc)[TN][TM], int b, int row_base, int col_base, int out_len, int lane,
+                                                unsigned char* stage ) {
+    constexpr int NW = TN * 32, EP = NW * 4 + 16, LPR = NW / 8, RPP = 64 / LPR, NP = 32 / RPP;
+    const long ooff = (long)b * a.o_bs, roff = (long)b * a.r_bs;
+    const int c8 = lane % LPR, n = col_base + c8 * 8;
+    const bool nok = n < a.N;
+    const float alpha = a.alpha;
+    f32x2 bcol[4];
+#pragma unroll
+    for (int e = 0; e < 4; e++) bcol[e] = (f32x2){0.f, 0.f};
+    if (nok) {
+        const float4 b0 = *(const float4*)(a.bias + n), b1 = *(const float4*)(a.bias + n + 4);
+        bcol[0] = (f32x2){b0.x, b0.y}; bcol[1] = (f32x2){b0.z, b0.w}; bcol[2] = (f32x2){b1.x, b1.y}; bcol[3] = (f32x2){b1.z, b1.w};
+    }
+#pragma unroll
+    for (int j = 0; j < TM; j++) {
+#pragma unroll
+        for (int i = 0; i < TN; i++)
+#pragma unroll
+            for (int g = 0; g < 4; g++)
+                *(float4*)(stage + (lane & 31) * EP + (i * 32 + 8 * g + 4 * (lane >> 5)) * 4) =
+                    make_float4(acc[i][j][4 * g], acc[i][j][4 * g + 1], acc[i][j][4 * g + 2], acc[i][j][4 * g + 3]);
+#pragma unroll
+        for (int p = 0; p < NP; p++) {
+            const int rl = p * RPP + lane / LPR, r = row_base + j * 32 + rl;
+            const bool ok = r < a.M && r < out_len && nok;
+            const float4 v0 = *(const float4*)(stage + rl * EP + c8 * 32), v1 = *(const float4*)(stage + rl * EP + c8 * 32 + 16);
+            f32x2 t[4] = {(f32x2){v0.x, v0.y}, (f32x2){v0.z, v0.w}, (f32x2){v1.x, v1.y}, (f32x2){v1.z, v1.w}};
+#pragma unroll
+            for (int e = 0; e < 4; e++) t[e] = t[e] * alpha + bcol[e];
+            if (!ok) continue;
+            if (EPI == 1) {
+                const float* rp = (const float*)a.res + roff + (long)r * a.ldr + n;
+                const float4 t0 = *(const float4*)rp, t1 = *(const float4*)(rp + 4);
+                t[0] += (f32x2){t0.x, t0.y}; t[1] += (f32x2){t0.z, t0.w}; t[2] += (f32x2){t1.x, t1.y}; t[3] += (f32x2){t1.z, t1.w};
+            }
+            if (EPI == 2) {
+                unsigned short* op = (unsigned short*)a.out + ooff + (long)r * a.ldo + n;
+                u32x4 hv, lv;
+#pragma unroll
+                for (int e = 0; e < 4; e++) {
+                    const f32x2 v = (f32x2){fmaxf(t[e].x, 0.f), fmaxf(t[e].y, 0.f)};
+                    const unsigned hp = pack_f16x2_sat(v.x, v.y);
+                    const f32x2 rem = (v - unpack_f16x2(hp)) * 2048.f;
+                    hv[e] = hp; lv[e] = pack_f16x2_sat(rem.x, rem.y);
+                }
+                *(u32x4*)op = hv; *(u32x4*)(op + a.N) = lv;
+            } else {
+                float* op = (float*)a.out + ooff + (long)r * a.ldo + n;
+                *(float4*)op = make_float4(t[0].x, t[0].y, t[1].x, t[1].y);
+                *(float4*)(op + 4) = make_float4(t[2].x, t[2].y, t[3].x, t[3].y);
+            }
+        }
+    }
+}
+
+template <int BM, int BN, int WM, int WN, bool FULLK, int MINW, int EPI>
+__global__ __launch_bounds__(256, MINW) void convslab_split2_kernel(const GemmArgs a) {
+    constexpr int TM = BM / WM / 32, TN = BN / WN / 32, MAXH = 64;
+    constexpr int NIT = ((BM + MAXH) * 8 + 255) / 256;
+    static_assert(WM * WN == 4, "4 waves");
+    extern __shared__ __attribute__((aligned(16))) unsigned char slab[];
+
+    const int tid = threadIdx.x, lane = tid & 63, wave = __builtin_amdgcn_readfirstlane(tid >> 6);
+    const int wr = wave % WM, wc = wave / WM;
+    const int ntn = (a.N + BN - 1) / BN;
+    int wg, b;
+    if (a.xcd_flat) {
+        const int nx = gridDim.x, nwg = nx * gridDim.y, id = blockIdx.y * nx + blockIdx.x, q = nwg >> 3, r = nwg & 7, xcd = id & 7;
+        const int w = (xcd < r ? xcd * (q + 1) : r * (q + 1) + (xcd - r) * q) + (id >> 3);
+        b = w / nx; wg = w - b * nx;
+    } else {
+        const int nwg = gridDim.x, id = blockIdx.x, q = nwg >> 3, r = nwg & 7, xcd = id & 7;
+        wg = (xcd < r ? xcd * (q + 1) : r * (q + 1) + (xcd - r) * q) + (id >> 3);
+        b = blockIdx.y;
+    }
+    const int nt = wg % ntn, mt = wg / ntn;
+    const int m0 = mt * BM, n0 = nt * BN;
+    const int out_len = a.out_len ? a.out_len[b] : a.M;
+    const int in_len = a.in_len ? a.in_len[b] : a.in_len_static;
+    if (m0 >= out_len || m0 >= a.M) return;
+
+    const int HL = a.halo_l, SR = BM + a.halo_l + a.halo_r;
+    const int nkc = (a.K + SLAB_KC - 1) / SLAB_KC, n16 = a.K >> 4, ntaps = a.ntaps;
+    const unsigned short* Xp = (const unsigned short*)a.X + (long)b * a.x_bs;
+    const unsigned slab_lo = (unsigned)SR * SLAB_PITCH;
+
+    f32x16 acc[TN][TM];
+#pragma unroll
+    for (int i = 0; i < TN; i++)
+#pragma unroll
+        for (int j = 0; j < TM; j++)
+#pragma unroll
+            for (int e = 0; e < 16; e++) acc[i][j][e] = 0.f;
+
+    constexpr int WD = 4, WAITN = (WD - 1) * 2 * TN;
+    const int nt32_total = (a.N + 31) >> 5;
+    const int stotal = nkc * ntaps * 4;
+    const int xrow0 = HL + wr * (BM / WM) + (lane & 31);
+    const int koff = (lane >> 5) * 16;
+    const unsigned lds_base = (unsigned)(size_t)(__attribute__((address_space(3))) unsigned char*)slab;
+    const int dvreg = a.dv[lane & (ZVX_MAX_TAPS - 1)];
+    const unsigned char* wq[TN];
+#pragma unroll
+    for (int i = 0; i < TN; i++) {
+        const int t32 = (n0 >> 5) + wc * TN + i;
+        wq[i] = (const unsigned char*)a.Wp + (long)(t32 < nt32_total ? t32 : 0) * stotal * 2048;
+    }
+    const bool wave_dead = __builtin_amdgcn_readfirstlane((int)(n0 + wc * TN * 32 >= a.N || m0 + wr * (BM / WM) >= out_len)) != 0;
+    const unsigned lane16 = lane * 16;
+    u32x4 wreg[WD][2][TN] = {};
+    auto wload = [&](int s, int slot) {
+        const int sc = s < stotal ? s : stotal - 1;
+        const long off = ((long)(sc >> 2) * 8 + (sc & 3)) * 1024;
+#pragma unroll
+        for (int i = 0; i < TN; i++) {
+            asm volatile("global_load_dwordx4 %0, %1, %2" : "+v"(wreg[slot][0][i]) : "v"(lane16), "s"(wq[i] + off) : "memory");
+            asm volatile("global_load_dwordx4 %0, %1, %2" : "+v"(wreg[slot][1][i]) : "v"(lane16), "s"(wq[i] + off + 4096) : "memory");
+        }
+    };
+    wload(0, 0); wload(1, 1); wload(2, 2); wload(3, 3);
+
+    for (int kc = 0; kc < nkc; kc++) {
+        const int kbase = kc * SLAB_KC;
+        {
+            uint4 sv[2][NIT];
+#pragma unroll
+            for (int pl = 0; pl < 2; pl++)
+#pragma unroll
+                for (int it = 0; it < NIT; it++) {
+                    const int c = tid + it * 256;
+                    const int row = c >> 3, q = c & 7;
+                    const int g = m0 - HL + row, k = kbase + q * 8;
+                    sv[pl][it] = make_uint4(0, 0, 0, 0);
+                    if (c < SR * 8 && g >= 0 && g < in_len && k < a.K) sv[pl][it] = *(const uint4*)(Xp + (long)g * a.ldx + pl * a.K + k);
+                }
+            if (kc) __syncthreads();
+#pragma unroll
+            for (int pl = 0; pl < 2; pl++)
+#pragma unroll
+                for (int it = 0; it < NIT; it++) {
+                    const int c = tid + it * 256;
+                    if (c < SR * 8) *(uint4*)(slab + pl * slab_lo + (c >> 3) * SLAB_PITCH + (c & 7) * 16) = sv[pl][it];
+                }
+        }
+        __syncthreads();
+        int nk16 = 4;
+        if (!FULLK) { nk16 = n16 - kc * 4; if (nk16 > 4) nk16 = 4; }
+        if (wave_dead) nk16 = 0;
+
+        uint4 hA[TM], lA[TM], hB[TM], lB[TM];
+        auto rd = [&](uint4 (&hf)[TM], uint4 (&lf)[TM], unsigned rowoff, int kk) {
+#pragma unroll
+            for (int j = 0; j < TM; j++) {
+                asm volatile("ds_read_b128 %0, %1" : "=v"(hf[j]) : "v"(lds_base + rowoff + j * 32 * SLAB_PITCH + kk * 32));
+                asm volatile("ds_read_b128 %0, %1" : "=v"(lf[j]) : "v"(lds_base + slab_lo + rowoff + j * 32 * SLAB_PITCH + kk * 32));
+            }
+        };
+        auto mma = [&](uint4 (&hf)[TM], uint4 (&lf)[TM], int slot) {
+            f16x8 wh[TN], wl[TN], ws[TN];
+#pragma unroll
+            for (int i = 0; i < TN; i++) {
+                wh[i] = __builtin_bit_cast(f16x8, wreg[slot][0][i]); wl[i] = __builtin_bit_cast(f16x8, wreg[slot][1][i]);
+                ws[i] = wh[i] * (_Float16)0.00048828125f;
+            }
+#pragma unroll
+            for (int i = 0; i < TN; i++)
+#pragma unroll
+                for (int j = 0; j < TM; j++) acc[i][j] = __builtin_amdgcn_mfma_f32_32x32x16_f16(wh[i], __builtin_bit_cast(f16x8, hf[j]), acc[i][j], 0, 0, 0);
+#pragma unroll
+            for (int i = 0; i < TN; i++)
+#pragma unroll
+                for (int j = 0; j < TM; j++) acc[i][j] = __builtin_amdgcn_mfma_f32_32x32x16_f16(wl[i], __builtin_bit_cast(f16x8, hf[j]), acc[i][j], 0, 0, 0);
+#pragma unroll
+            for (int i = 0; i < TN; i++)
+#pragma unroll
+                for (int j = 0; j < TM; j++) acc[i][j] = __builtin_amdgcn_mfma_f32_32x32x16_f16(ws[i], __builtin_bit_cast(f16x8, lf[j]), acc[i][j], 0, 0, 0);
+        };
+        auto rowoff_of = [&](int tap) {
+            const int d = __builtin_amdgcn_readlane(dvreg, tap < ntaps ? tap : ntaps - 1);
+            return (unsigned)((xrow0 + d) * SLAB_PITCH + koff);
+        };
+        unsigned rowoff = rowoff_of(0);
+        const int s0 = kc * ntaps * 4;
+        rd(hA, lA, rowoff, 0);
+        for (int tap = 0; tap < ntaps; tap++) {
+            const unsigned rowoff_next = rowoff_of(tap + 1);
+#pragma unroll
+            for (int kk = 0; kk < 4; kk++) {
+                const int s = s0 + tap * 4 + kk;
+                asm volatile("s_waitcnt vmcnt(%0)" :: "n"(WAITN) : "memory");
+                if (kk & 1) rd(hA, lA, kk == 3 ? rowoff_next : rowoff, (kk + 1) & 3);
+                else        rd(hB, lB, rowoff, kk + 1);
+                asm volatile("s_waitcnt lgkmcnt(%0)" :: "n"(2 * TM) : "memory");
+                __builtin_amdgcn_sched_barrier(0);
+                if (kk < nk16) { if (kk & 1) mma(hB, lB, kk); else mma(hA, lA, kk); }
+                __builtin_amdgcn_sched_barrier(0);
+                wload(s + WD, kk);
+            }
+            rowoff = rowoff_next;
+        }
+        asm volatile("s_waitcnt lgkmcnt(0)" ::: "memory");
+    }
+#pragma unroll
+    for (int sl = 0; sl < WD; sl++)
+#pragma unroll
+        for (int pl = 0; pl < 2; pl++)
+#pragma unroll
+            for (int i = 0; i < TN; i++) asm volatile("s_waitcnt vmcnt(0)" : "+v"(wreg[sl][pl][i]) :: "memory");
+    __syncthreads();
+    epilogue_split2<TM, TN, EPI>(a, acc, b, m0 + wr * (BM / WM), n0 + wc * (BN / WN), out_len, lane, slab + wave * (32 * (TN * 32 * 4 + 16)));
 }
 
 template <int C, int NT, int BM, int WM, int WN, int MINW, int MAXH = 64, bool F16 = false>
@@ -1948,8 +2162,46 @@
 }
 
 
+template <int EPI>
+static void launch_split2_variant(const GemmArgs& a, bool n32, dim3 grid, size_t lds, hipStream_t stream) {
+    const bool fullk = a.K % SLAB_KC == 0;
+    if (n32) {
+        if (fullk) ZVX_LAUNCH((convslab_split2_kernel<128, 32, 4, 1, true, 2, EPI>), grid, dim3(256), lds, stream, a);
+        else ZVX_LAUNCH((convslab_split2_kernel<128, 32, 4, 1, false, 2, EPI>), grid, dim3(256), lds, stream, a);
+        return;
+    }
+    if (fullk) ZVX_LAUNCH((convslab_split2_kernel<64, 128, 2, 2, true, 2, EPI>), grid, dim3(256), lds, stream, a);
+    else ZVX_LAUNCH((convslab_split2_kernel<64, 128, 2, 2, false, 2, EPI>), grid, dim3(256), lds, stream, a);
+}
+static int launch_convslab_split2(GemmArgs a, hipStream_t stream) {
+    if (!a.Wp || a.dtype != DT_F16 || a.K % 16 || a.N % 8 || a.ldx % 8 || a.ldx < 2 * a.K || a.K2 || a.flat_win || a.wout > 0 || a.nheads != 1 || a.w_bs || a.k_len) return -2;
+    if (a.bias_mode != 1 || !a.bias || !a.out || a.out_dtype != DT_F32 || a.accum_mode || a.post_scale || a.out_scale != 1.f || a.ldo % 8) return -2;
+    int epi;
+    if (a.out_split3 == 3 && a.act == ACT_RELU && !a.res_mode && a.ldo >= 2 * a.N) epi = 2;
+    else if (!a.out_split3 && a.act == ACT_NONE && a.res_mode == 1 && a.res && a.res_dtype == DT_F32 && a.ldr % 4 == 0) epi = 1;
+    else if (!a.out_split3 && a.act == ACT_NONE && !a.res_mode) epi = 0;
+    else return -2;
+    int hl = 0, hr = 0;
+    for (int i = 0; i < a.ntaps; i++) { hl = a.dv[i] < -hl ? -a.dv[i] : hl; hr = a.dv[i] > hr ? a.dv[i] : hr; }
+    if (hl + hr > 64) return -4;
+    a.halo_l = hl; a.halo_r = hr; a.bflat = 0;
+    const bool n32 = (a.slab_small & 7) >= 2 && a.M <= 64 && a.nbatch * ((a.N + 127) / 128) * 4 <= num_cus() && a.N >= 64;
+    const int bm = n32 ? 128 : 64;
+    dim3 grid(n32 ? (a.N + 31) / 32 : ((a.N + 127) / 128) * ((a.M + 63) / 64), a.nbatch);
+    size_t lds = (size_t)2 * (bm + hl + hr) * SLAB_PITCH;
+    const size_t stage = (size_t)4 * 32 * (2 * 128 + 16);
+    if (lds < stage) lds = stage;
+    switch (epi) {
+        case 0: launch_split2_variant<0>(a, n32, grid, lds, stream); break;
+        case 1: launch_split2_variant<1>(a, n32, grid, lds, stream); break;
+        default: launch_split2_variant<2>(a, n32, grid, lds, stream);
+    }
+    return n32 ? 9 : 22;
+}
+
 int launch_gemm(const GemmArgs& a, hipStream_t stream) {
     if (a.N <= 0 || a.M <= 0 || a.nbatch <= 0) return -1;
+    if (a.fused == 3) return (a.ntaps < 1 || a.ntaps > ZVX_MAX_TAPS) ? -2 : launch_convslab_split2(a, stream);
     if (a.ds_out) return launch_conv2d_s2(a, stream) ? 28 : -7;
     if (a.stride == 2 && a.wout > 0 && a.ntaps == 9 && a.K == 64 && a.Wp && launch_conv2d_s2(a, stream)) return 29;
     if (a.ntaps < 1 || a.ntaps > ZVX_MAX_TAPS) return -2;
@@ -2019,7 +2271,7 @@
 
 int gemm_variant_of(const GemmArgs& a) {
     g_dry_run = true;
-    const int id = a.fused == 2 ? launch_rb2fuse(a, nullptr) : (a.fused ? launch_resfuse(a, nullptr) : launch_gemm(a, nullptr));
+    const int id = a.fused == 2 ? launch_rb2fuse(a, nullptr) : (a.fused == 1 ? launch_resfuse(a, nullptr) : launch_gemm(a, nullptr));
     g_dry_run = false;
     return id;
 }
diff --git a/zerovox_amd/csrc/ops.hip b/zerovox_amd/csrc/ops.hip
--- a/zerovox_amd/csrc/ops.hip
+++ b/zerovox_amd/csrc/ops.hip
@@ -106,14 +106,16 @@
     const int b = blockIdx.y, r = blockIdx.x;
     const bool live = r < (rows ? rows[b] : rows_max);
     const float* xr = x + ((long)b * rows_max + r) * ldx;
-    unsigned short* o = out + ((long)b * rows_max + r) * 3 * C;
+    const int np = f16 == 2 ? 2 : 3;
+    unsigned short* o = out + ((long)b * rows_max + r) * np * C;
     for (int c = threadIdx.x * 4; c < C; c += blockDim.x * 4) {
         unsigned short h[4], l[4];
         if (live) { const float4 v = *(const float4*)(xr + c); split2x(v.x, f16, h[0], l[0]); split2x(v.y, f16, h[1], l[1]); split2x(v.z, f16, h[2], l[2]); split2x(v.w, f16, h[3], l[3]); }
         else { for (int e = 0; e < 4; e++) h[e] = l[e] = 0; }
         const uint2 hv = make_uint2(h[0] | ((unsigned)h[1] << 16), h[2] | ((unsigned)h[3] << 16));
         const uint2 lv = make_uint2(l[0] | ((unsigned)l[1] << 16), l[2] | ((unsigned)l[3] << 16));
-        *(uint2*)(o + c) = hv; *(uint2*)(o + C + c) = hv; *(uint2*)(o + 2 * C + c) = lv;
+        if (np == 2) { *(uint2*)(o + c) = hv; *(uint2*)(o + C + c) = lv; }
+        else { *(uint2*)(o + c) = hv; *(uint2*)(o + C + c) = hv; *(uint2*)(o + 2 * C + c) = lv; }
     }
 }
 void launch_split3(const float* x, int ldx, void* out, int B, int rows_max, const int* rows, int C, hipStream_t s, int f16) {
@@ -138,6 +140,22 @@
 void launch_split3_weights(const float* w, void* out, long nrows, int K, hipStream_t s, int f16, float scale) {
     hipLaunchKernelGGL(k_split3_w, dim3((unsigned)nrows), dim3(256), 0, s, w, (unsigned short*)out, nrows, K, f16, scale);
 }
+__global__ void k_split2_w(const float* w, unsigned short* out, int ntaps, int N, int K, float scale) {
+    const long r = blockIdx.x;
+    if (r >= (long)ntaps * N) return;
+    const long tap = r / N, n = r - tap * N;
+    unsigned short* oh = out + ((2 * tap) * N + n) * K;
+    unsigned short* ol = out + ((2 * tap + 1) * N + n) * K;
+    for (int k = threadIdx.x; k < K; k += blockDim.x) {
+        const float v = w[r * K + k] * scale;
+        const _Float16 wh = (_Float16)clamp_h(v);
+        oh[k] = __builtin_bit_cast(unsigned short, wh);
+        ol[k] = __builtin_bit_cast(unsigned short, (_Float16)(v - (float)wh));
+    }
+}
+void launch_split2_weights(const float* w, void* out, int ntaps, int N, int K, hipStream_t s, float scale) {
+    hipLaunchKernelGGL(k_split2_w, dim3((unsigned)((long)ntaps * N)), dim3(256), 0, s, w, (unsigned short*)out, ntaps, N, K, scale);
+}
 __global__ void k_absmax(const float* x, size_t n, unsigned* out) {
     float m = 0.f;
     for (size_t i = (size_t)blockIdx.x * blockDim.x + threadIdx.x; i < n; i += (size_t)gridDim.x * blockDim.x) m = fmaxf(m, fabsf(x[i]));
@@ -176,7 +194,8 @@
     const int lane = threadIdx.x & 63;
     const int nr = rows ? rows[b] : rows_max;
     if (r >= nr) {
-        if (planes && r < rows_max) { unsigned short* o = planes + ((long)b * rows_max + r) * 3 * C; for (int c = lane; c < 3 * C; c += 64) o[c] = 0; }
+        const int np = planes_f16 == 2 ? 2 : 3;
+        if (planes && r < rows_max) { unsigned short* o = planes + ((long)b * rows_max + r) * np * C; for (int c = lane; c < np * C; c += 64) o[c] = 0; }
         return;
     }
     const long xo = ((long)b * rows_max + r) * ldx, yo = ((long)b * rows_max + r) * ldy;
@@ -230,8 +249,13 @@
                 for (int e = 0; e < 8; e++) split2x(o[e], planes_f16, hh[e], ll[e]);
                 const uint4 hv = make_uint4(hh[0] | ((unsigned)hh[1] << 16), hh[2] | ((unsigned)hh[3] << 16), hh[4] | ((unsigned)hh[5] << 16), hh[6] | ((unsigned)hh[7] << 16));
                 const uint4 lv = make_uint4(ll[0] | ((unsigned)ll[1] << 16), ll[2] | ((unsigned)ll[3] << 16), ll[4] | ((unsigned)ll[5] << 16), ll[6] | ((unsigned)ll[7] << 16));
-                unsigned short* po = planes + ((long)b * rows_max + r) * 3 * C + c;
-                *(uint4*)po = hv; *(uint4*)(po + C) = hv; *(uint4*)(po + 2 * C) = lv;
+                if (planes_f16 == 2) {
+                    unsigned short* po = planes + ((long)b * rows_max + r) * 2 * C + c;
+                    *(uint4*)po = hv; *(uint4*)(po + C) = lv;
+                } else {
+                    unsigned short* po = planes + ((long)b * rows_max + r) * 3 * C + c;
+                    *(uint4*)po = hv; *(uint4*)(po + C) = hv; *(uint4*)(po + 2 * C) = lv;
+                }
             }
         }
         return;
@@ -255,8 +279,8 @@
         if (planes) {
             unsigned short hi, lo;
             split2x(v, planes_f16, hi, lo);
-            unsigned short* o = planes + ((long)b * rows_max + r) * 3 * C;
-            o[c] = hi; o[C + c] = hi; o[2 * C + c] = lo;
+            if (planes_f16 == 2) { unsigned short* o = planes + ((long)b * rows_max + r) * 2 * C; o[c] = hi; o[C + c] = lo; }
+            else { unsigned short* o = planes + ((long)b * rows_max + r) * 3 * C; o[c] = hi; o[C + c] = hi; o[2 * C + c] = lo; }
         }
     }
 }
diff --git a/zerovox_amd/csrc/zvx.hip b/zerovox_amd/csrc/zvx.hip
--- a/zerovox_amd/csrc/zvx.hip
+++ b/zerovox_amd/csrc/zvx.hip
@@ -265,7 +265,7 @@
         if (!a.Wp && a.dtype != DT_F32) { auto it = packed.find(a.W); if (it != packed.end()) a.Wp = it->second; }
         a.slab_small = slab_small | (spk_s2_fuse ? 0 : 32); a.xcd_flat = slab_flat;
         profiled([&] { return gemm_variant_of(a); }, [&] {
-            const int id = a.fused == 2 ? launch_rb2fuse(a, stream) : (a.fused ? launch_resfuse(a, stream) : launch_gemm(a, stream));
+            const int id = a.fused == 2 ? launch_rb2fuse(a, stream) : (a.fused == 1 ? launch_resfuse(a, stream) : launch_gemm(a, stream));
             if (id < 0) fail(ZVX_E_INVALID, "launch_gemm rejected shape M=%d N=%d K=%d taps=%d", a.M, a.N, a.K, a.ntaps);
             return id;
         }, [&](GemmEvent& ev) {
@@ -273,7 +273,7 @@
             const double esz = dtype_size(a.dtype);
             const double cells = (double)a.M * a.nbatch * a.nheads * a.N;
             ev.bytes = ((double)a.M * a.nbatch * a.nheads) * (double)(a.K + a.K2) * esz + (double)a.N * ((double)a.K * a.ntaps + a.K2) * esz * (a.fused ? 2 : 1) +
-                       (a.out ? cells * dtype_size(a.out_dtype) : 0.0) + ((a.res_mode && !a.fused) ? cells * dtype_size(a.res_dtype) : 0.0) +
+                       (a.out ? cells * dtype_size(a.out_dtype) : 0.0) + ((a.res_mode && (!a.fused || a.fused == 3)) ? cells * dtype_size(a.res_dtype) : 0.0) +
                        ((a.accum && (a.accum_mode & 1)) ? cells * dtype_size(a.accum_dtype) : 0.0) + ((a.accum && (a.accum_mode & 2)) ? cells * dtype_size(a.accum_dtype) : 0.0);
         });
         if (sat_check && a.nheads == 1) {
@@ -398,8 +398,26 @@
     if (first) fail(ZVX_E_MANIFEST, "manifest: empty");
 }
 
-void build_split_weights(zvx_ctx* c, bool f16) {
-    const char* sfx = f16 ? ".s3h" : ".s3";
+static void drop_split_weights(zvx_ctx* c, const char* sfx, const char* arena) {
+    const size_t n = strlen(sfx);
+    bool any = false;
+    for (auto it = c->tensors.begin(); it != c->tensors.end();) {
+        const std::string& k = it->first;
+        if (it->second.kind == 's' && k.size() > n && k.compare(k.size() - n, n, sfx) == 0) { c->packed.erase(it->second.dev); it = c->tensors.erase(it); any = true; }
+        else ++it;
+    }
+    auto b = c->bufs.find(arena);
+    if (any && b != c->bufs.end() && b->second.base) {
+        c->drain_for_free();
+        HIPCHK(hipFree(b->second.base)); b->second.base = nullptr; b->second.p = nullptr; b->second.cap = 0;
+    }
+}
+void build_split_weights(zvx_ctx* c, int mode) {
+    const bool f16 = mode >= 2, two = mode == 3;
+    if (two) { drop_split_weights(c, ".s3h", "weights_split_h"); drop_split_weights(c, ".s3", "weights_split"); }
+    else drop_split_weights(c, ".s2h", "weights_split_2h");
+    const char* sfx = two ? ".s2h" : (f16 ? ".s3h" : ".s3");
+    const int np = two ? 2 : 3;
     if (c->has(std::string("enc.0.wqk") + sfx)) return;
     std::vector<std::pair<std::string, Tensor>> add;
     size_t stotal = 0;
@@ -408,11 +426,13 @@
         const bool mine = kv.first.rfind("enc.", 0) == 0;
         if (!mine || t.kind != 'f' || t.dtype != DT_F32 || t.dims.size() != 3 || (3 * t.dim(2)) % 16 || t.dim(1) % 8) continue;
         Tensor s3 = t;
-        s3.kind = 's'; s3.dtype = f16 ? DT_F16 : DT_BF16; s3.dims = {t.dim(0), t.dim(1), 3 * t.dim(2)}; s3.numel = t.numel * 3; s3.host = nullptr;
+        if (two && t.dim(2) % 16) continue;
+        s3.kind = 's'; s3.dtype = f16 ? DT_F16 : DT_BF16; s3.numel = t.numel * np; s3.host = nullptr;
+        if (two) s3.dims = {2 * t.dim(0), t.dim(1), t.dim(2)}; else s3.dims = {t.dim(0), t.dim(1), 3 * t.dim(2)};
         stotal += ((s3.numel * 2 + 255) & ~(size_t)255) + ((packed_weight_elems(s3.dim(0), s3.dim(1), s3.dim(2)) * 2 + 255) & ~(size_t)255);
         add.emplace_back(kv.first + sfx, s3);
     }
-    char* sarena = stotal ? (char*)c->buf(f16 ? "weights_split_h" : "weights_split", stotal) : nullptr;
+    char* sarena = stotal ? (char*)c->buf(two ? "weights_split_2h" : (f16 ? "weights_split_h" : "weights_split"), stotal) : nullptr;
     float* mx_d = f16 ? c->fbuf("weights_split_absmax", 64) : nullptr;
     size_t soff = 0;
     for (auto& kv : add) {
@@ -431,7 +451,8 @@
             s3.alpha = ldexpf(1.f, -sh);
         }
         s3.dev = sarena + soff; soff += (s3.numel * 2 + 255) & ~(size_t)255;
-        launch_split3_weights((const float*)src.dev, s3.dev, (long)src.dim(0) * src.dim(1), src.dim(2), c->stream, f16 ? 1 : 0, scale);
+        if (two) launch_split2_weights((const float*)src.dev, s3.dev, src.dim(0), src.dim(1), src.dim(2), c->stream, scale);
+        else launch_split3_weights((const float*)src.dev, s3.dev, (long)src.dim(0) * src.dim(1), src.dim(2), c->stream, f16 ? 1 : 0, scale);
         void* pk = sarena + soff; soff += (packed_weight_elems(s3.dim(0), s3.dim(1), s3.dim(2)) * 2 + 255) & ~(size_t)255;
         launch_pack_weights(s3.dev, s3.dim(0), s3.dim(1), s3.dim(2), pk, c->stream);
         c->packed[s3.dev] = pk;
@@ -561,7 +582,7 @@
         }
         for (auto& kv : add) c->tensors[kv.first] = kv.second;
     }
-    if (c->enc_split) build_split_weights(c, c->enc_split == 2);
+    if (c->enc_split) build_split_weights(c, c->enc_split);
     HIPCHK(hipStreamSynchronize(c->stream));
     DevBuf& st = c->bufs["weights_staging"];
     HIPCHK(hipFree(st.base)); st.base = nullptr; st.p = nullptr; st.cap = 0;
@@ -572,7 +593,7 @@
     if (it == c->cfg.end()) fail(ZVX_E_MANIFEST, "manifest: missing cfg 'precision'");
     if (it->second == "bf16") c->dt = DT_BF16; else if (it->second == "f32") c->dt = DT_F32;
     else fail(ZVX_E_MANIFEST, "manifest: unknown precision '%s'", it->second.c_str());
-    c->enc_split = c->dt == DT_BF16 ? (c->cfg.count("enc_split") ? std::max(0, std::min(2, c->cfg_int("enc_split"))) : 2) : 0;
+    c->enc_split = c->dt == DT_BF16 ? (c->cfg.count("enc_split") ? std::max(0, std::min(3, c->cfg_int("enc_split"))) : 3) : 0;
     c->H = c->cfg_int("hidden"); c->emb_dim = c->cfg_int("emb_dim"); c->punct_dim = c->cfg_int("punct_dim");
     c->n_phone_rows = c->cfg_int("n_phone_rows"); c->n_punct_rows = c->cfg_int("n_punct_rows");
     c->max_txt_len = c->cfg_int("max_txt_len"); c->max_mel_len = c->cfg_int("max_mel_len");
@@ -620,13 +641,22 @@
     const int ydt = h16 ? (int)DT_F16 : (int)DT_F32;
     void* hbuf = c->buf("fft.h", (size_t)B * Ls * F * es);
 
-    const bool sp16 = c->enc_split == 2;
-    const char* const s3 = sp16 ? ".s3h" : ".s3";
+    const bool sp2 = c->enc_split == 3;
+    const int sp16 = sp2 ? 2 : (c->enc_split == 2 ? 1 : 0);
+    const int np = sp2 ? 2 : 3;
+    const char* const s3 = sp2 ? ".s2h" : (sp16 ? ".s3h" : ".s3");
     const bool split = dt == DT_F32 && c->enc_split && c->has(w.p + ".wqk" + s3);
-    void* xs = split ? c->buf("fft.xs", (size_t)B * Ls * 3 * H * 2) : nullptr;
+    void* xs = split ? c->buf("fft.xs", (size_t)B * Ls * np * H * 2) : nullptr;
     auto split_of = [&](const float* src, int C, void* dst) { launch_split3(src, C, dst, B, Ls, len_dev, C, c->stream, sp16); };
     auto as_split = [&](GemmArgs& a, const void* planes, int C, const std::string& wname) {
         const Tensor& ws = c->t(wname + s3);
+        if (sp2) {
+            a.dtype = DT_F16; a.X = planes; a.x_bs = (long)Ls * 2 * C; a.ldx = 2 * C; a.K = C; a.fused = 3;
+            a.alpha = ws.alpha;
+            a.W = ws.dev; a.ldw = C; a.w_ts = (long)ws.dim(1) * C;
+            a.flops = 2.0 * (double)a.M * a.nbatch * a.N * C * a.ntaps;
+            return;
+        }
         a.dtype = sp16 ? DT_F16 : DT_BF16; a.X = planes; a.x_bs = (long)Ls * 3 * C; a.ldx = 3 * C; a.K = 3 * C;
         a.alpha = ws.alpha;
         a.W = ws.dev; a.ldw = 3 * C; a.w_ts = (long)ws.dim(1) * 3 * C;
@@ -743,11 +773,11 @@
         set_taps_1d(a, c->ffn_k0, 1);
         a.bias = c->pf(w.p + ".b1"); a.bias_mode = 1; a.act = ACT_RELU;
         a.out = hbuf; a.o_bs = (long)Ls * F; a.ldo = F;
-        void* hs = split ? c->buf("fft.hs", (size_t)B * Ls * 3 * F * 2) : nullptr;
+        void* hs = split ? c->buf("fft.hs", (size_t)B * Ls * np * F * 2) : nullptr;
         if (split) {
             if (w.scln) split_of((const float*)x, H, xs);
             as_split(a, xs, H, w.p + ".w1");
-            a.out_dtype = DT_F32; a.out_split3 = sp16 ? 2 : 1; a.out = hs; a.o_bs = (long)Ls * 3 * F; a.ldo = 3 * F;
+            a.out_dtype = DT_F32; a.out_split3 = sp2 ? 3 : (sp16 ? 2 : 1); a.out = hs; a.o_bs = (long)Ls * np * F; a.ldo = np * F;
         }
         c->gemm(a);
     }
@@ -759,7 +789,7 @@
         a.bias = c->pf(w.p + ".b2"); a.bias_mode = 1;
         a.res = x; a.r_bs = (long)Ls * H; a.ldr = H; a.res_mode = 1; a.res_dtype = dt;
         a.out = yv; a.out_dtype = ydt; a.o_bs = (long)Ls * H; a.ldo = H;
-        if (split) as_split(a, c->buf("fft.hs", (size_t)B * Ls * 3 * F * 2), F, w.p + ".w2");
+        if (split) as_split(a, c->buf("fft.hs", (size_t)B * Ls * np * F * 2), F, w.p + ".w2");
         c->gemm(a);
     }
     c->timed(0, ln_bytes, [&] {
@@ -2231,7 +2261,7 @@
     {"f16_sat_check", &zvx_ctx::sat_check, flag},
     {"poison_pads", &zvx_ctx::poison_pads, flag},
     {"max_frames", &zvx_ctx::max_frames, [](int64_t v) { return v >= 1 && v <= (1 << 24); }},
-    {"enc_split", &zvx_ctx::enc_split, [](int64_t v) { return v >= 0 && v <= 2; }},
+    {"enc_split", &zvx_ctx::enc_split, [](int64_t v) { return v >= 0 && v <= 3; }},
     {"attn_f32", &zvx_ctx::use_attn_f32, flag},
     {"flash", &zvx_ctx::use_flash, flag},
     {"front_overlap", &zvx_ctx::front_overlap, [](int64_t v) { return v >= 0 && v <= 2; }},
@@ -2305,7 +2335,7 @@
         if (k == "front_overlap") c->front_dirty_main = true;
         if (k == "enc_split") {
             if (c->dt != DT_BF16) c->enc_split = 0;
-            if (c->enc_split) { c->sync(); build_split_weights(c, c->enc_split == 2); }
+            if (c->enc_split) { c->sync(); build_split_weights(c, c->enc_split); }
         }
     });
 }
diff --git a/zerovox_amd/csrc/zvx_kernels.h b/zerovox_amd/csrc/zvx_kernels.h
--- a/zerovox_amd/csrc/zvx_kernels.h
+++ b/zerovox_amd/csrc/zvx_kernels.h
@@ -169,6 +169,7 @@
 
 void launch_split3(const float* x, int ldx, void* out, int B, int rows_max, const int* rows, int C, hipStream_t s, int f16 = 0);
 void launch_split3_weights(const float* w, void* out, long nrows, int K, hipStream_t s, int f16 = 0, float scale = 1.f);
+void launch_split2_weights(const float* w, void* out, int ntaps, int N, int K, hipStream_t s, float scale);
 void launch_absmax(const float* x, size_t n, float* out , hipStream_t s);
 
 void launch_embed(const int* phoneme, const int* puncts, const float* emb, int emb_dim, const float* pemb,
```

Measured after the change: 350.5 million, median of 6. No clear change (+0.6%).
